# facebookresearch/PartDistillation

Measured on AMD Instinct MI355X. Metric: images/sec training step, R50 Mask2Former 1024² bs=2/GPU, 1/2/4/8 MI355X, higher is better.
Workload: dtype bf16

## Files before the change

### include/pd_attention.h

```cpp
#ifndef PD_ATTENTION_H
#define PD_ATTENTION_H

#include <stdint.h>

#ifdef __cplusplus
extern "C" {
#endif

int64_t pd_attn_workspace_floats(int B, int H, int Lq, int Lk);

int pd_attn_fwd_d32(const void *q, const void *k, const void *v, const uint8_t *mask, void *o, float *lse,
                    float *workspace, int B, int H, int Lq, int Lk, float scale, int dtype, void *stream);

int pd_attn_fwd_d32_ld(const void *q, const void *k, const void *v, const uint8_t *mask, void *o, float *lse,
                       float *workspace, int B, int H, int Lq, int Lk, float scale, int dtype, int ld_kv, void *stream);

int pd_attn_bwd_d32(const void *q, const void *k, const void *v, const uint8_t *mask, const void *o, const void *d_o,
                    const float *lse, void *dq, void *dk, void *dv, float *workspace, int B, int H, int Lq, int Lk,
                    float scale, int dtype, void *stream);

int pd_attn_bwd_d32_ld(const void *q, const void *k, const void *v, const uint8_t *mask, const void *o, const void *d_o,
                       const float *lse, void *dq, void *dk, void *dv, float *workspace, int B, int H, int Lq, int Lk,
                       float scale, int dtype, int ld_kv, void *stream);

#ifdef __cplusplus
}
#endif
#endif
```

### include/pd_declayer.h

```cpp
#ifndef PD_DECLAYER_H
#define PD_DECLAYER_H

#include <stdint.h>

#ifdef __cplusplus
extern "C" {
#endif

typedef struct PdDecPack {
  const void *src;
  void *dst;
  int32_t rows, cols, transpose;
} PdDecPack;
int64_t pd_dec_pack_table_bytes(int count);
int pd_dec_pack_grouped(const PdDecPack *descs, int count, void *table_host_pinned, void *table_device, void *stream);

int pd_dec_split(void);
int64_t pd_dec_workspace_bytes(int R);

int pd_dec_fwd_a(const void *o, const float *res, const float *qpos, int pos_div, const void *w_o, const void *b_o, const float *ln_w,
                 const float *ln_b, float eps, const void *w_qkv, const void *b_qkv, float *z, float *stats, float *y, void *y_c,
                 void *ypos_c, void *q, void *k, void *v, int R, void *stream);

int pd_dec_fwd_b(const void *o, const float *res, const float *qpos, int pos_div, const void *w_o, const void *b_o, const float *ln2_w,
                 const float *ln2_b, const void *w_1, const void *b_1, const void *w_2, const void *b_2, const float *ln3_w,
                 const float *ln3_b, const float *dn_w, const float *dn_b, const void *m0_w, const void *m0_b, const void *m1_w,
                 const void *m1_b, const void *m2_w, const void *m2_b, const void *wq_next, const void *bq_next, float eps, float *z2,
                 float *stats2, void *y2_c, void *h, float *z3, float *stats3, float *y3, void *ypos_c, float *dec_out, float *hstats,
                 void *ef, void *qc_next, void *workspace, int R, int flags, void *stream);

int pd_dec_bwd_b(const void *dqc_next, const void *wqT_next, const float *d_out, const float *d_res, const float *y3, const float *hstats,
                 const float *dn_w, float *dgb_dn, const float *z3, const float *stats3, const float *ln3_w, float *dgb3, float *db3,
                 float *pos_acc, int pos_div, const void *w2T, const void *h, const void *w1T, const float *z2, const float *stats2,
                 const float *ln2_w, float *dgb2, float *db2, const void *woT, void *dz3_c, void *dh, float *dz2, void *dz2_c, void *d_o,
                 void *workspace, int R, void *stream);

int pd_dec_bwd_a(const void *dq, const void *dk, const void *dv, const void *wqkvT, const float *dz_in, const float *z, const float *stats,
                 const float *ln_w, float *dgb, float *db, float *pos_acc, int pos_div, const void *woT, float *dz1, void *dz1_c, void *d_o,
                 int R, void *stream);

#ifdef __cplusplus
}
#endif
#endif
```

### partdistillation_amd/csrc/attention.hip

```cpp
#include <hip/hip_runtime.h>
#include <math.h>
#include <stdint.h>

#include "pd_attention.h"
#include "pd_common.h"
#include "mfma_bf16.h"
#include "pd_msda.h"

int g_attn_bwd_kc = 0;

namespace {

constexpr int D = 32;
constexpr int QP = 128;
constexpr int KT = 64;
constexpr int KC_FWD = 256;
constexpr int KC_DQ = 512;

typedef unsigned short bf16_t;

__device__ __forceinline__ float bf2f(bf16_t h) { return __uint_as_float((unsigned)h << 16); }
__device__ __forceinline__ bf16_t f2bf(float f)
{
  unsigned u = __float_as_uint(f);
// ... 92 lines not shown
    __syncthreads();
    if (!active) continue;
    const int kk0 = half * (KT / 2);
    float s[KT / 2];
    float m_t = -INFINITY;
    const uint8_t *mrow = mask ? mask + ((int64_t)b * Lq + qi) * Lk + k0 + kk0 : nullptr;
#pragma unroll
    for (int kk = 0; kk < KT / 2; ++kk) {
      float acc = 0.f;
#pragma unroll
      for (int d = 0; d < D; ++d) acc += qv[d] * Ks[kk0 + kk][d];
      const bool blocked = (k0 + kk0 + kk >= Lk) || (mrow && mrow[kk]);
      s[kk] = blocked ? -INFINITY : acc;
      m_t = fmaxf(m_t, s[kk]);
    }
    const float m_new = fmaxf(m_run, m_t);
    if (m_new == -INFINITY) continue;
    const float alpha = __expf(m_run - m_new);
    l_run *= alpha;
#pragma unroll
    for (int d = 0; d < D; ++d) o[d] *= alpha;
#pragma unroll
    for (int kk = 0; kk < KT / 2; ++kk) {
      const float p = __expf(s[kk] - m_new);
      l_run += p;
#pragma unroll
      for (int d = 0; d < D; ++d) o[d] += p * Vs[kk0 + kk][d];
    }
    m_run = m_new;
  }
  __syncthreads();
  const int ql = threadIdx.x & (QP - 1);
  if (half == 1) {
#pragma unroll
    for (int d = 0; d < D; ++d) red[ql][d] = o[d];
    red[ql][D] = m_run; red[ql][D + 1] = l_run;
  }
  __syncthreads();
  if (half == 0 && active) {
    const float m2 = red[ql][D], l2 = red[ql][D + 1];
    const float M = fmaxf(m_run, m2);
    const float a1 = (M == -INFINITY) ? 0.f : __expf(m_run - M), a2 = (M == -INFINITY) ? 0.f : __expf(m2 - M);
    const int64_t base = (((int64_t)b * H + h) * nchunk + chunk) * Lq + qi;
    float *po = part_o + base * D;
#pragma unroll
    for (int d = 0; d < D; d += 4)
      *reinterpret_cast<float4 *>(po + d) = make_float4(a1 * o[d] + a2 * red[ql][d], a1 * o[d + 1] + a2 * red[ql][d + 1],
                                                        a1 * o[d + 2] + a2 * red[ql][d + 2], a1 * o[d + 3] + a2 * red[ql][d + 3]);
    part_ml[base * 2] = M;
    part_ml[base * 2 + 1] = a1 * l_run + a2 * l2;
  }
}

template <typename T>
__global__ __launch_bounds__(256) void attn_fwd_combine(const float *__restrict__ part_o, const float *__restrict__ part_ml,
                                                         T *__restrict__ o, float *__restrict__ lse, int B, int H, int Lq, int nchunk)
{
  const int g = blockIdx.x * 8 + (threadIdx.x >> 5), d = threadIdx.x & 31;
  if (g >= B * H * Lq) return;
  const int qi = g % Lq, bh = g / Lq, h = bh % H, b = bh / H;
  float M = -INFINITY;
  const float2 *ml = reinterpret_cast<const float2 *>(part_ml) + (int64_t)bh * nchunk * Lq + qi;
  const float *po = part_o + ((int64_t)bh * nchunk * Lq + qi) * D + d;
  int c = 0;
  for (; c + 8 <= nchunk; c += 8) {
    float m8[8];
#pragma unroll
    for (int u = 0; u < 8; ++u) m8[u] = ml[(int64_t)(c + u) * Lq].x;
#pragma unroll
    for (int u = 0; u < 8; ++u) M = fmaxf(M, m8[u]);
  }
  for (; c < nchunk; ++c) M = fmaxf(M, ml[(int64_t)c * Lq].x);
  float L = 0.f, acc = 0.f;
  if (M != -INFINITY) {
    c = 0;
    for (; c + 8 <= nchunk; c += 8) {
      float2 s8[8];
      float o8[8];
#pragma unroll
      for (int u = 0; u < 8; ++u) { s8[u] = ml[(int64_t)(c + u) * Lq]; o8[u] = po[(int64_t)(c + u) * Lq * D]; }
#pragma unroll
      for (int u = 0; u < 8; ++u) {
        const float w = __expf(s8[u].x - M);
        L += w * s8[u].y;
        acc += w * o8[u];
      }
    }
    for (; c < nchunk; ++c) {
      const float2 sv = ml[(int64_t)c * Lq];
      const float w = __expf(sv.x - M);
      L += w * sv.y;
      acc += w * po[(int64_t)c * Lq * D];
    }
  }
  const float outv = L > 0.f ? acc / L : 0.f;
  T *dst = o + ((int64_t)qi * B + b) * (H * D) + h * D + d;
  if (sizeof(T) == 2) *reinterpret_cast<bf16_t *>(dst) = f2bf(outv); else *reinterpret_cast<float *>(dst) = outv;
  if (d == 0) lse[(int64_t)bh * Lq + qi] = L > 0.f ? M + __logf(L) : -INFINITY;
}

template <typename T>
__global__ __launch_bounds__(256) void attn_bwd_dq(const T *__restrict__ q, const T *__restrict__ k, const T *__restrict__ v,
                                                    const uint8_t *__restrict__ mask, const T *__restrict__ o, const T *__restrict__ d_o,
                                                    const float *__restrict__ lse, float *__restrict__ part_dq, int B, int H, int Lq,
                                                    int Lk, float scale, int nchunk, int qpass)
{
  __shared__ __attribute__((aligned(16))) float Ks[KT][D];
  __shared__ __attribute__((aligned(16))) float Vs[KT][D];
  __shared__ float red[QP][D];
  const int chunk = blockIdx.x, h = blockIdx.y, b = blockIdx.z;
  const int qi = qpass * QP + (threadIdx.x & (QP - 1)), half = threadIdx.x >> 7;
  const bool active = qi < Lq;
  float qv[D], dov[D], dq[D];
  float lse_q = 0.f, delta = 0.f;
#pragma unroll
  for (int d = 0; d < D; ++d) dq[d] = 0.f;
  if (active) {
    const int64_t off = ((int64_t)qi * B + b) * (H * D) + h * D;
    float ov[D];
    IO<T>::load32(q + off, qv);
    IO<T>::load32(d_o + off, dov);
    IO<T>::load32(o + off, ov);
#pragma unroll
    for (int d = 0; d < D; ++d) { delta += dov[d] * ov[d]; qv[d] *= scale; }
    lse_q = lse[((int64_t)b * H + h) * Lq + qi];
  }
  const int kbeg = chunk * KC_DQ, kend = min(Lk, kbeg + KC_DQ);
  for (int k0 = kbeg; k0 < kend; k0 += KT) {
    __syncthreads();
    stage_rows<T>(k, Ks, k0, Lk, b, h, B, H);
    stage_rows<T>(v, Vs, k0, Lk, b, h, B, H);
    __syncthreads();
    if (!active || lse_q == -INFINITY) continue;
    const int kk0 = half * (KT / 2);
    const uint8_t *mrow = mask ? mask + ((int64_t)b * Lq + qi) * Lk + k0 + kk0 : nullptr;
#pragma unroll 4
    for (int kk = 0; kk < KT / 2; ++kk) {
      const bool blocked = (k0 + kk0 + kk >= Lk) || (mrow && mrow[kk]);
      if (blocked) continue;
      float s = 0.f, dp = 0.f;
#pragma unroll
      for (int d = 0; d < D; ++d) { s += qv[d] * Ks[kk0 + kk][d]; dp += dov[d] * Vs[kk0 + kk][d]; }
      const float ds = __expf(s - lse_q) * (dp - delta);
#pragma unroll
      for (int d = 0; d < D; ++d) dq[d] += ds * Ks[kk0 + kk][d];
    }
  }
  __syncthreads();
  const int ql = threadIdx.x & (QP - 1);
  if (half == 1) {
#pragma unroll
    for (int d = 0; d < D; ++d) red[ql][d] = dq[d];
  }
  __syncthreads();
  if (half == 0 && active) {
    float *dst = part_dq + ((((int64_t)b * H + h) * nchunk + chunk) * Lq + qi) * D;
#pragma unroll
    for (int d = 0; d < D; d += 4)
      *reinterpret_cast<float4 *>(dst + d) = make_float4((dq[d] + red[ql][d]) * scale, (dq[d + 1] + red[ql][d + 1]) * scale,
                                                         (dq[d + 2] + red[ql][d + 2]) * scale, (dq[d + 3] + red[ql][d + 3]) * scale);
  }
}

template <typename T>
__global__ __launch_bounds__(256) void attn_bwd_dq_reduce(const float *__restrict__ part_dq, T *__restrict__ dq, int B, int H, int Lq, int nchunk)
{
  const int g = blockIdx.x * 8 + (threadIdx.x >> 5), d = threadIdx.x & 31;
  if (g >= B * H * Lq) return;
  const int qi = g % Lq, bh = g / Lq, h = bh % H, b = bh / H;
  float acc = 0.f;
  for (int c = 0; c < nchunk; ++c) acc += part_dq[(((int64_t)bh * nchunk + c) * Lq + qi) * D + d];
  T *dst = dq + ((int64_t)qi * B + b) * (H * D) + h * D + d;
  if (sizeof(T) == 2) *reinterpret_cast<bf16_t *>(dst) = f2bf(acc); else *reinterpret_cast<float *>(dst) = acc;
}

// ... 351 lines not shown
#pragma unroll
            for (int i = 0; i < 4; ++i) {
              const bool blocked = (mybits >> (8 * g + 4 * hh + i)) & 1u;
              p[i] = blocked ? 0.f : __expf(sN[4 * g + i] * scale - la[i]);
              ds[i] = p[i] * (dpN[4 * g + i] - da[i]);
            }
            pN[g] = pack4(p[0], p[1], p[2], p[3]);
            dsN[g] = pack4(ds[0], ds[1], ds[2], ds[3]);
          }
#pragma unroll
          for (int j = 0; j < 4; ++j) {
            mma(dvacc, lds4(&Ot[r][32 * sub + 8 * j + 4 * hh]), pN[j]);
            mma(dkacc, lds4(&Qt[r][32 * sub + 8 * j + 4 * hh]), dsN[j]);
          }
        }
      }
      if (kvalid) {
        bf16_t *dkp = dk + ((int64_t)key * B + b) * rs + h * D, *dvp = dv + ((int64_t)key * B + b) * rs + h * D;
#pragma unroll
        for (int g = 0; g < 4; ++g) {
          *reinterpret_cast<bf16x4 *>(dkp + 8 * g + 4 * hh) = pack4(dkacc[4 * g] * scale, dkacc[4 * g + 1] * scale, dkacc[4 * g + 2] * scale, dkacc[4 * g + 3] * scale);
          *reinterpret_cast<bf16x4 *>(dvp + 8 * g + 4 * hh) = pack4(dvacc[4 * g], dvacc[4 * g + 1], dvacc[4 * g + 2], dvacc[4 * g + 3]);
        }
      }
    }
  }
  for (int w = 0; w < 4; ++w) {
    __syncthreads();
    if (wave == w) {
#pragma unroll
      for (int sub = 0; sub < 4; ++sub)
#pragma unroll
        for (int e = 0; e < 16; ++e) {
          const int d = (e & 3) + 8 * (e >> 2) + 4 * hh;
          if (w == 0) dqs[32 * sub + r][d] = dqacc[sub][e];
          else dqs[32 * sub + r][d] += dqacc[sub][e];
        }
    }
  }
  __syncthreads();
  for (int idx = tid; idx < Lq * D; idx += 256) {
    const int qq = idx >> 5, d = idx & 31;
    const float val = dqs[qq][d] * scale;
    if (nchunk == 1) dq[((int64_t)qq * B + b) * rs + h * D + d] = f2bf(val);
    else part_dq[((bh * nchunk + chunk) * Lq + qq) * D + d] = val;
  }
}

inline int nchunks(int Lk, int kc) { return Lk <= 0 ? 1 : (Lk + kc - 1) / kc; }
inline int mfma_fwd_chunk(int B, int H, int Lk)
{
  int kc = KC_FWD;
  if (Lk > KC_FWD)
    while (kc > 64 && (int64_t)B * H * nchunks(Lk, kc) < 512) kc >>= 1;
  return kc;
}
inline int mfma_bwd_chunk(int B, int H, int Lk)
{
  if (g_attn_bwd_kc == 128 || g_attn_bwd_kc == 256 || g_attn_bwd_kc == 512) return g_attn_bwd_kc;
  int kc = KC_DQ;
  while (kc > 128 && (int64_t)B * H * nchunks(Lk, kc) < 256) kc >>= 1;
  return kc;
}

int check(const void *a, const void *b, const void *c, int B, int H, int Lq, int Lk, int dtype, const char *who)
{
  if (B < 0 || H <= 0 || Lq < 0 || Lk < 0) return pd_set_error(PD_ERR_INVALID_ARG, "%s: bad sizes B=%d H=%d Lq=%d Lk=%d", who, B, H, Lq, Lk);
  if (dtype != PD_F32 && dtype != PD_BF16) return pd_set_error(PD_ERR_INVALID_ARG, "%s: dtype %d (float32 / bfloat16 only)", who, dtype);
  if (B * Lq * Lk != 0 && (!a || !b || !c)) return pd_set_error(PD_ERR_INVALID_ARG, "%s: null pointer", who);
  return PD_OK;
}

}

int g_pd_dbg_attn_scalar = 0;

extern "C" int64_t pd_attn_workspace_floats(int B, int H, int Lq, int Lk)
{
  const int64_t n1 = (int64_t)B * H * nchunks(Lk, mfma_fwd_chunk(B, H, Lk)) * Lq * (D + 2);
  const int64_t n2 = (int64_t)B * H * nchunks(Lk, 128) * Lq * D;
  return (n1 > n2 ? n1 : n2) + 64;
}

extern "C" int pd_attn_fwd_d32(const void *q, const void *k, const void *v, const uint8_t *mask, void *o, float *lse,
                               float *workspace, int B, int H, int Lq, int Lk, float scale, int dtype, void *stream_)
{
  return pd_attn_fwd_d32_ld(q, k, v, mask, o, lse, workspace, B, H, Lq, Lk, scale, dtype, H * D, stream_);
}

extern "C" int pd_attn_fwd_d32_ld(const void *q, const void *k, const void *v, const uint8_t *mask, void *o, float *lse,
                                  float *workspace, int B, int H, int Lq, int Lk, float scale, int dtype, int ld_kv, void *stream_)
{
  int rc = check(q, k, v, B, H, Lq, Lk, dtype, "pd_attn_fwd_d32");
  if (rc) return rc;
  if (ld_kv < H * D || (ld_kv & 7)) return pd_set_error(PD_ERR_INVALID_ARG, "pd_attn_fwd_d32_ld: ld_kv=%d (>= H * 32, a multiple of 8)", ld_kv);
  if (ld_kv != H * D && !(dtype == PD_BF16 && Lq <= MQ && Lk > 0 && !g_pd_dbg_attn_scalar))
    return pd_set_error(PD_ERR_INVALID_ARG, "pd_attn_fwd_d32_ld: strided k / v only on the matrix-core path (bf16, <= %d queries)", MQ);
  if (B * Lq == 0) return PD_OK;
  if (!o || !lse || !workspace) return pd_set_error(PD_ERR_INVALID_ARG, "pd_attn_fwd_d32: null output");
  hipStream_t s = (hipStream_t)stream_;
  if (dtype == PD_BF16 && Lq <= MQ && Lk > 0 && !g_pd_dbg_attn_scalar) {
    const int kc = mfma_fwd_chunk(B, H, Lk), nc = nchunks(Lk, kc);
    float *part_o = workspace, *part_ml = workspace + (int64_t)B * H * nc * Lq * D;
    if (mask) hipLaunchKernelGGL(attn_fwd_mfma<true>, dim3(nc, H, B), dim3(256), 0, s, (const bf16_t *)q, (const bf16_t *)k, (const bf16_t *)v,
                                 mask, (bf16_t *)o, lse, part_o, part_ml, B, H, Lq, Lk, scale, nc, ld_kv, kc);
    else hipLaunchKernelGGL(attn_fwd_mfma<false>, dim3(nc, H, B), dim3(256), 0, s, (const bf16_t *)q, (const bf16_t *)k, (const bf16_t *)v,
                            mask, (bf16_t *)o, lse, part_o, part_ml, B, H, Lq, Lk, scale, nc, ld_kv, kc);
    if (nc > 1) hipLaunchKernelGGL(attn_fwd_combine<bf16_t>, dim3((B * H * Lq + 7) / 8), dim3(256), 0, s, part_o, part_ml, (bf16_t *)o, lse, B, H, Lq, nc);
    return pd_check_launch("pd_attn_fwd_d32");
  }
  const int nc = nchunks(Lk, KC_FWD);
  float *part_o = workspace, *part_ml = workspace + (int64_t)B * H * nc * Lq * D;
  for (int qp = 0; qp * QP < Lq; ++qp) {
    if (dtype == PD_BF16)
      hipLaunchKernelGGL(attn_fwd_partial<bf16_t>, dim3(nc, H, B), dim3(256), 0, s, (const bf16_t *)q, (const bf16_t *)k,
                         (const bf16_t *)v, mask, part_o, part_ml, B, H, Lq, Lk, scale, nc, qp);
    else
      hipLaunchKernelGGL(attn_fwd_partial<float>, dim3(nc, H, B), dim3(256), 0, s, (const float *)q, (const float *)k,
                         (const float *)v, mask, part_o, part_ml, B, H, Lq, Lk, scale, nc, qp);
  }
  const int groups = B * H * Lq;
  if (dtype == PD_BF16)
    hipLaunchKernelGGL(attn_fwd_combine<bf16_t>, dim3((groups + 7) / 8), dim3(256), 0, s, part_o, part_ml, (bf16_t *)o, lse, B, H, Lq, nc);
  else
    hipLaunchKernelGGL(attn_fwd_combine<float>, dim3((groups + 7) / 8), dim3(256), 0, s, part_o, part_ml, (float *)o, lse, B, H, Lq, nc);
  return pd_check_launch("pd_attn_fwd_d32");
}

extern "C" int pd_attn_bwd_d32(const void *q, const void *k, const void *v, const uint8_t *mask, const void *o, const void *d_o,
                               const float *lse, void *dq, void *dk, void *dv, float *workspace, int B, int H, int Lq,
                               int Lk, float scale, int dtype, void *stream_)
{
  return pd_attn_bwd_d32_ld(q, k, v, mask, o, d_o, lse, dq, dk, dv, workspace, B, H, Lq, Lk, scale, dtype, H * D, stream_);
}

extern "C" int pd_attn_bwd_d32_ld(const void *q, const void *k, const void *v, const uint8_t *mask, const void *o, const void *d_o,
                                  const float *lse, void *dq, void *dk, void *dv, float *workspace, int B, int H, int Lq,
                                  int Lk, float scale, int dtype, int ld_kv, void *stream_)
{
  int rc = check(q, k, v, B, H, Lq, Lk, dtype, "pd_attn_bwd_d32");
  if (rc) return rc;
  if (ld_kv < H * D || (ld_kv & 3)) return pd_set_error(PD_ERR_INVALID_ARG, "pd_attn_bwd_d32_ld: ld_kv=%d (>= H * 32, a multiple of 4)", ld_kv);
  if (ld_kv != H * D && !(dtype == PD_BF16 && Lq <= MQ && !g_pd_dbg_attn_scalar))
    return pd_set_error(PD_ERR_INVALID_ARG, "pd_attn_bwd_d32_ld: strided k / v only on the matrix-core path (bf16, <= %d queries)", MQ);
  if (B * Lq * Lk == 0) return PD_OK;
  if (!o || !d_o || !lse || !dq || !dk || !dv || !workspace) return pd_set_error(PD_ERR_INVALID_ARG, "pd_attn_bwd_d32: null pointer");
  hipStream_t s = (hipStream_t)stream_;
  const int groups = B * H * Lq;
  if (dtype == PD_BF16 && Lq <= MQ && !g_pd_dbg_attn_scalar) {
    const int kc = mfma_bwd_chunk(B, H, Lk), nc = nchunks(Lk, kc);
    if (mask) hipLaunchKernelGGL(attn_bwd_mfma<true>, dim3(nc, H, B), dim3(256), 0, s, (const bf16_t *)q, (const bf16_t *)k, (const bf16_t *)v,
                                 mask, (const bf16_t *)o, (const bf16_t *)d_o, lse, workspace, (bf16_t *)dq, (bf16_t *)dk, (bf16_t *)dv,
                                 B, H, Lq, Lk, scale, nc, kc, ld_kv);
    else hipLaunchKernelGGL(attn_bwd_mfma<false>, dim3(nc, H, B), dim3(256), 0, s, (const bf16_t *)q, (const bf16_t *)k, (const bf16_t *)v,
                            mask, (const bf16_t *)o, (const bf16_t *)d_o, lse, workspace, (bf16_t *)dq, (bf16_t *)dk, (bf16_t *)dv,
                            B, H, Lq, Lk, scale, nc, kc, ld_kv);
    if (nc > 1) hipLaunchKernelGGL(attn_bwd_dq_reduce<bf16_t>, dim3((groups + 7) / 8), dim3(256), 0, s, workspace, (bf16_t *)dq, B, H, Lq, nc);
    return pd_check_launch("pd_attn_bwd_d32");
  }
  const int nc = nchunks(Lk, KC_DQ);
  if (dtype == PD_BF16) {
    for (int qp = 0; qp * QP < Lq; ++qp)
      hipLaunchKernelGGL(attn_bwd_dq<bf16_t>, dim3(nc, H, B), dim3(256), 0, s, (const bf16_t *)q, (const bf16_t *)k, (const bf16_t *)v,
                         mask, (const bf16_t *)o, (const bf16_t *)d_o, lse, workspace, B, H, Lq, Lk, scale, nc, qp);
    hipLaunchKernelGGL(attn_bwd_dq_reduce<bf16_t>, dim3((groups + 7) / 8), dim3(256), 0, s, workspace, (bf16_t *)dq, B, H, Lq, nc);
    hipLaunchKernelGGL(attn_bwd_dkv<bf16_t>, dim3((Lk + 255) / 256, H, B), dim3(256), 0, s, (const bf16_t *)q, (const bf16_t *)k,
                       (const bf16_t *)v, mask, (const bf16_t *)o, (const bf16_t *)d_o, lse, (bf16_t *)dk, (bf16_t *)dv, B, H, Lq, Lk, scale);
  } else {
    for (int qp = 0; qp * QP < Lq; ++qp)
      hipLaunchKernelGGL(attn_bwd_dq<float>, dim3(nc, H, B), dim3(256), 0, s, (const float *)q, (const float *)k, (const float *)v,
                         mask, (const float *)o, (const float *)d_o, lse, workspace, B, H, Lq, Lk, scale, nc, qp);
    hipLaunchKernelGGL(attn_bwd_dq_reduce<float>, dim3((groups + 7) / 8), dim3(256), 0, s, workspace, (float *)dq, B, H, Lq, nc);
    hipLaunchKernelGGL(attn_bwd_dkv<float>, dim3((Lk + 255) / 256, H, B), dim3(256), 0, s, (const float *)q, (const float *)k,
                       (const float *)v, mask, (const float *)o, (const float *)d_o, lse, (float *)dk, (float *)dv, B, H, Lq, Lk, scale);
  }
  return pd_check_launch("pd_attn_bwd_d32");
}
```

### partdistillation_amd/csrc/cmdbuf.hip

```cpp
#include <hip/hip_runtime.h>
#include <stdint.h>
#include <string.h>

#include <type_traits>
#include <utility>

#include "pd_common.h"
#include "pd_cmdbuf.h"
#include "pd_attention.h"
#include "pd_conv.h"
#include "pd_declayer.h"
#include "pd_criterion.h"
#include "pd_fused.h"
#include "pd_gemm.h"
#include "pd_grouping.h"
#include "pd_igemm.h"
#include "pd_input.h"
#include "pd_kmeans.h"
#include "pd_msda.h"
#include "pd_mx8.h"
#include "pd_optim.h"
#include "pd_rowwise.h"
#include "pd_smallgemm.h"
#include "pd_stem.h"
// ... 15 lines not shown
    return static_cast<T>(static_cast<int64_t>(w));
  }
}

template <auto F> struct Thunk;
template <class... A, int (*F)(A...)>
struct Thunk<F> {
  static constexpr int nargs = (int)sizeof...(A);
  template <size_t... I>
  static int invoke(const uint64_t *w, std::index_sequence<I...>) { return F(word_to<A>(w[I])...); }
  static int call(const uint64_t *w) { return invoke(w, std::index_sequence_for<A...>{}); }
};

struct Entry { const char *name; int (*call)(const uint64_t *); int nargs; };
#define PD_E(f) {#f, &Thunk<&f>::call, Thunk<&f>::nargs}
const Entry kTable[] = {
  PD_E(pd_adamw_clipped),
  PD_E(pd_adamw_clipped_shadow),
  PD_E(pd_add_layernorm_bwd),
  PD_E(pd_add_layernorm_bwd_amax),
  PD_E(pd_add_layernorm_fwd),
  PD_E(pd_add_layernorm_fwd_amax),
  PD_E(pd_add_rows_amax_f32),
  PD_E(pd_affine_act_bwd2_bf16),
  PD_E(pd_affine_act_bwd_bf16),
  PD_E(pd_affine_act_fwd_bf16),
  PD_E(pd_attn_bwd_d32),
  PD_E(pd_attn_fwd_d32),
  PD_E(pd_attn_mask_u8),
  PD_E(pd_cast_bf16_f32_amax),
  PD_E(pd_colsum_acc),
  PD_E(pd_conv3x3_nhwc_f16x2),
  PD_E(pd_conv3x3_nhwc_f32x3),
  PD_E(pd_conv3x3_wgrad_nhwc_f16x2),
  PD_E(pd_conv3x3_wgrad_nhwc_f32x3),
  PD_E(pd_conv_bf16_dgrad),
  PD_E(pd_conv_bf16_fwd),
  PD_E(pd_conv_bf16_wgrad),
  PD_E(pd_conv_bf16_wgrad_grouped),
  PD_E(pd_dec_bwd_a),
  PD_E(pd_dec_bwd_b),
  PD_E(pd_dec_fwd_a),
  PD_E(pd_dec_fwd_b),
  PD_E(pd_dec_pack_grouped),
  PD_E(pd_decoder_head_bf16),
  PD_E(pd_filter_transpose_grouped),
  PD_E(pd_gemm_tn_f16x2),
  PD_E(pd_gemm_tn_f16x2_bf16out),
  PD_E(pd_gemm_tn_f32),
  PD_E(pd_gemm_tn_f32x3),
  PD_E(pd_gemm_tn_f32x3_pre),
  PD_E(pd_gemm_tn_f32x3_relu_bits),
  PD_E(pd_gemm_tn_f32x3_relumask),
  PD_E(pd_gemm_wgrad_acc_f16x2_ws),
  PD_E(pd_gemm_wgrad_acc_f32),
  PD_E(pd_gemm_wgrad_acc_f32x3),
  PD_E(pd_gemm_wgrad_acc_f32x3_ws),
  PD_E(pd_gemm_wgrad_f16x2_grouped),
  PD_E(pd_gemm_wgrad_f32),
  PD_E(pd_gemm_wgrad_f32x3_grouped),
  PD_E(pd_gn_coeffs_bwd),
  PD_E(pd_gn_coeffs_fwd),
  PD_E(pd_igemm_bf16),
  PD_E(pd_igemm_bf16_seq),
  PD_E(pd_kmeans_assign),
  PD_E(pd_kmeans_assign_bounded),
  PD_E(pd_kmeans_assign_partial),
  PD_E(pd_kmeans_reduce),
  PD_E(pd_kmeans_reduce_update),
  PD_E(pd_kmeans_reduce_update_shift),
  PD_E(pd_kmeans_update),
  PD_E(pd_layernorm_rows_f32_bwd),
  PD_E(pd_layernorm_rows_f32_fwd),
  PD_E(pd_loss_vectors_bwd),
  PD_E(pd_loss_vectors_fwd),
  PD_E(pd_lsa_batched),
  PD_E(pd_mask_assign),
  PD_E(pd_mask_point_losses_bwd),
  PD_E(pd_mask_point_losses_fwd),
  PD_E(pd_matcher_costs),
  PD_E(pd_copy_segments),
  PD_E(pd_attn_fwd_d32_ld),
  PD_E(pd_attn_bwd_d32_ld),
  PD_E(pd_match_point_logits),
  PD_E(pd_swin_merge_ln_fwd),
  PD_E(pd_swin_tail_ln_fwd),
  PD_E(pd_swin_tail_ln_bwd),
  PD_E(pd_swin_merge_ln_bwd),
  PD_E(pd_matcher_point_terms),
  PD_E(pd_maxpool3s2_bwd_bf16),
  PD_E(pd_maxpool3s2_fwd_bf16),
  PD_E(pd_mem_prep_bwd),
  PD_E(pd_mem_prep_fwd),
  PD_E(pd_memcpy_d2d_async),
  PD_E(pd_memset_async),
  PD_E(pd_msda_backward),
  PD_E(pd_msda_forward),
  PD_E(pd_msda_forward_amax),
  PD_E(pd_msda_fused_backward),
  PD_E(pd_msda_fused_forward),
  PD_E(pd_msda_prep_bwd),
  PD_E(pd_msda_prep_bwd_amax),
  PD_E(pd_msda_prep_fwd),
  PD_E(pd_multi_gather_sumsq),
  PD_E(pd_mx8_gemm),
  PD_E(pd_mx8_quantize_bf16),
  PD_E(pd_mx8_quantize_grouped),
  PD_E(pd_nc_affine2_amax_f32),
  PD_E(pd_nc_affine2_f32),
  PD_E(pd_nc_affine_amax_f32),
  PD_E(pd_nc_affine_f32),
  PD_E(pd_nc_sums_f32),
  PD_E(pd_normalize_u8_nhwc),
  PD_E(pd_pair_logits_bwd_rows),
  PD_E(pd_pair_logits_bwd_tok),
  PD_E(pd_pair_logits_fwd),
  PD_E(pd_point_sample_nhwc_f32),
  PD_E(pd_point_sample_nhwc_f32_bf16),
  PD_E(pd_point_sample_planar_bwd_f32),
  PD_E(pd_point_sample_planar_f32),
  PD_E(pd_point_sample_u8),
  PD_E(pd_relu_bwd_colsum),
  PD_E(pd_resample_cols_u8),
  PD_E(pd_resample_rows_u8),
  PD_E(pd_resize_bilinear_nhwc_f32),
  PD_E(pd_rle_sample_u8),
  PD_E(pd_row_amax_f32),
  PD_E(pd_scores_argmax_u8),
  PD_E(pd_sgemm_nn_bf16),
  PD_E(pd_sgemm_nn_splitn_bf16),
  PD_E(pd_sgemm_tn_batched_bf16),
  PD_E(pd_sgemm_tn_bf16),
  PD_E(pd_sgemm_tn_multi_bf16),
  PD_E(pd_sgemm_tn_splitk_bf16),
  PD_E(pd_sgemm_wgrad_bf16),
  PD_E(pd_sgemm_wgrad_grouped_bf16),
  PD_E(pd_sgemm_wgrad_split_bf16),
  PD_E(pd_skinny_linear_bwd),
  PD_E(pd_skinny_linear_fwd),
  PD_E(pd_split3_bf16),
  PD_E(pd_stem7x7_fwd),
  PD_E(pd_stem7x7_wgrad),
  PD_E(pd_sum3_sum2_f32),
  PD_E(pd_sumsq_accumulate),
  PD_E(pd_swin_ln_bwd),
  PD_E(pd_swin_ln_fwd),
  PD_E(pd_transpose_batched_f32),
  PD_E(pd_uncertain_points),
  PD_E(pd_upsample2x_bwd_nhwc_f32),
  PD_E(pd_upsample_add_amax_nhwc_f32),
  PD_E(pd_upsample_add_nhwc_f32),
  PD_E(pd_wgrad_bf16),
  PD_E(pd_wgrad_bf16_seq),
  PD_E(pd_window_attn_bwd_w12),
  PD_E(pd_window_attn_fwd_w12),
};
constexpr int kCount = (int)(sizeof(kTable) / sizeof(kTable[0]));
}

extern "C" int pd_memset_async(void *dst, int value, int64_t bytes, void *stream)
{
  if (bytes <= 0) return PD_OK;
  return hipMemsetAsync(dst, value, (size_t)bytes, (hipStream_t)stream) == hipSuccess ? PD_OK : pd_set_error(PD_ERR_LAUNCH, "pd_memset_async failed");
}

extern "C" int pd_memcpy_d2d_async(void *dst, const void *src, int64_t bytes, void *stream)
// ... 36 lines not shown
```

### partdistillation_amd/csrc/common.hip

```cpp
#include <hip/hip_runtime.h>
#include <stdarg.h>
#include <stdio.h>
#include <string.h>

#include "pd_common.h"
#include "pd_msda.h"

namespace {
thread_local char g_err[512] = {0};
}

int pd_set_error(int code, const char *fmt, ...)
{
  va_list ap;
  va_start(ap, fmt);
  vsnprintf(g_err, sizeof(g_err), fmt, ap);
  va_end(ap);
  return code;
}

int pd_check_launch(const char *what)
{
  hipError_t e = hipGetLastError();
  if (e == hipSuccess) return PD_OK;
  return pd_set_error(PD_ERR_LAUNCH, "%s: %s", what, hipGetErrorString(e));
}

extern "C" const char *pd_last_error(void) { return g_err; }
extern "C" int pd_abi_version(void) { return 40; }

extern int g_pd_dbg_atomic_scope;
extern int g_pd_dbg_force_generic;
extern int g_pd_dbg_ablate;
extern int g_pd_dbg_x3_narrow;
extern int g_pd_dbg_f16x2;
extern int g_pd_dbg_wgrad_wide;
extern "C" void pd_dbg_set_wgrad_xcd(int v);
extern "C" void pd_dbg_set_wgrad_fast(int v);
extern int g_pd_dbg_bwd_variant;
extern int g_pd_dbg_msda_gate_pct;
extern int g_pd_dbg_wgrad_wgs;
extern int g_pd_dbg_bwd_threads;
extern int g_pd_dbg_attn_scalar;
extern int g_pd_dbg_wattn;
extern int g_pd_dbg_x3;
extern int g_pd_dbg_kmeans;
extern int g_pd_dbg_conv_group_rows;
extern int g_pd_dbg_conv_xcd_major;
extern int g_pd_dbg_sgemm_deep;
extern int g_ig_bn, g_ig_nst, g_ig_splits, g_ig_patch, g_ig_pcls;
extern int g_mx_bn, g_mx_nst;
extern int g_swin_ln_abl;
extern int g_ln_bwd_cap;
extern int g_crit_abl;
extern int g_attn_bwd_kc;
extern int g_wg_nst, g_wg_splits, g_wg_mode;
extern "C" int pd_debug_set(const char *key, int value)
{
  if (!key) return PD_ERR_INVALID_ARG;
  if (!strcmp(key, "msda_bwd_atomic_scope")) { g_pd_dbg_atomic_scope = value; return PD_OK; }
  if (!strcmp(key, "msda_ablate")) { g_pd_dbg_ablate = value; return PD_OK; }
  if (!strcmp(key, "msda_bwd_variant")) { g_pd_dbg_bwd_variant = value; return PD_OK; }
  if (!strcmp(key, "msda_gate_pct")) { g_pd_dbg_msda_gate_pct = value; return PD_OK; }
  if (!strcmp(key, "attn_scalar")) { g_pd_dbg_attn_scalar = value; return PD_OK; }
  if (!strcmp(key, "msda_bwd_threads")) { g_pd_dbg_bwd_threads = value; return PD_OK; }
  if (!strcmp(key, "wgrad_wgs")) { g_pd_dbg_wgrad_wgs = value; return PD_OK; }
  if (!strcmp(key, "kmeans_ablate")) { g_pd_dbg_kmeans = value; return PD_OK; }
  if (!strcmp(key, "wg_nst")) { g_wg_nst = value; return PD_OK; }
  if (!strcmp(key, "wg_splits")) { g_wg_splits = value; return PD_OK; }
  if (!strcmp(key, "wg_mode")) { g_wg_mode = value; return PD_OK; }
  if (!strcmp(key, "ig_bn")) { g_ig_bn = value; return PD_OK; }
  if (!strcmp(key, "ig_patch")) { g_ig_patch = value; return PD_OK; }
  if (!strcmp(key, "ig_pcls")) { g_ig_pcls = value; return PD_OK; }
  if (!strcmp(key, "ig_nst")) { g_ig_nst = value; return PD_OK; }
  if (!strcmp(key, "mx_bn")) { g_mx_bn = value; return PD_OK; }
  if (!strcmp(key, "attn_bwd_kc")) { g_attn_bwd_kc = value; return PD_OK; }
  if (!strcmp(key, "crit_abl")) { g_crit_abl = value; return PD_OK; }
  if (!strcmp(key, "ln_bwd_cap")) { g_ln_bwd_cap = value; return PD_OK; }
  if (!strcmp(key, "swin_ln_abl")) { g_swin_ln_abl = value; return PD_OK; }
  if (!strcmp(key, "mx_nst")) { g_mx_nst = value; return PD_OK; }
  if (!strcmp(key, "ig_splits")) { g_ig_splits = value; return PD_OK; }
  if (!strcmp(key, "sgemm_deep")) { g_pd_dbg_sgemm_deep = value; return PD_OK; }
  if (!strcmp(key, "conv_group_rows")) { g_pd_dbg_conv_group_rows = value; return PD_OK; }
  if (!strcmp(key, "conv_xcd_major")) { g_pd_dbg_conv_xcd_major = value; return PD_OK; }
  if (!strcmp(key, "x3_ablate")) { g_pd_dbg_x3 = value; return PD_OK; }
  if (!strcmp(key, "f16x2_tile")) { g_pd_dbg_f16x2 = value; return PD_OK; }
  if (!strcmp(key, "wgrad_wide")) { g_pd_dbg_wgrad_wide = value; return PD_OK; }
  if (!strcmp(key, "wgrad_xcd")) { pd_dbg_set_wgrad_xcd(value); return PD_OK; }
  if (!strcmp(key, "wgrad_fast")) { pd_dbg_set_wgrad_fast(value); return PD_OK; }
  if (!strcmp(key, "x3_narrow")) { g_pd_dbg_x3_narrow = value; return PD_OK; }
  if (!strcmp(key, "wattn_ablate")) { g_pd_dbg_wattn = value; return PD_OK; }
  if (!strcmp(key, "msda_force_generic")) { g_pd_dbg_force_generic = value; return PD_OK; }
  return pd_set_error(PD_ERR_INVALID_ARG, "pd_debug_set: unknown key %s", key);
}
```

### partdistillation_amd/csrc/declayer.hip

```cpp
#include <hip/hip_runtime.h>
#include <stdint.h>
#include <stdlib.h>

#include "pd_common.h"
#include "pd_msda.h"
#include "pd_declayer.h"

namespace {

typedef unsigned short bf16_t;
typedef __bf16 hwbf16x8 __attribute__((ext_vector_type(8)));
typedef __bf16 hwbf16x2 __attribute__((ext_vector_type(2)));
typedef float f32x4 __attribute__((ext_vector_type(4)));
typedef float f32x2 __attribute__((ext_vector_type(2)));

constexpr int C = 256, FF = 2048, RB = 16, NTH = 512, NW = 8;
constexpr int PA = C + 8;
constexpr int PZ = C + 4;

__device__ __forceinline__ float bf2f(bf16_t h) { return __uint_as_float((unsigned)h << 16); }
__device__ __forceinline__ float bf_lo(unsigned u) { return __uint_as_float(u << 16); }
__device__ __forceinline__ float bf_hi(unsigned u) { return __uint_as_float(u & 0xffff0000u); }
__device__ __forceinline__ unsigned pk_bf16(float lo, float hi)
{
  const f32x2 x = {lo, hi};
  return __builtin_bit_cast(unsigned, __builtin_convertvector(x, hwbf16x2));
}
__device__ __forceinline__ uint2 pack4(float a, float b, float c, float d) { return make_uint2(pk_bf16(a, b), pk_bf16(c, d)); }
__device__ __forceinline__ float rbf(float x) { return bf_lo(pk_bf16(x, 0.f)); }

template <int CTRL>
__device__ __forceinline__ float dpp_mov(float v)
{
  return __int_as_float(__builtin_amdgcn_update_dpp(0, __float_as_int(v), CTRL, 0xF, 0xF, true));
}
__device__ __forceinline__ float wave_sum(float v)
{
  v += dpp_mov<0xB1>(v);
  v += dpp_mov<0x4E>(v);
  v += dpp_mov<0x141>(v);
  v += dpp_mov<0x140>(v);
  v += __shfl_xor(v, 16, 64);
  v += __shfl_xor(v, 32, 64);
  return v;
}
__device__ __forceinline__ float4 add4(float4 a, float4 b) { return make_float4(a.x + b.x, a.y + b.y, a.z + b.z, a.w + b.w); }
__device__ __forceinline__ float4 ld4(const float *p) { return *reinterpret_cast<const float4 *>(p); }
__device__ __forceinline__ void st4(float *p, float4 v) { *reinterpret_cast<float4 *>(p) = v; }
__device__ __forceinline__ float4 zero4() { return make_float4(0.f, 0.f, 0.f, 0.f); }

__device__ __forceinline__ void zero_acc(f32x4 (&acc)[2])
{
#pragma unroll
  for (int t = 0; t < 2; ++t)
#pragma unroll
    for (int r = 0; r < 4; ++r) acc[t][r] = 0.f;
}

template <bool BIAS, bool RELU>
__device__ __forceinline__ void epi4(const f32x4 &a, const bf16_t *bias_lds, int n, float (&v)[4])
{
#pragma unroll
  for (int r = 0; r < 4; ++r) v[r] = a[r];
  if (BIAS) {
    const uint2 b = *reinterpret_cast<const uint2 *>(bias_lds + n);
    v[0] += bf_lo(b.x); v[1] += bf_hi(b.x); v[2] += bf_lo(b.y); v[3] += bf_hi(b.y);
  }
  if (RELU) {
#pragma unroll
    for (int r = 0; r < 4; ++r) v[r] = fmaxf(v[r], 0.f);
  }
}
template <bool BIAS, bool RELU>
__device__ __forceinline__ void store_tile_bf16(const f32x4 (&acc)[2], const bf16_t *bias_lds, int nb_bias, bf16_t *dst, int pitch, int nb, int lane)
{
  const int m = lane & 15, g = lane >> 4;
#pragma unroll
  for (int t = 0; t < 2; ++t) {
    float v[4];
    epi4<BIAS, RELU>(acc[t], bias_lds, nb_bias + 16 * t + 4 * g, v);
    *reinterpret_cast<uint2 *>(dst + m * pitch + nb + 16 * t + 4 * g) = pack4(v[0], v[1], v[2], v[3]);
  }
}
// ... 24 lines not shown
{
  for (int i = tid * 8; i < n; i += NTH * 8) *reinterpret_cast<uint4 *>(dst + i) = *reinterpret_cast<const uint4 *>(src + i);
}
__device__ __forceinline__ void lds_copy_f32(float *dst, const float *__restrict__ src, int n, int tid)
{
  for (int i = tid * 4; i < n; i += NTH * 4) st4(dst + i, ld4(src + i));
}

__device__ __forceinline__ float4 ln_row(float4 v, float4 gm, float4 bt, float eps, float &mu, float &rs)
{
  const float s = (v.x + v.y) + (v.z + v.w);
  mu = wave_sum(s) * (1.f / C);
  v.x -= mu; v.y -= mu; v.z -= mu; v.w -= mu;
  const float q = (v.x * v.x + v.y * v.y) + (v.z * v.z + v.w * v.w);
  rs = rsqrtf(wave_sum(q) * (1.f / C) + eps);
  return make_float4(v.x * rs * gm.x + bt.x, v.y * rs * gm.y + bt.y, v.z * rs * gm.z + bt.z, v.w * rs * gm.w + bt.w);
}
__device__ __forceinline__ float4 ln_row_bwd(float4 t, float4 z, float mu, float rs, float4 gm, float4 &ag, float4 &ab)
{
  float4 h = make_float4((z.x - mu) * rs, (z.y - mu) * rs, (z.z - mu) * rs, (z.w - mu) * rs);
  ag.x += t.x * h.x; ag.y += t.y * h.y; ag.z += t.z * h.z; ag.w += t.w * h.w;
  ab = add4(ab, t);
  t.x *= gm.x; t.y *= gm.y; t.z *= gm.z; t.w *= gm.w;
  const float s1 = (t.x + t.y) + (t.z + t.w);
  const float s2 = (t.x * h.x + t.y * h.y) + (t.z * h.z + t.w * h.w);
  const float m1 = wave_sum(s1) * (1.f / C), m2 = wave_sum(s2) * (1.f / C);
  return make_float4(rs * (t.x - m1 - h.x * m2), rs * (t.y - m1 - h.y * m2), rs * (t.z - m1 - h.z * m2), rs * (t.w - m1 - h.w * m2));
}
__device__ __forceinline__ float4 bf4(const bf16_t *p)
{
  const uint2 u = *reinterpret_cast<const uint2 *>(p);
  return make_float4(bf_lo(u.x), bf_hi(u.x), bf_lo(u.y), bf_hi(u.y));
}
__device__ __forceinline__ void st_bf4(bf16_t *p, float4 v) { *reinterpret_cast<uint2 *>(p) = pack4(v.x, v.y, v.z, v.w); }

template <int NARR>
__device__ __forceinline__ void flush_colsums(const float *red, float *const (&outs)[NARR], int tid)
{
  for (int i = tid; i < NARR * C; i += NTH) {
    const int k = i / C, c = i - k * C;
    if (!outs[k]) continue;
    float s = 0.f;
#pragma unroll
    for (int w = 0; w < NW; ++w) s += red[(w * NARR + k) * C + c];
    atomicAdd(outs[k] + c, s);
  }
}

constexpr int BLK = 8192;
struct WHalf { uint4 v[2][4]; };
__device__ __forceinline__ void wloadh(WHalf &w, const bf16_t *__restrict__ blk, int half, int lane)
{
  const bf16_t *p = blk + lane * 8 + half * (4 * 512);
#pragma unroll
  for (int t = 0; t < 2; ++t)
#pragma unroll
    for (int s = 0; s < 4; ++s) w.v[t][s] = *reinterpret_cast<const uint4 *>(p + (t * 8 + s) * 512);
}
__device__ __forceinline__ void wmmah(f32x4 (&acc)[2], const WHalf &w, const bf16_t *xs)
{
#pragma unroll
  for (int s = 0; s < 4; ++s) {
    const hwbf16x8 x = *reinterpret_cast<const hwbf16x8 *>(xs + 32 * s);
    acc[0] = __builtin_amdgcn_mfma_f32_16x16x32_bf16(__builtin_bit_cast(hwbf16x8, w.v[0][s]), x, acc[0], 0, 0, 0);
    acc[1] = __builtin_amdgcn_mfma_f32_16x16x32_bf16(__builtin_bit_cast(hwbf16x8, w.v[1][s]), x, acc[1], 0, 0, 0);
  }
}
#define PD_HP(h) do { if ((h) < 2 * NBLK) wloadh(w[(h) & 3], bp((h) >> 1), (h) & 1, lane); } while (0)
#define PD_BLK(b, XS) do { PD_HP(2 * (b) + 3); wmmah(acc, w[(2 * (b)) & 3], (XS)); PD_HP(2 * (b) + 4); wmmah(acc, w[(2 * (b) + 1) & 3], (XS) + 128); } while (0)

__device__ __forceinline__ void slab_store(float *__restrict__ slab, const f32x4 (&acc)[2], int nb, int lane)
{
  const int m = lane & 15, g = lane >> 4;
#pragma unroll
  for (int t = 0; t < 2; ++t) st4(slab + m * C + nb + 16 * t + 4 * g, make_float4(acc[t][0], acc[t][1], acc[t][2], acc[t][3]));
}
__device__ __forceinline__ float4 slab_sum(const float *__restrict__ slabs, int P, int row, int lane)
{
  float4 s = zero4();
  for (int p = 0; p < P; ++p) s = add4(s, ld4(slabs + (size_t)p * (RB * C) + row * C + 4 * lane));
  return s;
}

struct FwdA {
  const bf16_t *o; const float *res, *qpos; int pos_div;
  const bf16_t *w_o, *b_o; const float *ln_w, *ln_b; float eps;
  const bf16_t *w_qkv, *b_qkv;
  float *z, *stats, *y; bf16_t *y_c, *ypos_c, *q, *k, *v; int R;
};

__global__ __launch_bounds__(NTH) void dec_fwd_a(const FwdA a)
{
  extern __shared__ __attribute__((aligned(16))) unsigned char smem[];
  bf16_t *X0 = reinterpret_cast<bf16_t *>(smem);
  bf16_t *X1 = X0 + RB * PA;
  bf16_t *X2 = X1 + RB * PA;
  bf16_t *X3 = X2 + RB * PA;
  bf16_t *X4 = X3 + RB * PA;
  float *Zs = reinterpret_cast<float *>(X4 + RB * PA);
  bf16_t *Bs = reinterpret_cast<bf16_t *>(Zs + RB * PZ);
  float *Ls = reinterpret_cast<float *>(Bs + 4 * C);
  const int tid = threadIdx.x, wave = tid >> 6, lane = tid & 63, r0 = blockIdx.x * RB, R = a.R;
  constexpr int NBLK = 4;
  auto bp = [&](int b) { return b == 0 ? a.w_o + (size_t)wave * BLK : a.w_qkv + (size_t)((b - 1) * 8 + wave) * BLK; };
  WHalf w[4];
  PD_HP(0); PD_HP(1); PD_HP(2);
  tile_in(X0, a.o, r0, R, tid);
  lds_copy_bf16(Bs, a.b_o, C, tid);
  lds_copy_bf16(Bs + C, a.b_qkv, 3 * C, tid);
  lds_copy_f32(Ls, a.ln_w, C, tid);
  lds_copy_f32(Ls + C, a.ln_b, C, tid);
  float4 res[2], pos[2];
#pragma unroll
  for (int i = 0; i < 2; ++i) {
    const int m = min(r0 + 2 * wave + i, R - 1);
    res[i] = ld4(a.res + (size_t)m * C + 4 * lane);
    pos[i] = ld4(a.qpos + (size_t)(m / a.pos_div) * C + 4 * lane);
  }
  __syncthreads();
  const int xo = (lane & 15) * PA + 8 * (lane >> 4);
  f32x4 acc[2];
  zero_acc(acc);
  PD_BLK(0, X0 + xo);
  store_tile_f32r<true>(acc, Bs, 32 * wave, Zs, 32 * wave, lane);
  __syncthreads();
#pragma unroll
  for (int i = 0; i < 2; ++i) {
    const int row = 2 * wave + i, m = r0 + row;
    const float4 zv = add4(ld4(Zs + row * PZ + 4 * lane), res[i]);
    float mu, rs;
    const float4 y = ln_row(zv, ld4(Ls + 4 * lane), ld4(Ls + C + 4 * lane), a.eps, mu, rs);
    const float4 yp = add4(y, pos[i]);
    st_bf4(X1 + row * PA + 4 * lane, y);
    st_bf4(X2 + row * PA + 4 * lane, yp);
    if (m < R) {
      st4(a.z + (size_t)m * C + 4 * lane, zv);
      st4(a.y + (size_t)m * C + 4 * lane, y);
      if (lane == 0) { a.stats[m] = mu; a.stats[R + m] = rs; }
    }
  }
  __syncthreads();
  tile_out(a.y_c, X1, r0, R, tid);
  tile_out(a.ypos_c, X2, r0, R, tid);
  zero_acc(acc);
  PD_BLK(1, X2 + xo);
  store_tile_bf16<true, false>(acc, Bs + C, 32 * wave, X0, PA, 32 * wave, lane);
  zero_acc(acc);
  PD_BLK(2, X2 + xo);
  store_tile_bf16<true, false>(acc, Bs + 2 * C, 32 * wave, X3, PA, 32 * wave, lane);
  zero_acc(acc);
  PD_BLK(3, X1 + xo);
  store_tile_bf16<true, false>(acc, Bs + 3 * C, 32 * wave, X4, PA, 32 * wave, lane);
  __syncthreads();
  tile_out(a.q, X0, r0, R, tid);
  tile_out(a.k, X3, r0, R, tid);
  tile_out(a.v, X4, r0, R, tid);
}
constexpr size_t kSmemFwdA = (size_t)5 * RB * PA * 2 + (size_t)RB * PZ * 4 + 4 * C * 2 + 2 * C * 4;

struct FwdB {
  const bf16_t *o; const float *res, *qpos; int pos_div;
  const bf16_t *w_o, *b_o; const float *ln2_w, *ln2_b;
  const bf16_t *w_1, *b_1, *w_2, *b_2; const float *ln3_w, *ln3_b, *dn_w, *dn_b;
  const bf16_t *m_w[3], *m_b[3], *wq_next, *bq_next; float eps;
  float *z2, *stats2; bf16_t *y2_c, *h; float *z3, *stats3, *y3; bf16_t *ypos_c; float *dec_out, *hstats;
  bf16_t *ef, *qc_next; int R; float *slabs, *rows; int nsplit;
};

template <int P, int PART, bool LAYER, bool MLP>
__global__ __launch_bounds__(NTH) void dec_fwd_b(const FwdB a)
{
  static_assert(PART != 2 || !LAYER, "PART 2 starts behind the FFN");
  constexpr int NB = 8 / P, HW = FF / P, PHS = HW + 8;
  extern __shared__ __attribute__((aligned(16))) unsigned char smem[];
  bf16_t *X0 = reinterpret_cast<bf16_t *>(smem);
  bf16_t *X1 = X0 + RB * PA;
  bf16_t *X2 = X1 + RB * PA;
  bf16_t *Hs = X2 + RB * PA;
  float *Zs = reinterpret_cast<float *>(Hs + RB * (PHS > PA ? PHS : PA));
  bf16_t *Bs = reinterpret_cast<bf16_t *>(Zs + RB * PZ);
  float *Ls = reinterpret_cast<float *>(Bs + (6 * C + FF));
  float *Ys = Ls + 6 * C;
  float *Ps = Ys + RB * PZ;
  const int tid = threadIdx.x, wave = tid >> 6, lane = tid & 63, R = a.R;
  const int rb = blockIdx.x / P, p = blockIdx.x - rb * P, r0 = rb * RB;
  constexpr int B1 = C, B2 = C + FF, BM = 2 * C + FF, BQ = 5 * C + FF;
  constexpr int I0 = LAYER ? 2 * NB + 1 : 0;
  constexpr int NBLK = I0 + (MLP && PART != 1 ? 4 : 0);
  auto bp = [&](int b) -> const bf16_t * {
    if (LAYER && b == 0) return a.w_o + (size_t)wave * BLK;
// ... 69 lines not shown
      const int idx = i * NTH + tid, row = idx / (HW / 8), col = (idx % (HW / 8)) * 8;
      if (r0 + row < R) *reinterpret_cast<uint4 *>(a.h + (size_t)(r0 + row) * FF + p * HW + col) = *reinterpret_cast<const uint4 *>(Hs + row * PHS + col);
    }
    const int ho = (lane & 15) * PHS + 8 * (lane >> 4);
    zero_acc(acc);
#pragma unroll
    for (int c = 0; c < NB; ++c) {
      PD_BLK(NB + 1 + c, Hs + ho + 256 * c);
    }
    if (PART == 1) {
      slab_store(a.slabs + (size_t)(rb * P + p) * (RB * C), acc, 32 * wave, lane);
      return;
    }
    store_tile_f32r<true>(acc, Bs + B2, 32 * wave, Zs, 32 * wave, lane);
    __syncthreads();
  }
#pragma unroll
  for (int i = 0; i < 2; ++i) {
    const int row = 2 * wave + i, m = r0 + row;
    float4 y3 = ld4(Ys + row * PZ + 4 * lane);
    float mu, rs;
    if (LAYER || PART == 2) {
      float4 x3;
      if (PART == 2) {
        x3 = add4(slab_sum(a.slabs + (size_t)rb * a.nsplit * (RB * C), a.nsplit, row, lane), bf4(Bs + B2 + 4 * lane));
        x3 = make_float4(rbf(x3.x), rbf(x3.y), rbf(x3.z), rbf(x3.w));
      } else {
        x3 = ld4(Zs + row * PZ + 4 * lane);
      }
      const float4 zv = add4(x3, y3);
      y3 = ln_row(zv, ld4(Ls + 2 * C + 4 * lane), ld4(Ls + 3 * C + 4 * lane), a.eps, mu, rs);
      if (m < R) {
        st4(a.z3 + (size_t)m * C + 4 * lane, zv);
        st4(a.y3 + (size_t)m * C + 4 * lane, y3);
        if (lane == 0) { a.stats3[m] = mu; a.stats3[R + m] = rs; }
      }
    }
    st_bf4(X2 + row * PA + 4 * lane, add4(y3, ld4(Ps + row * PZ + 4 * lane)));
    const float4 d = ln_row(y3, ld4(Ls + 4 * C + 4 * lane), ld4(Ls + 5 * C + 4 * lane), a.eps, mu, rs);
    st_bf4(X0 + row * PA + 4 * lane, d);
    if (m < R) {
      st4(a.dec_out + (size_t)m * C + 4 * lane, d);
      if (lane == 0) { a.hstats[m] = mu; a.hstats[R + m] = rs; }
    }
  }
  __syncthreads();
  tile_out(a.ypos_c, X2, r0, R, tid);
  if (!MLP) return;
  zero_acc(acc);
  PD_BLK(I0, X0 + xo);
  store_tile_bf16<true, true>(acc, Bs + BM, 32 * wave, X1, PA, 32 * wave, lane);
  __syncthreads();
  zero_acc(acc);
  PD_BLK(I0 + 1, X1 + xo);
  store_tile_bf16<true, true>(acc, Bs + BM + C, 32 * wave, X0, PA, 32 * wave, lane);
  __syncthreads();
  zero_acc(acc);
  PD_BLK(I0 + 2, X0 + xo);
  store_tile_bf16<true, false>(acc, Bs + BM + 2 * C, 32 * wave, X1, PA, 32 * wave, lane);
  zero_acc(acc);
  PD_BLK(I0 + 3, X2 + xo);
  store_tile_bf16<true, false>(acc, Bs + BQ, 32 * wave, Hs, PA, 32 * wave, lane);
  __syncthreads();
  tile_out(a.qc_next, Hs, r0, R, tid);
  {
    const int row = tid >> 5, col = (tid & 31) * 8, m = r0 + row;
    if (m < R) {
      const int B = a.pos_div, q = m / B, b = m - q * B, Q = R / B;
      *reinterpret_cast<uint4 *>(a.ef + ((size_t)b * Q + q) * C + col) = *reinterpret_cast<const uint4 *>(X1 + row * PA + col);
    }
  }
}
template <int P>
constexpr size_t smem_fwd_b()
{
  return (size_t)3 * RB * PA * 2 + (size_t)RB * ((FF / P + 8) > PA ? (FF / P + 8) : PA) * 2 + (size_t)3 * RB * PZ * 4 + (size_t)(6 * C + FF) * 2 + 6 * C * 4;
}

struct BwdB {
  const bf16_t *dqc_next, *wqT_next; const float *d_out, *d_res, *y3, *hstats, *dn_w; float *dgb_dn;
  const float *z3, *stats3, *ln3_w; float *dgb3, *db3, *pos_acc; int pos_div;
  const bf16_t *w2T, *h, *w1T; const float *z2, *stats2, *ln2_w; float *dgb2, *db2; const bf16_t *woT;
  bf16_t *dz3_c, *dh; float *dz2; bf16_t *dz2_c, *d_o; int R; float *slabs, *rows; int nsplit;
};

template <int P, int PART, bool NXT>
__global__ __launch_bounds__(NTH) void dec_bwd_b(const BwdB a)
{
  constexpr int NB = 8 / P, HW = FF / P, PHS = HW + 8;
  extern __shared__ __attribute__((aligned(16))) unsigned char smem[];
  bf16_t *X0 = reinterpret_cast<bf16_t *>(smem);
  bf16_t *X1 = X0 + RB * PA;
  bf16_t *Hs = X1 + RB * PA;
  float *Zs = reinterpret_cast<float *>(Hs + RB * PHS);
  float *red = Zs + RB * PZ;
  float *Ls = red + NW * 5 * C;
  float *Gs = Ls + 3 * C;
  const int tid = threadIdx.x, wave = tid >> 6, lane = tid & 63, R = a.R;
  const int rb = blockIdx.x / P, p = blockIdx.x - rb * P, r0 = rb * RB;
  constexpr int I0 = NXT ? 1 : 0;
  constexpr int IW = PART == 2 ? 0 : I0 + 2 * NB;
  constexpr int NBLK = PART == 1 ? I0 + 2 * NB : IW + 1;
  auto bp = [&](int b) -> const bf16_t * {
    if (PART == 2) return a.woT + (size_t)wave * BLK;
    if (NXT && b == 0) return a.wqT_next + (size_t)wave * BLK;
    const int j = b - I0;
    return j < NB ? a.w2T + (size_t)(p * (64 / P) + wave * NB + j) * BLK
                  : j < 2 * NB ? a.w1T + (size_t)(8 * wave + p * NB + j - NB) * BLK : a.woT + (size_t)wave * BLK;
  };
  WHalf w[4];
  PD_HP(0); PD_HP(1); PD_HP(2);
  const int xo = (lane & 15) * PA + 8 * (lane >> 4);
  f32x4 acc[2];
  lds_copy_f32(Ls + 2 * C, a.ln2_w, C, tid);
  if (PART != 2) {
  if (NXT) tile_in(X0, a.dqc_next, r0, R, tid);
#pragma unroll
  for (int i = 0; i < HW * RB / 8 / NTH; ++i) {
    const int idx = i * NTH + tid, row = idx / (HW / 8), col = (idx % (HW / 8)) * 8;
    *reinterpret_cast<uint4 *>(Hs + row * PHS + col) = *reinterpret_cast<const uint4 *>(a.h + (size_t)min(r0 + row, R - 1) * FF + p * HW + col);
  }
  lds_copy_f32(Ls, a.dn_w, C, tid);
  lds_copy_f32(Ls + C, a.ln3_w, C, tid);
  float4 dy[2], y3v[2], z3v[2];
  float st[2][4];
#pragma unroll
  for (int i = 0; i < 2; ++i) {
    const int mr = r0 + 2 * wave + i, m = min(mr, R - 1);
    const size_t o = (size_t)m * C + 4 * lane;
    dy[i] = mr < R ? ld4(a.d_out + o) : zero4();
    y3v[i] = ld4(a.y3 + o); z3v[i] = ld4(a.z3 + o);
    st[i][0] = a.hstats[m]; st[i][1] = a.hstats[R + m];
    st[i][2] = a.stats3[m]; st[i][3] = a.stats3[R + m];
  }
  __syncthreads();
  if (NXT) {
    zero_acc(acc);
    PD_BLK(0, X0 + xo);
    store_tile_f32r<false>(acc, nullptr, 0, Zs, 32 * wave, lane);
    __syncthreads();
  }
  {
    float4 ag_dn = zero4(), ab_dn = zero4(), ag = zero4(), ab = zero4(), ad = zero4();
    const float4 gdn = ld4(Ls + 4 * lane), g3w = ld4(Ls + C + 4 * lane);
#pragma unroll
    for (int i = 0; i < 2; ++i) {
      const int row = 2 * wave + i, mr = r0 + row;
      const bool valid = mr < R;
      float4 t = ln_row_bwd(dy[i], y3v[i], st[i][0], st[i][1], gdn, ag_dn, ab_dn);
      if (a.d_res && valid) t = add4(t, ld4(a.d_res + (size_t)mr * C + 4 * lane));
      if (NXT && valid) {
        const float4 ps = ld4(Zs + row * PZ + 4 * lane);
        t = add4(t, ps);
        if (p == 0) {
          float *pa = a.pos_acc + (size_t)(mr / a.pos_div) * C + 4 * lane;
          atomicAdd(pa, ps.x); atomicAdd(pa + 1, ps.y); atomicAdd(pa + 2, ps.z); atomicAdd(pa + 3, ps.w);
        }
      }
      if (!valid) t = zero4();
      const float4 o = ln_row_bwd(t, z3v[i], st[i][2], st[i][3], g3w, ag, ab);
      ad = add4(ad, o);
      st4(Gs + row * PZ + 4 * lane, o);
      st_bf4(X0 + row * PA + 4 * lane, o);
      if (PART == 1 && p == 0 && valid) st4(a.rows + (size_t)mr * C + 4 * lane, o);
    }
    float *rw = red + wave * 5 * C + 4 * lane;
    st4(rw, ag_dn); st4(rw + C, ab_dn); st4(rw + 2 * C, ag); st4(rw + 3 * C, ab); st4(rw + 4 * C, ad);
  }
  __syncthreads();
  if (p == 0) {
    tile_out(a.dz3_c, X0, r0, R, tid);
    float *const outs[5] = {a.dgb_dn, a.dgb_dn + C, a.dgb3, a.dgb3 + C, a.db3};
    flush_colsums<5>(red, outs, tid);
  }
#pragma unroll
  for (int c = 0; c < NB; ++c) {
    zero_acc(acc);
    PD_BLK(I0 + c, X0 + xo);
    const int m = lane & 15, g = lane >> 4;
#pragma unroll
    for (int t = 0; t < 2; ++t) {
      bf16_t *hp = Hs + m * PHS + (wave * NB + c) * 32 + 16 * t + 4 * g;
      const uint2 hv = *reinterpret_cast<const uint2 *>(hp);
      float v[4] = {acc[t][0], acc[t][1], acc[t][2], acc[t][3]};
      if (!(bf_lo(hv.x) > 0.f)) v[0] = 0.f;
      if (!(bf_hi(hv.x) > 0.f)) v[1] = 0.f;
      if (!(bf_lo(hv.y) > 0.f)) v[2] = 0.f;
      if (!(bf_hi(hv.y) > 0.f)) v[3] = 0.f;
      *reinterpret_cast<uint2 *>(hp) = pack4(v[0], v[1], v[2], v[3]);
    }
  }
  __syncthreads();
#pragma unroll
  for (int i = 0; i < HW * RB / 8 / NTH; ++i) {
    const int idx = i * NTH + tid, row = idx / (HW / 8), col = (idx % (HW / 8)) * 8;
    if (r0 + row < R) *reinterpret_cast<uint4 *>(a.dh + (size_t)(r0 + row) * FF + p * HW + col) = *reinterpret_cast<const uint4 *>(Hs + row * PHS + col);
  }
  const int ho = (lane & 15) * PHS + 8 * (lane >> 4);
  zero_acc(acc);
// ... 147 lines not shown
  while (lo < hi) {
    const int mid = (lo + hi + 1) >> 1;
    if (tab[mid].first_block <= bid) lo = mid; else hi = mid - 1;
  }
  PackProblem pr = tab[lo];
  pr.src = pd_as_global(pr.src); pr.dst = pd_as_global(pr.dst);
  const int local = bid - pr.first_block;
  const int K = pr.transpose ? pr.rows : pr.cols, kcn = K / 256, nb = local / kcn, kc = local - nb * kcn;
  bf16_t *dst = pr.dst + (size_t)local * BLK;
  const int tid = threadIdx.x;
  if (!pr.transpose) {
#pragma unroll
    for (int j = 0; j < 4; ++j) {
      const int piece = j * 256 + tid, i = piece >> 6, lane = piece & 63, t = i >> 3, s = i & 7;
      const uint4 v = *reinterpret_cast<const uint4 *>(pr.src + (size_t)(32 * nb + 16 * t + (lane & 15)) * pr.cols + 256 * kc + 32 * s + 8 * (lane >> 4));
      *reinterpret_cast<uint4 *>(dst + (size_t)piece * 8) = v;
    }
    return;
  }
#pragma unroll
  for (int j = 0; j < 4; ++j) {
    const int piece = j * 256 + tid, k = piece >> 2, c8 = (piece & 3) * 8;
    *reinterpret_cast<uint4 *>(&tile[k][c8]) = *reinterpret_cast<const uint4 *>(pr.src + (size_t)(256 * kc + k) * pr.cols + 32 * nb + c8);
  }
  __syncthreads();
#pragma unroll
  for (int j = 0; j < 4; ++j) {
    const int piece = j * 256 + tid, i = piece >> 6, lane = piece & 63, t = i >> 3, s = i & 7;
    const int n = 16 * t + (lane & 15), k0 = 32 * s + 8 * (lane >> 4);
    unsigned short e[8];
#pragma unroll
    for (int q = 0; q < 8; ++q) e[q] = tile[k0 + q][n];
    uint4 o;
    o.x = e[0] | ((unsigned)e[1] << 16); o.y = e[2] | ((unsigned)e[3] << 16); o.z = e[4] | ((unsigned)e[5] << 16); o.w = e[6] | ((unsigned)e[7] << 16);
    *reinterpret_cast<uint4 *>(dst + (size_t)piece * 8) = o;
  }
}

template <class K>
int allow_smem(K kernel, size_t bytes, const char *who)
{
  if (hipFuncSetAttribute(reinterpret_cast<const void *>(kernel), hipFuncAttributeMaxDynamicSharedMemorySize, (int)bytes) != hipSuccess)
    return pd_set_error(PD_ERR_LAUNCH, "%s: cannot reserve %zu bytes of LDS", who, bytes);
  return PD_OK;
}

int g_split = -1;
int split_mode()
{
  if (g_split < 0) {
    const char *e = getenv("PD_DEC_SPLIT");
    const int v = e ? atoi(e) : 4;
    g_split = (v == 1 || v == 2 || v == 4 || v == 8) ? v : 4;
  }
  return g_split;
}

template <int P, int PART, bool LAYER, bool MLP>
int launch_fwd_b(const FwdB &a, hipStream_t s)
{
  static int ok = allow_smem(dec_fwd_b<P, PART, LAYER, MLP>, smem_fwd_b<P>(), "pd_dec_fwd_b");
  if (ok != PD_OK) return ok;
  hipLaunchKernelGGL((dec_fwd_b<P, PART, LAYER, MLP>), dim3(((a.R + RB - 1) / RB) * (PART == 1 ? P : 1)), dim3(NTH), smem_fwd_b<P>(), s, a);
  return pd_check_launch("pd_dec_fwd_b");
}
template <int P>
int launch_fwd_b_split(const FwdB &a, bool mlp, hipStream_t s)
{
  const int rc = launch_fwd_b<P, 1, true, false>(a, s);
  if (rc != PD_OK) return rc;
  return mlp ? launch_fwd_b<1, 2, false, true>(a, s) : launch_fwd_b<1, 2, false, false>(a, s);
}
template <int P, int PART, bool NXT>
int launch_bwd_b(const BwdB &a, hipStream_t s)
{
  static int ok = allow_smem(dec_bwd_b<P, PART, NXT>, smem_bwd_b<P>(), "pd_dec_bwd_b");
  if (ok != PD_OK) return ok;
  hipLaunchKernelGGL((dec_bwd_b<P, PART, NXT>), dim3(((a.R + RB - 1) / RB) * (PART == 1 ? P : 1)), dim3(NTH), smem_bwd_b<P>(), s, a);
  return pd_check_launch("pd_dec_bwd_b");
}
template <int P>
int launch_bwd_b_split(const BwdB &a, hipStream_t s)
{
  const int rc = a.dqc_next ? launch_bwd_b<P, 1, true>(a, s) : launch_bwd_b<P, 1, false>(a, s);
  if (rc != PD_OK) return rc;
  return launch_bwd_b<1, 2, false>(a, s);
}

}

extern "C" int pd_dec_split(void) { return split_mode(); }
extern "C" int64_t pd_dec_workspace_bytes(int R) { return R <= 0 ? 0 : (int64_t)((R + RB - 1) / RB) * (8 + 1) * RB * C * 4; }
extern "C" int64_t pd_dec_pack_table_bytes(int count) { return (int64_t)count * sizeof(PackProblem); }

extern "C" int pd_dec_pack_grouped(const PdDecPack *descs, int count, void *table_host_pinned, void *table_device, void *stream)
{
  if (count <= 0) return PD_OK;
  if (!descs || !table_host_pinned || !table_device) return pd_set_error(PD_ERR_INVALID_ARG, "pd_dec_pack_grouped: null pointer");
  PackProblem *h = reinterpret_cast<PackProblem *>(table_host_pinned);
  int blocks = 0;
  for (int i = 0; i < count; ++i) {
    const PdDecPack &d = descs[i];
    const int N = d.transpose ? d.cols : d.rows, K = d.transpose ? d.rows : d.cols;
    if (!d.src || !d.dst || N <= 0 || K <= 0 || N % 32 || K % 256)
      return pd_set_error(PD_ERR_INVALID_ARG, "pd_dec_pack_grouped: problem %d: output rows %% 32 == 0 and contraction %% 256 == 0 required (%d x %d)", i, N, K);
    h[i] = PackProblem{(const bf16_t *)d.src, (bf16_t *)d.dst, d.rows, d.cols, d.transpose, blocks};
    blocks += (N / 32) * (K / 256);
  }
  if (hipMemcpyAsync(table_device, h, (size_t)count * sizeof(PackProblem), hipMemcpyHostToDevice, (hipStream_t)stream) != hipSuccess)
    return pd_set_error(PD_ERR_LAUNCH, "pd_dec_pack_grouped: table upload failed");
  hipLaunchKernelGGL(dec_pack_grouped, dim3((unsigned)blocks), dim3(256), 0, (hipStream_t)stream, (const PackProblem *)table_device, count);
  return pd_check_launch("pd_dec_pack_grouped");
}

extern "C" int pd_dec_fwd_a(const void *o, const float *res, const float *qpos, int pos_div, const void *w_o, const void *b_o, const float *ln_w,
                            const float *ln_b, float eps, const void *w_qkv, const void *b_qkv, float *z, float *stats, float *y, void *y_c,
                            void *ypos_c, void *q, void *k, void *v, int R, void *stream)
{
  if (!o || !res || !qpos || !w_o || !b_o || !ln_w || !ln_b || !w_qkv || !b_qkv || !z || !stats || !y || !y_c || !ypos_c || !q || !k || !v)
    return pd_set_error(PD_ERR_INVALID_ARG, "pd_dec_fwd_a: null pointer");
  if (R <= 0 || pos_div <= 0) return pd_set_error(PD_ERR_INVALID_ARG, "pd_dec_fwd_a: R = %d, pos_div = %d", R, pos_div);
  static int ok = allow_smem(dec_fwd_a, kSmemFwdA, "pd_dec_fwd_a");
  if (ok != PD_OK) return ok;
  FwdA a{(const bf16_t *)o, res, qpos, pos_div, (const bf16_t *)w_o, (const bf16_t *)b_o, ln_w, ln_b, eps, (const bf16_t *)w_qkv, (const bf16_t *)b_qkv,
         z, stats, y, (bf16_t *)y_c, (bf16_t *)ypos_c, (bf16_t *)q, (bf16_t *)k, (bf16_t *)v, R};
  hipLaunchKernelGGL(dec_fwd_a, dim3((R + RB - 1) / RB), dim3(NTH), kSmemFwdA, (hipStream_t)stream, a);
  return pd_check_launch("pd_dec_fwd_a");
}

extern "C" int pd_dec_fwd_b(const void *o, const float *res, const float *qpos, int pos_div, const void *w_o, const void *b_o, const float *ln2_w,
                            const float *ln2_b, const void *w_1, const void *b_1, const void *w_2, const void *b_2, const float *ln3_w,
                            const float *ln3_b, const float *dn_w, const float *dn_b, const void *m0_w, const void *m0_b, const void *m1_w,
                            const void *m1_b, const void *m2_w, const void *m2_b, const void *wq_next, const void *bq_next, float eps, float *z2,
                            float *stats2, void *y2_c, void *h, float *z3, float *stats3, float *y3, void *ypos_c, float *dec_out, float *hstats,
                            void *ef, void *qc_next, void *workspace, int R, int flags, void *stream)
{
  const bool layer = flags & 1, mlp = flags & 2;
  if (!res || !qpos || !dn_w || !dn_b || !ypos_c || !dec_out || !hstats) return pd_set_error(PD_ERR_INVALID_ARG, "pd_dec_fwd_b: null pointer");
  if (layer && (!o || !w_o || !b_o || !ln2_w || !ln2_b || !w_1 || !b_1 || !w_2 || !b_2 || !ln3_w || !ln3_b || !z2 || !stats2 || !y2_c || !h || !z3 || !stats3 ||
                !y3))
    return pd_set_error(PD_ERR_INVALID_ARG, "pd_dec_fwd_b: null pointer (layer part)");
  if (mlp && (!m0_w || !m0_b || !m1_w || !m1_b || !m2_w || !m2_b || !wq_next || !bq_next || !ef || !qc_next))
    return pd_set_error(PD_ERR_INVALID_ARG, "pd_dec_fwd_b: null pointer (head part)");
  if (R <= 0 || pos_div <= 0 || R % pos_div) return pd_set_error(PD_ERR_INVALID_ARG, "pd_dec_fwd_b: R = %d, pos_div = %d", R, pos_div);
  FwdB a{(const bf16_t *)o, res, qpos, pos_div, (const bf16_t *)w_o, (const bf16_t *)b_o, ln2_w, ln2_b, (const bf16_t *)w_1, (const bf16_t *)b_1,
         (const bf16_t *)w_2, (const bf16_t *)b_2, ln3_w, ln3_b, dn_w, dn_b,
         {(const bf16_t *)m0_w, (const bf16_t *)m1_w, (const bf16_t *)m2_w}, {(const bf16_t *)m0_b, (const bf16_t *)m1_b, (const bf16_t *)m2_b},
         (const bf16_t *)wq_next, (const bf16_t *)bq_next, eps, z2, stats2, (bf16_t *)y2_c, (bf16_t *)h, z3, stats3, y3, (bf16_t *)ypos_c, dec_out, hstats,
         (bf16_t *)ef, (bf16_t *)qc_next, R, reinterpret_cast<float *>(workspace),
         reinterpret_cast<float *>(workspace) + (size_t)((R + RB - 1) / RB) * 8 * RB * C, (layer && workspace) ? split_mode() : 1};
  hipStream_t s = (hipStream_t)stream;
  if (!layer) return mlp ? launch_fwd_b<1, 0, false, true>(a, s) : launch_fwd_b<1, 0, false, false>(a, s);
  switch (a.nsplit) {
    case 2: return launch_fwd_b_split<2>(a, mlp, s);
    case 4: return launch_fwd_b_split<4>(a, mlp, s);
    case 8: return launch_fwd_b_split<8>(a, mlp, s);
    default: return mlp ? launch_fwd_b<1, 0, true, true>(a, s) : launch_fwd_b<1, 0, true, false>(a, s);
  }
}

extern "C" int pd_dec_bwd_b(const void *dqc_next, const void *wqT_next, const float *d_out, const float *d_res, const float *y3, const float *hstats,
                            const float *dn_w, float *dgb_dn, const float *z3, const float *stats3, const float *ln3_w, float *dgb3, float *db3,
                            float *pos_acc, int pos_div, const void *w2T, const void *h, const void *w1T, const float *z2, const float *stats2,
                            const float *ln2_w, float *dgb2, float *db2, const void *woT, void *dz3_c, void *dh, float *dz2, void *dz2_c, void *d_o,
                            void *workspace, int R, void *stream)
{
  if (!d_out || !y3 || !hstats || !dn_w || !dgb_dn || !z3 || !stats3 || !ln3_w || !dgb3 || !db3 || !w2T || !h || !w1T || !z2 || !stats2 || !ln2_w ||
      !dgb2 || !db2 || !woT || !dz3_c || !dh || !dz2 || !dz2_c || !d_o)
    return pd_set_error(PD_ERR_INVALID_ARG, "pd_dec_bwd_b: null pointer");
  if ((dqc_next != nullptr) != (wqT_next != nullptr) || (dqc_next && !pos_acc)) return pd_set_error(PD_ERR_INVALID_ARG, "pd_dec_bwd_b: next-layer operands");
  if (R <= 0 || pos_div <= 0) return pd_set_error(PD_ERR_INVALID_ARG, "pd_dec_bwd_b: R = %d, pos_div = %d", R, pos_div);
  BwdB a{(const bf16_t *)dqc_next, (const bf16_t *)wqT_next, d_out, d_res, y3, hstats, dn_w, dgb_dn, z3, stats3, ln3_w, dgb3, db3, pos_acc, pos_div,
         (const bf16_t *)w2T, (const bf16_t *)h, (const bf16_t *)w1T, z2, stats2, ln2_w, dgb2, db2, (const bf16_t *)woT, (bf16_t *)dz3_c, (bf16_t *)dh, dz2,
         (bf16_t *)dz2_c, (bf16_t *)d_o, R, reinterpret_cast<float *>(workspace),
         reinterpret_cast<float *>(workspace) + (size_t)((R + RB - 1) / RB) * 8 * RB * C, workspace ? split_mode() : 1};
  hipStream_t s = (hipStream_t)stream;
  switch (a.nsplit) {
    case 2: return launch_bwd_b_split<2>(a, s);
    case 4: return launch_bwd_b_split<4>(a, s);
    case 8: return launch_bwd_b_split<8>(a, s);
    default: return a.dqc_next ? launch_bwd_b<1, 0, true>(a, s) : launch_bwd_b<1, 0, false>(a, s);
  }
}

extern "C" int pd_dec_bwd_a(const void *dq, const void *dk, const void *dv, const void *wqkvT, const float *dz_in, const float *z, const float *stats,
                            const float *ln_w, float *dgb, float *db, float *pos_acc, int pos_div, const void *woT, float *dz1, void *dz1_c, void *d_o,
                            int R, void *stream)
{
  if (!dq || !dk || !dv || !wqkvT || !dz_in || !z || !stats || !ln_w || !dgb || !db || !pos_acc || !woT || !dz1 || !dz1_c || !d_o)
    return pd_set_error(PD_ERR_INVALID_ARG, "pd_dec_bwd_a: null pointer");
  if (R <= 0 || pos_div <= 0) return pd_set_error(PD_ERR_INVALID_ARG, "pd_dec_bwd_a: R = %d, pos_div = %d", R, pos_div);
  static int ok = allow_smem(dec_bwd_a, kSmemBwdA, "pd_dec_bwd_a");
  if (ok != PD_OK) return ok;
  BwdA a{(const bf16_t *)dq, (const bf16_t *)dk, (const bf16_t *)dv, (const bf16_t *)wqkvT, dz_in, z, stats, ln_w, dgb, db, pos_acc, pos_div,
         (const bf16_t *)woT, dz1, (bf16_t *)dz1_c, (bf16_t *)d_o, R};
  hipLaunchKernelGGL(dec_bwd_a, dim3((R + RB - 1) / RB), dim3(NTH), kSmemBwdA, (hipStream_t)stream, a);
  return pd_check_launch("pd_dec_bwd_a");
}
```

### partdistillation_amd/functions/attention.py

```python
import torch
from torch.autograd import Function

from .. import lib as _lib

_DT = {torch.float32: _lib.PD_F32, torch.bfloat16: _lib.PD_BF16}
_WS = {}


def _workspace(B, H, Lq, Lk, device):
    n = int(_lib.load().pd_attn_workspace_floats(B, H, Lq, Lk))
    from .. import cmdbuf
    if cmdbuf.active() is not None:
        return torch.empty(max(n, 1), dtype=torch.float32, device=device)
    key = str(device)
    ws = _WS.get(key)
    if ws is None or ws.numel() < n:
        ws = torch.empty(n, dtype=torch.float32, device=device)
        _WS[key] = ws
    return ws


def _stream():
    return _lib.current_stream()


def _ld_kv(k, v):
    assert k.dim() == 2 and k.shape == v.shape and k.stride(1) == 1 and v.stride(1) == 1 and k.stride(0) == v.stride(0) >= k.shape[1]
    return k.stride(0)


def attn_fwd_raw(q, k, v, m8, B, nheads, scale):
    Lq, Lk = q.shape[0] // B, k.shape[0] // B
    o = torch.empty_like(q)
    lse = torch.empty((B, nheads, Lq), dtype=torch.float32, device=q.device)
    ws = _workspace(B, nheads, Lq, Lk, q.device)
    _lib.check(_lib.load().pd_attn_fwd_d32_ld(q.data_ptr(), k.data_ptr(), v.data_ptr(), m8.data_ptr() if m8 is not None else None,
                                              o.data_ptr(), lse.data_ptr(), ws.data_ptr(), B, nheads, Lq, Lk, float(scale),
                                              _DT[q.dtype], _ld_kv(k, v), _stream()))
    return o, lse


def attn_bwd_raw(q, k, v, m8, o, d_o, lse, B, nheads, scale):
    Lq, Lk = q.shape[0] // B, k.shape[0] // B
    dq = torch.empty_like(q)
    dk, dv = (torch.empty(k.shape, dtype=k.dtype, device=k.device) for _ in range(2))
    ws = _workspace(B, nheads, Lq, Lk, q.device)
    _lib.check(_lib.load().pd_attn_bwd_d32_ld(q.data_ptr(), k.data_ptr(), v.data_ptr(), m8.data_ptr() if m8 is not None else None,
                                              o.data_ptr(), d_o.data_ptr(), lse.data_ptr(), dq.data_ptr(), dk.data_ptr(), dv.data_ptr(),
                                              ws.data_ptr(), B, nheads, Lq, Lk, float(scale), _DT[q.dtype], _ld_kv(k, v), _stream()))
    return dq, dk, dv


class MaskedAttention32(Function):

    @staticmethod
    def forward(ctx, q, k, v, mask, nheads, scale):
        if not q.is_cuda:
            raise RuntimeError("pd_attn_fwd_d32 runs on the GPU only (no CPU fallback in partdistillation_amd)")
        q, k, v = q.contiguous(), k.contiguous(), v.contiguous()
        Lq, B, C = q.shape
        Lk = k.shape[0]
        assert C == nheads * 32 and q.dtype in _DT and k.dtype == q.dtype and v.dtype == q.dtype
        m8 = None
        if mask is not None:
            m8 = mask.contiguous().view(torch.uint8)
            assert m8.shape == (B, Lq, Lk)
        o = torch.empty_like(q)
        lse = torch.empty((B, nheads, Lq), dtype=torch.float32, device=q.device)
        ws = _workspace(B, nheads, Lq, Lk, q.device)
        with torch.cuda.device(q.device):
            rc = _lib.load().pd_attn_fwd_d32(q.data_ptr(), k.data_ptr(), v.data_ptr(), m8.data_ptr() if m8 is not None else None,
                                             o.data_ptr(), lse.data_ptr(), ws.data_ptr(), B, nheads, Lq, Lk, float(scale),
                                             _DT[q.dtype], _stream())
        _lib.check(rc)
        ctx.save_for_backward(q, k, v, m8, o, lse)
        ctx.nheads, ctx.scale = nheads, float(scale)
        return o

    @staticmethod
    def backward(ctx, d_o):
        q, k, v, m8, o, lse = ctx.saved_tensors
        d_o = d_o.contiguous()
        Lq, B, C = q.shape
        Lk = k.shape[0]
        dq, dk, dv = torch.empty_like(q), torch.empty_like(k), torch.empty_like(v)
        ws = _workspace(B, ctx.nheads, Lq, Lk, q.device)
        with torch.cuda.device(q.device):
            rc = _lib.load().pd_attn_bwd_d32(q.data_ptr(), k.data_ptr(), v.data_ptr(), m8.data_ptr() if m8 is not None else None,
                                             o.data_ptr(), d_o.data_ptr(), lse.data_ptr(), dq.data_ptr(), dk.data_ptr(), dv.data_ptr(),
                                             ws.data_ptr(), B, ctx.nheads, Lq, Lk, ctx.scale, _DT[q.dtype], _stream())
        _lib.check(rc)
        return dq, dk, dv, None, None, None


def masked_attention_d32(q, k, v, mask, nheads, scale=None):
    return MaskedAttention32.apply(q, k, v, mask, nheads, (32 ** -0.5) if scale is None else scale)
```

### partdistillation_amd/functions/declayer.py

```python
import ctypes

import torch

from .. import lib as _lib

C, FF = 256, 2048
bf16 = torch.bfloat16


def _stream():
    return _lib.current_stream()


def _p(t):
    return None if t is None else t.data_ptr()


def supported(C_, ff, cdt):
    return C_ == C and ff == FF and cdt == bf16


class _PackDesc(ctypes.Structure):
    _fields_ = [("src", ctypes.c_void_p), ("dst", ctypes.c_void_p), ("rows", ctypes.c_int32), ("cols", ctypes.c_int32), ("transpose", ctypes.c_int32)]


_PK = {}


def pack(weights, transpose=False):
    from .fused import PinnedRing
    key = (tuple((w.data_ptr(), tuple(w.shape)) for w in weights), bool(transpose))
    L = _lib.load()
    dev = weights[0].device
    hit = _PK.get(key)
    if hit is None:
        offs, total = [], 0
        for w in weights:
            assert w.dtype == bf16 and w.is_contiguous() and w.dim() == 2
            n, k = (w.shape[1], w.shape[0]) if transpose else w.shape
            assert n % 32 == 0 and k % 256 == 0, (n, k)
            offs.append(total)
            total += w.numel()
        tb = int(L.pd_dec_pack_table_bytes(len(weights)))
        hit = _PK[key] = ((_PackDesc * len(weights))(), offs, total, PinnedRing(tb, torch.uint8, pin=True), torch.empty(tb, dtype=torch.uint8, device=dev))
        if len(_PK) > 16:
            _PK.pop(next(iter(_PK)))
    descs, offs, total, ring, tdev = hit
    from .. import cmdbuf
    if cmdbuf.active() is not None:
        descs = (_PackDesc * len(weights))()
        tdev = torch.empty(tdev.numel(), dtype=torch.uint8, device=dev)
        for w in weights:
            cmdbuf.require_stable(w.data_ptr(), "weight to pack")
    buf = torch.empty(total, dtype=bf16, device=dev)
    base = buf.data_ptr()
    for d, w, o in zip(descs, weights, offs):
        d.src, d.dst, d.rows, d.cols, d.transpose = w.data_ptr(), base + 2 * o, w.shape[0], w.shape[1], int(bool(transpose))
    host = ring.acquire()
    rc = L.pd_dec_pack_grouped(descs, len(weights), host.data_ptr(), tdev.data_ptr(), _stream())
    ring.release()
    _lib.check(rc)
    return [buf[o:o + w.numel()] for w, o in zip(weights, offs)]


def workspace(R, dev):
    return torch.empty(int(_lib.load().pd_dec_workspace_bytes(int(R))), dtype=torch.uint8, device=dev)


def _e(shape, dtype, dev):
    return torch.empty(shape, dtype=dtype, device=dev)


def fwd_a(o, res, qpos, pos_div, w_o, b_o, ln_w, ln_b, eps, w_qkv, b_qkv):
    R, dev = o.shape[0], o.device
    z, y = _e((R, C), torch.float32, dev), _e((R, C), torch.float32, dev)
    stats = _e((2, R), torch.float32, dev)
    y_c, ypos_c, q, k, v = (_e((R, C), bf16, dev) for _ in range(5))
    _lib.check(_lib.load().pd_dec_fwd_a(o.data_ptr(), res.data_ptr(), qpos.data_ptr(), int(pos_div), w_o.data_ptr(), b_o.data_ptr(), ln_w.data_ptr(),
                                        ln_b.data_ptr(), float(eps), w_qkv.data_ptr(), b_qkv.data_ptr(), z.data_ptr(), stats.data_ptr(), y.data_ptr(),
                                        y_c.data_ptr(), ypos_c.data_ptr(), q.data_ptr(), k.data_ptr(), v.data_ptr(), R, _stream()))
    return z, stats, y, y_c, ypos_c, q, k, v


def fwd_b(o, res, qpos, pos_div, lay, dn_w, dn_b, mlp, q_next, eps, dec_out, ws=None):
    R, dev = res.shape[0], res.device
    layer, head = lay is not None, mlp is not None
    out = {}
    if layer:
        out.update(z2=_e((R, C), torch.float32, dev), stats2=_e((2, R), torch.float32, dev), y2_c=_e((R, C), bf16, dev), h=_e((R, FF), bf16, dev),
                   z3=_e((R, C), torch.float32, dev), stats3=_e((2, R), torch.float32, dev), y3=_e((R, C), torch.float32, dev))
    out.update(ypos_c=_e((R, C), bf16, dev), hstats=_e((2, R), torch.float32, dev))
    if head:
        out.update(ef=_e((pos_div, R // pos_div, C), bf16, dev), qc=_e((R, C), bf16, dev))
    g = out.get
    L = lay if layer else (None,) * 10
    M = mlp if head else (None,) * 6
    Qn = q_next if head else (None, None)
    _lib.check(_lib.load().pd_dec_fwd_b(_p(o), res.data_ptr(), qpos.data_ptr(), int(pos_div), *[_p(t) for t in L], dn_w.data_ptr(), dn_b.data_ptr(),
                                        *[_p(t) for t in M], _p(Qn[0]), _p(Qn[1]), float(eps), _p(g("z2")), _p(g("stats2")), _p(g("y2_c")), _p(g("h")),
                                        _p(g("z3")), _p(g("stats3")), _p(g("y3")), out["ypos_c"].data_ptr(), dec_out.data_ptr(), out["hstats"].data_ptr(),
                                        _p(g("ef")), _p(g("qc")), _p(ws), R, (1 if layer else 0) | (2 if head else 0), _stream()))
    return out


def bwd_b(dqc_next, wqT_next, d_out, d_res, y3, hstats, dn_w, dgb_dn, z3, stats3, ln3_w, dgb3, db3, pos_acc, pos_div, w2T, h, w1T, z2, stats2,
          ln2_w, dgb2, db2, woT, ws=None):
    R, dev = z3.shape[0], z3.device
    dz3_c, dz2_c, d_o = (_e((R, C), bf16, dev) for _ in range(3))
    dh = _e((R, FF), bf16, dev)
    dz2 = _e((R, C), torch.float32, dev)
    _lib.check(_lib.load().pd_dec_bwd_b(_p(dqc_next), _p(wqT_next), d_out.data_ptr(), _p(d_res), y3.data_ptr(), hstats.data_ptr(), dn_w.data_ptr(),
                                        dgb_dn.data_ptr(), z3.data_ptr(), stats3.data_ptr(), ln3_w.data_ptr(), dgb3.data_ptr(), db3.data_ptr(), _p(pos_acc),
                                        int(pos_div), w2T.data_ptr(), h.data_ptr(), w1T.data_ptr(), z2.data_ptr(), stats2.data_ptr(), ln2_w.data_ptr(),
                                        dgb2.data_ptr(), db2.data_ptr(), woT.data_ptr(), dz3_c.data_ptr(), dh.data_ptr(), dz2.data_ptr(), dz2_c.data_ptr(),
                                        d_o.data_ptr(), _p(ws), R, _stream()))
    return dz3_c, dh, dz2, dz2_c, d_o


def bwd_a(dq, dk, dv, wqkvT, dz_in, z, stats, ln_w, dgb, db, pos_acc, pos_div, woT):
    R, dev = z.shape[0], z.device
    dz1 = _e((R, C), torch.float32, dev)
    dz1_c, d_o = _e((R, C), bf16, dev), _e((R, C), bf16, dev)
    _lib.check(_lib.load().pd_dec_bwd_a(dq.data_ptr(), dk.data_ptr(), dv.data_ptr(), wqkvT.data_ptr(), dz_in.data_ptr(), z.data_ptr(), stats.data_ptr(),
                                        ln_w.data_ptr(), dgb.data_ptr(), db.data_ptr(), pos_acc.data_ptr(), int(pos_div), woT.data_ptr(), dz1.data_ptr(),
                                        dz1_c.data_ptr(), d_o.data_ptr(), R, _stream()))
    return dz1, dz1_c, d_o
```

### partdistillation_amd/functions/decoder_core.py

```python
from typing import List

import torch
from torch.autograd import Function

from .. import cmdbuf
from .. import lib as _lib
from . import rowwise as rw
from . import conv_bf16, igemm
from . import declayer as dl
from . import smallgemm as sg
from .attention import attn_bwd_raw, attn_fwd_raw


class DecoderSpec:

    def __init__(self, B, Q, C, nheads, num_layers, sizes, pos_tables, pooled, eps, cdt, num_levels=3):
        self.B, self.Q, self.C, self.H, self.L = B, Q, C, nheads, num_layers
        self.sizes, self.pos, self.pooled, self.eps, self.cdt, self.num_levels = sizes, pos_tables, pooled, eps, cdt, num_levels


import os

SMALL_M = int(os.environ.get("PD_SGEMM_MAX_M", "1024"))
SMALL_M_WGRAD = 1024


def _small(x, cdt, limit=None):
    return cdt == torch.bfloat16 and x.shape[0] <= (SMALL_M if limit is None else limit)


KV_IGEMM_ROWS = int(__import__("os").environ.get("PD_KV_IGEMM_ROWS", "4096"))


def _lin(x, w, b, relu=False):
    if _small(x, x.dtype) and w.shape[1] % 64 == 0:
        return sg.linear(x, w, b, relu)
    y = torch.addmm(b, x, w.t())
    return torch.relu_(y) if relu else y


def _lin_relu(x, w, b):
    return _lin(x, w, b, True)


def _dgrad(dy, w, relu_ref=None, out=None, accumulate=False):
    if _small(dy, dy.dtype) and w.shape[0] % 64 == 0:
        return sg.dgrad(dy, w, relu_ref, out, accumulate)
    if accumulate:
        out.addmm_(dy, w)
        dx = out
    else:
        dx = torch.mm(dy, w) if out is None else torch.mm(dy, w, out=out)
    if relu_ref is not None:
        rw.relu_bwd_colsum(dx, relu_ref, None)
    return dx


def _wgrad(dy, x, out=None, bias_acc=None, queue=None, big=None):
    if _small(dy, dy.dtype, SMALL_M_WGRAD):
        if queue is not None:
            return queue.add(dy, x, out, bias_acc)
        return sg.wgrad(dy, x, out, bias_acc)
    if big is not None and dy.dtype == torch.bfloat16 and dy.shape[1] % 8 == 0 and x.shape[1] % 8 == 0 and dy.is_contiguous() \
            and x.is_contiguous():
        dw = out if out is not None else torch.empty((dy.shape[1], x.shape[1]), dtype=torch.bfloat16, device=dy.device)
        big.append(conv_bf16.rows_entry(dy, x, dw, bias_acc))
        return dw
    dw = torch.mm(dy.t(), x) if out is None else torch.mm(dy.t(), x, out=out)
    if bias_acc is not None:
        rw.colsum_acc(dy, bias_acc)
    return dw


GROUP_WGRADS = True
MULTI_QKV = os.environ.get("PD_MULTI_QKV", "1") != "0"
FUSED_HEAD = os.environ.get("PD_FUSED_HEAD", "1") != "0"
KV_BATCH = os.environ.get("PD_DEC_KVBATCH", "1") != "0"
FUSED_LAYER = os.environ.get("PD_DEC_FUSED", "1") != "0"


class _Acc:

    def __init__(self):
        self.n, self.bias_n = 0, 0

    def take(self, n):
        off = self.n
        self.n += n
        return (off, n)


N_GLOBAL = 11
N_LAYER = 18


def _drop_backward_of(key, rec, cache):
    for k in [k for k in cache if k[0] == "bwd" and k[1] == id(rec)]:
        cache.pop(k)


_RECS = cmdbuf.LRU(24, _drop_backward_of)


def _rec_get(key):
    return _RECS.get(key)


def _flat_params(o):
    if isinstance(o, torch.Tensor):
        return [o]
    if isinstance(o, (list, tuple)):
        return [t for x in o for t in _flat_params(x)]
    return []


def _rec_put(key, rec):
    _RECS.put(key, rec)


class DecoderCore(Function):
    @staticmethod
    def forward(ctx, spec: DecoderSpec, *t):
        ctx.set_materialize_grads(False)
        B, Q, C, H, L, cdt = spec.B, spec.Q, spec.C, spec.H, spec.L, spec.cdt
        nl = spec.num_levels
        xs = t[:nl]
        g = t[nl:nl + N_GLOBAL]
        query_feat, query_embed, level_embed, dn_w, dn_b = g[:5]
        mlp = g[5:11]
        layers = [t[nl + N_GLOBAL + i * N_LAYER: nl + N_GLOBAL + (i + 1) * N_LAYER] for i in range(L)]
        R = Q * B
        qpos = query_embed.contiguous()
        tgt = query_feat.unsqueeze(1).expand(Q, B, C).reshape(R, C)
        tgtpos_c = (query_feat + query_embed).to(cdt).unsqueeze(1).expand(Q, B, C).reshape(R, C)
        fused_head = (FUSED_HEAD and cdt == torch.bfloat16 and C == 256 and all(tuple(mlp[j].shape) == (256, 256) for j in (0, 2, 4))
                      and all(mlp[j].is_contiguous() and mlp[j].dtype == torch.bfloat16 for j in range(6)))
        multi = MULTI_QKV and cdt == torch.bfloat16 and C <= 256 and C % 64 == 0
        pooled_ok = all(p_.dtype == torch.bfloat16 and p_.shape[2] % 8 == 0 and (p_.is_contiguous() or p_.transpose(1, 2).is_contiguous()) for p_ in spec.pooled)
        use_rec = (cmdbuf.usable() and xs[0].is_cuda and fused_head and multi and pooled_ok and any(ctx.needs_input_grad))
        fused_layer = (FUSED_LAYER and xs[0].is_cuda and fused_head and multi and pooled_ok and Q <= 1024 and igemm.supported(C, C) and
                       all(dl.supported(C, lay[12].shape[0], cdt) and tuple(lay[12].shape) == (dl.FF, C) and tuple(lay[14].shape) == (C, dl.FF) and
                           all(lay[j].dtype == torch.bfloat16 and lay[j].is_contiguous() for j in (0, 1, 2, 3, 6, 7, 8, 9, 12, 13, 14, 15)) and
                           all(lay[j].dtype == torch.float32 for j in (4, 5, 10, 11, 16, 17)) for lay in layers) and
                       dn_w.dtype == torch.float32 and query_embed.dtype == torch.float32)
        ctx.fused_layer = fused_layer
        flat_layers = [p_ for lay in layers for p_ in lay]
        if cmdbuf.DEBUG and not use_rec:
            import sys
            print("[cmdbuf] decoder forward runs eagerly:", dict(cuda=xs[0].is_cuda, fused_head=fused_head, multi=multi,
                  pooled=[(str(p_.dtype), p_.is_contiguous()) for p_ in spec.pooled], needs_grad=any(ctx.needs_input_grad)), file=sys.stderr, flush=True)
        if not use_rec:
            ctx.rec = None
            outs = DecoderCore._fwd_layers(spec, xs, qpos, tgt, tgtpos_c, level_embed, dn_w, dn_b, mlp, layers, fused_head, multi, fused_layer)
        else:
            consts = list(spec.pos[:nl]) + list(spec.pooled[:nl])
            head = list(xs) + [qpos, tgt, tgtpos_c] + consts
            params = [level_embed, dn_w, dn_b] + list(mlp) + flat_layers
            slots = head + params
            key = ("fwd", B, Q, C, H, L, nl, tuple(tuple(x.shape) for x in xs), params[0].data_ptr(), flat_layers[0].data_ptr(), str(xs[0].device),
                   _lib.current_stream(), fused_layer)
            rec = _rec_get(key)
# ... 92 lines not shown
            o, lse = attn_fwd_raw(q, k, v, None, B, H, scale)
            z, y, y_c, _, mean, rstd = rw.add_ln_fwd(_lin(o, sow, sob), tgt, snw, snb, spec.eps, c_dtype=cdt, want_yc=True)
            slf = (tgtpos_c, tgt_c, q, k, v, o, lse, z, mean, rstd)
            tgt, tgt_c = y, y_c
            h = _lin_relu(tgt_c, w1, b1)
            z, y, _, ypos_c, mean, rstd = rw.add_ln_fwd(_lin(h, w2, b2), tgt, fnw, fnb, spec.eps, c_dtype=cdt, pos=qpos,
                                                        pos_div=B, want_ypos=True)
            ffn = (tgt_c, h, z, mean, rstd, y)
            tgt, tgtpos_c = y, ypos_c
            saved.append((cross, slf, ffn))
            mask = head(i + 1, tgt, (i + 1) % nl if i + 1 < L else None)
        return dec_outs, tgt, saved, head_stats, mem, mempos

    @staticmethod
    def _mask_from_ef(spec, ef, lvl):
        B, Q = spec.B, spec.Q
        pooled = spec.pooled[lvl]
        pooled_t = pooled.transpose(1, 2)
        if pooled_t.is_contiguous() and sg.bmm_tn_supported(ef, pooled_t):
            return rw.attn_mask_u8(sg.bmm_tn(ef, pooled_t))
        logits = torch.empty((B, Q, pooled.shape[2]), dtype=torch.bfloat16, device=ef.device)
        for b in range(B):
            if pooled_t.is_contiguous():
                sg.linear(ef[b], pooled_t[b], None, False, out=logits[b])
            else:
                sg.dgrad(ef[b], pooled[b], out=logits[b])
        return rw.attn_mask_u8(logits)

    @staticmethod
    def _fwd_layers_fused(spec, xs, qpos, tgt, tgtpos_c, level_embed, dn_w, dn_b, mlp, layers):
        B, Q, C, H, L, cdt = spec.B, spec.Q, spec.C, spec.H, spec.L, spec.cdt
        nl = spec.num_levels
        R, scale = Q * B, 32 ** -0.5
        dev = xs[0].device
        if cmdbuf.active() is not None:
            tgt = rw.copy_d2d(torch.empty_like(tgt), tgt)
        mem, mempos = [], []
        for l in range(nl):
            m, mp = rw.mem_prep_fwd(xs[l], level_embed[l], spec.pos[l], cdt)
            mem.append(m), mempos.append(mp)
        dec_outs = torch.empty((L + 1, R, C), dtype=torch.float32, device=dev)
        saved, head_stats = [], []
        per = 6
        pk = dl.pack([w_ for lay in layers for w_ in (lay[0][:C], lay[2], lay[6], lay[8], lay[12], lay[14])] + [mlp[0], mlp[2], mlp[4]])
        mlp_p = [pk[per * L], mlp[1], pk[per * L + 1], mlp[3], pk[per * L + 2], mlp[5]]

        def qnext(i):
            return (pk[per * i], layers[i][1][:C])

        ws = dl.workspace(R, dev)
        Kb = Vb = None
        if KV_BATCH and cdt == torch.bfloat16 and C % 128 == 0:
            grp = [[i for i in range(L) if i % nl == l] for l in range(nl)]
            wk = [torch.empty((len(g_) * C, C), dtype=cdt, device=dev) for g_ in grp]
            wv = [torch.empty((len(g_) * C, C), dtype=cdt, device=dev) for g_ in grp]
            bk = [torch.empty(len(g_) * C, dtype=cdt, device=dev) for g_ in grp]
            bv = [torch.empty(len(g_) * C, dtype=cdt, device=dev) for g_ in grp]
            pairs = []
            for l, g_ in enumerate(grp):
                for j, i in enumerate(g_):
                    ciw, cib = layers[i][0], layers[i][1]
                    pairs += [(wk[l][j * C:(j + 1) * C], ciw[C:2 * C]), (wv[l][j * C:(j + 1) * C], ciw[2 * C:]),
                              (bk[l][j * C:(j + 1) * C], cib[C:2 * C]), (bv[l][j * C:(j + 1) * C], cib[2 * C:])]
            for a0 in range(0, len(pairs), rw.MAX_COPY_SEGS):
                rw.copy_segments(pairs[a0:a0 + rw.MAX_COPY_SEGS])
            Kb = [igemm.linear(mempos[l], wk[l], bk[l], out_col_slab=C) if grp[l] else None for l in range(nl)]
            Vb = [igemm.linear(mem[l], wv[l], bv[l], out_col_slab=C) if grp[l] else None for l in range(nl)]
        r = dl.fwd_b(None, tgt, qpos, B, None, dn_w, dn_b, mlp_p, qnext(0), spec.eps, dec_outs[0])
        head_stats.append((r["hstats"][0], r["hstats"][1]))
        mask = DecoderCore._mask_from_ef(spec, r["ef"], 0)
        tgtpos_c, qc = r["ypos_c"], r["qc"]
        for i in range(L):
            lvl = i % nl
            (ciw, cib, cow, cob, cnw, cnb, siw, sib, sow, sob, snw, snb, w1, b1, w2, b2, fnw, fnb) = layers[i]
            _, p_co, p_si, p_so, p_w1, p_w2 = pk[per * i:per * i + per]
            if Kb is not None:
                j = i // nl
                k, v = Kb[lvl][j], Vb[lvl][j]
            elif mem[lvl].shape[0] >= KV_IGEMM_ROWS:
                k = igemm.linear(mempos[lvl], ciw[C:2 * C], cib[C:2 * C])
                v = igemm.linear(mem[lvl], ciw[2 * C:], cib[2 * C:])
            else:
                k, v = sg.linear_multi([(mempos[lvl], ciw[C:2 * C], cib[C:2 * C]), (mem[lvl], ciw[2 * C:], cib[2 * C:])])
            o, lse = attn_fwd_raw(qc, k, v, mask, B, H, scale)
            z1, st1, y1, y1_c, y1pos_c, sq, sk, sv = dl.fwd_a(o, tgt, qpos, B, p_co, cob, cnw, cnb, spec.eps, p_si, sib)
            cross = (tgtpos_c, qc, k, v, mask, o, lse, z1, st1[0], st1[1])
            o_s, lse_s = attn_fwd_raw(sq, sk, sv, None, B, H, scale)
            slf = (y1pos_c, y1_c, sq, sk, sv, o_s, lse_s, None, None, None)
            last = i + 1 == L
            r = dl.fwd_b(o_s, y1, qpos, B, (p_so, sob, snw, snb, p_w1, b1, p_w2, b2, fnw, fnb), dn_w, dn_b, None if last else mlp_p,
                         None if last else qnext(i + 1), spec.eps, dec_outs[i + 1], ws)
            slf = slf[:7] + (r["z2"], r["stats2"][0], r["stats2"][1])
            ffn = (r["y2_c"], r["h"], r["z3"], r["stats3"][0], r["stats3"][1], r["y3"])
            saved.append((cross, slf, ffn))
            head_stats.append((r["hstats"][0], r["hstats"][1]))
            tgt, tgtpos_c = r["y3"], r["ypos_c"]
            if not last:
                qc = r["qc"]
                mask = DecoderCore._mask_from_ef(spec, r["ef"], (i + 1) % nl)
        return dec_outs, tgt, saved, head_stats, mem, mempos

    @staticmethod
    def backward(ctx, d_out, d_final):
        spec = ctx.spec
        B, Q, C, H, L, cdt = spec.B, spec.Q, spec.C, spec.H, spec.L, spec.cdt
        nl = spec.num_levels
        R = Q * B
        query_feat, query_embed, level_embed, dn_w, dn_b, mlp, layers = ctx.params
        dev = query_feat.device
        d_out = d_out.contiguous() if d_out is not None else torch.zeros((L + 1, R, C), dtype=torch.float32, device=dev)
        d_fin = d_final.contiguous() if d_final is not None else None
        need_x = tuple(bool(ctx.needs_input_grad[1 + l]) for l in range(nl))
        tgt0 = query_feat.unsqueeze(1).expand(Q, B, C).reshape(R, C)
        rec_f = getattr(ctx, "rec", None)
        args = (spec, ctx.saved, ctx.head_stats, ctx.mem, ctx.mempos, ctx.x_shapes, d_out, d_fin, tgt0, level_embed, dn_w, layers, getattr(ctx, "fused_layer", False))
        if rec_f is None:
            outs = DecoderCore._bwd_layers(*args)
        else:
            if rec_f.generation != ctx.rec_gen:
                raise RuntimeError("the fused decoder ran another forward before this backward: the recorded region's activation arena was "
                                   "overwritten (set PD_CMDBUF=0 for graphs that keep several forward passes alive)")
            flat_layers = [p_ for lay in layers for p_ in lay]
            head = [d_out] + ([d_fin] if d_fin is not None else []) + [tgt0]
            params = [level_embed, dn_w] + flat_layers
            slots = head + params
            key = ("bwd", id(rec_f), d_fin is not None)
            rec = _rec_get(key)
            if rec is None or not rec.matches(slots):
                rec = cmdbuf.Recording(slots, "decoder backward", stable=[rec_f], pinned=range(len(head), len(slots)))
                with rec:
                    outs = DecoderCore._bwd_layers(*args)
                    outs = outs[:-1] + (cmdbuf.Fresh([g_ for lay in outs[-1] for g_ in lay]),)
                outs = rec.finish(outs)
                _rec_put(key, rec)
            else:
                cmdbuf.unalias_grads(_flat_params(ctx.params), rec.owns)
                outs = rec.replay(slots)
            fl = outs[-1]
            outs = outs[:-1] + ([tuple(fl[6 * i:6 * i + 6]) for i in range(L)],)
        buf, slots_, dz0, d_res, d_pos_c, dtoks, d_level, wgrads = outs
        lay, n_bias, s_dnw, s_dnb, s_pos = slots_

        def A(s):
            return buf[s[0]:s[0] + s[1]]
        d_pos0 = d_pos_c.float().view(Q, B, C).sum(1)
        d_query_feat = (dz0 + d_res).view(Q, B, C).sum(1) + d_pos0
        d_query_embed = A(s_pos).view(Q, C) + d_pos0
        d_xs = [None] * nl
        for l in range(nl):
            if dtoks[l] is not None and need_x[l]:
                _, _, Hh, Ww = ctx.x_shapes[l]
                d_xs[l] = dtoks[l].view(B, Hh, Ww, C).permute(0, 3, 1, 2)
        bias_c = buf[:n_bias] if layers[0][1].dtype == torch.float32 else buf[:n_bias].to(layers[0][1].dtype)

        def Bc(s):
            return bias_c[s[0]:s[0] + s[1]]

        grads = [None]
        grads += d_xs
        grads += [d_query_feat, d_query_embed, d_level if rec_f is None else d_level.detach(), A(s_dnw), A(s_dnb)] + [None] * 6
        for i in range(L):
            g_ciw, g_cow, g_siw, g_sow, g_w1, g_w2 = wgrads[i]
            s_ = lay[i]
            grads += [g_ciw, Bc(s_["cib"]), g_cow, Bc(s_["cob"]), A(s_["cnw"]), A(s_["cnb"]),
                      g_siw, Bc(s_["sib"]), g_sow, Bc(s_["sob"]), A(s_["snw"]), A(s_["snb"]),
                      g_w1, Bc(s_["b1"]), g_w2, Bc(s_["b2"]), A(s_["fnw"]), A(s_["fnb"])]
        return tuple(grads)

    @staticmethod
    def _bwd_layers(spec, saved, head_stats, mem_f, mempos_f, x_shapes, d_out, d_final, tgt0, level_embed, dn_w, layers, fused_layer=False):
        B, Q, C, H, L, cdt = spec.B, spec.Q, spec.C, spec.H, spec.L, spec.cdt
        nl = spec.num_levels
        R, scale = Q * B, 32 ** -0.5
        dev = d_out.device
        acc = _Acc()
        lay = []
        for i in range(L):
            lay.append({"cib": acc.take(3 * C), "cob": acc.take(C), "sib": acc.take(3 * C), "sob": acc.take(C),
                        "b1": acc.take(layers[i][13].numel()), "b2": acc.take(C)})
        n_bias = acc.n
        for i in range(L):
            lay[i].update({"cnw": acc.take(C), "cnb": acc.take(C), "snw": acc.take(C), "snb": acc.take(C),
                           "fnw": acc.take(C), "fnb": acc.take(C)})
        s_dnw, s_dnb, s_pos = acc.take(C), acc.take(C), acc.take(Q * C)
        buf = torch.zeros(acc.n, dtype=torch.float32, device=dev)

        def A(s):
            return buf[s[0]:s[0] + s[1]]

        big_rows = cdt == torch.bfloat16 and any(not _small(m, cdt) for m in mem_f) and C % 64 == 0
        if big_rows:
            wts = igemm.transposed([layers[i][0][j * C:(j + 1) * C] for i in range(L) for j in (1, 2)])

        def dgrad_mem(dy, i, j, acc_into):
            w = layers[i][0][j * C:(j + 1) * C]
            if big_rows and not _small(dy, dy.dtype):
                return igemm.linear(dy, wts[2 * i + (j - 1)], res=acc_into)
            if acc_into is None:
                return _dgrad(dy, w)
            _dgrad(dy, w, out=acc_into, accumulate=True)
            return acc_into

        dmem: List = [None] * nl
        dmempos: List = [None] * nl
        wgrads = [None] * L
        wq = sg.WgradQueue() if GROUP_WGRADS else None
        big = [] if GROUP_WGRADS else None
        d_res = d_final
        d_pos_c = None
        if fused_layer:
            pkT = dl.pack([w_ for lay_ in layers for w_ in (lay_[0][:C], lay_[2], lay_[6], lay_[8], lay_[12], lay_[14])], transpose=True)
            ws = dl.workspace(R, dev)
            dq_next = None

            def A2(s0):
                return buf[s0[0]:s0[0] + 2 * s0[1]]
        for i in reversed(range(L)):
            lvl = i % nl
            (ciw, cib, cow, cob, cnw, cnb, siw, sib, sow, sob, snw, snb, w1, b1, w2, b2, fnw, fnb) = layers[i]
            cross, slf, ffn = saved[i]
            if fused_layer:
                cqT, coT, siT, soT, w1T, w2T = pkT[6 * i:6 * i + 6]
                hm, hr = head_stats[i + 1]
                x_c, h, z3, m3, r3, y3 = ffn
                tp_c, t_c, q, k, v, o, lse, z2, m2, r2 = slf
                dz3_c, dh, dz2, dz2_c, d_os = dl.bwd_b(dq_next, pkT[6 * (i + 1)] if dq_next is not None else None, d_out[i + 1], d_res, y3, hm, dn_w,
                                                       A2(s_dnw), z3, m3, fnw, A2(lay[i]["fnw"]), A(lay[i]["b2"]),
                                                       A(s_pos) if dq_next is not None else None, B, w2T, h, w1T, z2, m2, snw, A2(lay[i]["snw"]),
                                                       A(lay[i]["sob"]), soT, ws)
                g_w2 = _wgrad(dz3_c, h, queue=wq)
                g_w1 = _wgrad(dh, x_c, bias_acc=A(lay[i]["b1"]), queue=wq)
                g_sow = _wgrad(dz2_c, o, queue=wq)
                dq, dk, dv = attn_bwd_raw(q, k, v, None, o, d_os, lse, B, H, scale)
                g_siw = torch.empty_like(siw)
                sb = A(lay[i]["sib"])
                _wgrad(dq, tp_c, g_siw[:C], sb[:C], queue=wq)
                _wgrad(dk, tp_c, g_siw[C:2 * C], sb[C:2 * C], queue=wq)
                _wgrad(dv, t_c, g_siw[2 * C:], sb[2 * C:], queue=wq)
                tp_c, q, k, v, mask, o, lse, z1, m1, r1 = cross
                dz1, dz1_c, d_oc = dl.bwd_a(dq, dk, dv, siT, dz2, z1, m1, cnw, A2(lay[i]["cnw"]), A(lay[i]["cob"]), A(s_pos), B, coT)
                g_cow = _wgrad(dz1_c, o, queue=wq)
                dq, dk, dv = attn_bwd_raw(q, k, v, mask, o, d_oc, lse, B, H, scale)
                g_ciw = torch.empty_like(ciw)
                cb = A(lay[i]["cib"])
                _wgrad(dq, tp_c, g_ciw[:C], cb[:C], queue=wq)
                _wgrad(dk, mempos_f[lvl], g_ciw[C:2 * C], cb[C:2 * C], queue=wq, big=big)
                _wgrad(dv, mem_f[lvl], g_ciw[2 * C:], cb[2 * C:], queue=wq, big=big)
                dmempos[lvl] = dgrad_mem(dk, i, 1, dmempos[lvl])
                dmem[lvl] = dgrad_mem(dv, i, 2, dmem[lvl])
                dq_next = dq
                if i == 0:
                    d_pos_c = _dgrad(dq, ciw[:C])
                d_res = dz1
                wgrads[i] = (g_ciw, g_cow, g_siw, g_sow, g_w1, g_w2)
                continue
            hm, hr = head_stats[i + 1]
            dzh, _ = rw.add_ln_bwd(ffn[5], hm, hr, dn_w, dy=d_out[i + 1], dgamma=A(s_dnw), dbeta=A(s_dnb))
            x_c, h, z, mean, rstd, _ = ffn
            dz, dz_c = rw.add_ln_bwd(z, mean, rstd, fnw, dy=dzh, dy2=d_res, dypos_c=d_pos_c, dz_c_dtype=cdt,
                                     dgamma=A(lay[i]["fnw"]), dbeta=A(lay[i]["fnb"]), dbias=A(lay[i]["b2"]),
                                     dpos_acc=A(s_pos) if d_pos_c is not None else None, pos_div=B, out=dzh)
            g_w2 = _wgrad(dz_c, h, queue=wq)
            dh = _dgrad(dz_c, w2, relu_ref=h)
            g_w1 = _wgrad(dh, x_c, bias_acc=A(lay[i]["b1"]), queue=wq)
            dx_c = _dgrad(dh, w1)
            tp_c, t_c, q, k, v, o, lse, z, mean, rstd = slf
            dz, dz_c = rw.add_ln_bwd(z, mean, rstd, snw, dy=dz, dy_c=dx_c, dz_c_dtype=cdt, dgamma=A(lay[i]["snw"]),
                                     dbeta=A(lay[i]["snb"]), dbias=A(lay[i]["sob"]), out=dz)
            g_sow = _wgrad(dz_c, o, queue=wq)
            dq, dk, dv = attn_bwd_raw(q, k, v, None, o, _dgrad(dz_c, sow), lse, B, H, scale)
            g_siw = torch.empty_like(siw)
            sb = A(lay[i]["sib"])
            _wgrad(dq, tp_c, g_siw[:C], sb[:C], queue=wq)
            _wgrad(dk, tp_c, g_siw[C:2 * C], sb[C:2 * C], queue=wq)
            _wgrad(dv, t_c, g_siw[2 * C:], sb[2 * C:], queue=wq)
            d_tp = _dgrad(dq, siw[:C])
            _dgrad(dk, siw[C:2 * C], out=d_tp, accumulate=True)
            d_tc = _dgrad(dv, siw[2 * C:])
            tp_c, q, k, v, mask, o, lse, z, mean, rstd = cross
            dz, dz_c = rw.add_ln_bwd(z, mean, rstd, cnw, dy=dz, dy_c=d_tc, dypos_c=d_tp, dz_c_dtype=cdt,
                                     dgamma=A(lay[i]["cnw"]), dbeta=A(lay[i]["cnb"]), dbias=A(lay[i]["cob"]),
                                     dpos_acc=A(s_pos), pos_div=B, out=dz)
            g_cow = _wgrad(dz_c, o, queue=wq)
            dq, dk, dv = attn_bwd_raw(q, k, v, mask, o, _dgrad(dz_c, cow), lse, B, H, scale)
            g_ciw = torch.empty_like(ciw)
            cb = A(lay[i]["cib"])
            _wgrad(dq, tp_c, g_ciw[:C], cb[:C], queue=wq)
            _wgrad(dk, mempos_f[lvl], g_ciw[C:2 * C], cb[C:2 * C], queue=wq, big=big)
            _wgrad(dv, mem_f[lvl], g_ciw[2 * C:], cb[2 * C:], queue=wq, big=big)
            d_pos_c = _dgrad(dq, ciw[:C])
            dmempos[lvl] = dgrad_mem(dk, i, 1, dmempos[lvl])
            dmem[lvl] = dgrad_mem(dv, i, 2, dmem[lvl])
            d_res = dz
            wgrads[i] = (g_ciw, g_cow, g_siw, g_sow, g_w1, g_w2)

        hm, hr = head_stats[0]
        dz0, _ = rw.add_ln_bwd(tgt0, hm, hr, dn_w, dy=d_out[0], dgamma=A(s_dnw), dbeta=A(s_dnb))

        dtoks = [None] * nl
        d_level = torch.zeros_like(level_embed)
        use_colsum = level_embed.dtype == torch.float32 and C % 128 == 0
        for l in range(nl):
            _, _, Hh, Ww = x_shapes[l]
            if dmem[l] is None:
                continue
            dtok = rw.mem_prep_bwd(dmem[l], dmempos[l], B, Hh, Ww, C)
            if use_colsum and dtok.is_contiguous():
                rw.colsum_acc(dtok.view(-1, C), d_level[l])
            else:
                torch.sum(dtok.view(-1, C), dim=0, out=d_level[l])
            dtoks[l] = dtok
        if wq is not None:
            wq.run()
            conv_bf16.run_now(big)
        return buf, (lay, n_bias, s_dnw, s_dnb, s_pos), dz0, d_res, d_pos_c, dtoks, d_level, wgrads


def _ln_into(x_f32, gamma, beta, eps, y_out, cdt):
    rows, C = x_f32.shape
    from .. import lib as _lib
    y_c = torch.empty((rows, C), dtype=cdt, device=x_f32.device)
    stats = torch.empty((2, rows), dtype=torch.float32, device=x_f32.device)
    _lib.check(_lib.load().pd_add_layernorm_fwd(None, 0, x_f32.data_ptr(), gamma.data_ptr(), beta.data_ptr(), float(eps), None,
                                                y_out.data_ptr(), y_c.data_ptr(), None, 1, None, rw._DT[cdt], stats[0].data_ptr(),
                                                stats[1].data_ptr(), rows, C, rw._stream()))
    return None, y_out, y_c, None, stats[0], stats[1]
```

### partdistillation_amd/lib.py

```python
import ctypes
import os
import subprocess

_HERE = os.path.dirname(os.path.abspath(__file__))
LIB_PATH = os.environ.get("PD_LIB_PATH") or os.path.join(_HERE, "libpd_hip.so")
CSRC = os.path.join(_HERE, "csrc")

PD_F32, PD_F64, PD_BF16 = 0, 1, 2
ABI_VERSION = 40

_c_int, _c_vp = ctypes.c_int, ctypes.c_void_p

SIGNATURES = {
    "pd_msda_forward": (_c_int, [_c_vp] * 6 + [_c_int] * 9 + [_c_vp]),
    "pd_msda_backward": (_c_int, [_c_vp] * 9 + [_c_int] * 9 + [_c_vp]),
    "pd_msda_backward_last_gate": (_c_int, [_c_vp]),
    "pd_stem7x7_fwd": (_c_int, [_c_vp, _c_int] + [_c_vp] * 4 + [_c_int] * 4 + [_c_vp]),
    "pd_stem_wgrad_workspace_floats": (ctypes.c_int64, []),
    "pd_stem7x7_wgrad": (_c_int, [_c_vp, _c_int] + [_c_vp] * 4 + [_c_int, _c_vp] + [_c_int] * 4 + [_c_vp]),
    "pd_msda_fused_supported": (_c_int, [_c_int] * 7),
    "pd_msda_fused_forward": (_c_int, [_c_vp] * 4 + [_c_int] + [_c_vp] * 4 + [_c_int] * 7 + [_c_vp]),
    "pd_msda_fused_backward": (_c_int, [_c_vp] * 4 + [_c_int] + [_c_vp] * 6 + [_c_int, _c_vp, _c_vp] + [_c_int] * 7 + [_c_vp]),
    "pd_lsa_batched": (_c_int, [_c_vp] * 4 + [_c_int] * 3 + [_c_vp]),
    "pd_sumsq_accumulate": (_c_int, [_c_vp, ctypes.c_int64, _c_int, _c_vp, _c_vp]),
    "pd_adamw_clipped": (_c_int, [_c_vp] * 4 + [ctypes.c_int64, _c_int] + [ctypes.c_double] * 5 + [_c_int, _c_vp, ctypes.c_double, _c_vp, _c_vp]),
    "pd_gemm_tn_f32": (_c_int, [_c_vp] * 4 + [_c_int] * 7 + [_c_vp]),
    "pd_gemm_tn_f32x3": (_c_int, [_c_vp] * 4 + [_c_int] * 7 + [_c_vp]),
    "pd_gemm_wgrad_f16x2_takes_wide_tiles": (_c_int, [_c_int] * 2),
    "pd_gemm_wgrad_f16x2_ws_floats": (ctypes.c_int64, [_c_int] * 2),
    "pd_gemm_wgrad_f16x2_grouped_ws_floats": (ctypes.c_int64, [_c_vp, _c_int]),
    "pd_gemm_wgrad_acc_f16x2_ws": (_c_int, [_c_vp] * 7 + [ctypes.c_int64] + [_c_int] * 6 + [_c_vp]),
    "pd_gemm_wgrad_f16x2_grouped": (_c_int, [_c_vp, _c_int, _c_vp, _c_vp, _c_vp, ctypes.c_int64, _c_vp]),
    "pd_conv3x3_wgrad_nhwc_f16x2": (_c_int, [_c_vp] * 7 + [ctypes.c_int64] + [_c_int] * 5 + [_c_vp]),
    "pd_conv3x3_nhwc_f16x2": (_c_int, [_c_vp] * 7 + [_c_int] * 5 + [_c_vp]),
    "pd_gemm_tn_f16x2_which": (_c_int, [_c_int] * 6),
    "pd_gemm_tn_f16x2_bits_words": (ctypes.c_int64, [_c_int] * 2),
    "pd_gemm_tn_f16x2": (_c_int, [_c_vp] * 9 + [_c_int] * 7 + [_c_vp]),
    "pd_gemm_tn_f16x2_bf16out": (_c_int, [_c_vp] * 6 + [_c_int] * 6 + [_c_vp]),
    "pd_cast_bf16_f32_amax": (_c_int, [_c_vp, _c_int, _c_int, _c_vp, _c_vp, _c_vp]),
    "pd_row_amax_f32": (_c_int, [_c_vp, _c_int, _c_int, _c_int, _c_vp, _c_vp]),
    "pd_gemm_tn_f32x3_relumask": (_c_int, [_c_vp] * 5 + [_c_int] * 6 + [_c_vp]),
    "pd_gemm_tn_f32x3_relu_bits": (_c_int, [_c_vp] * 5 + [_c_int] * 6 + [_c_vp]),
    "pd_gemm_tn_f32x3_relu_bits_words": (ctypes.c_int64, [_c_int] * 2),
    "pd_split3_bf16": (_c_int, [_c_vp, _c_int, _c_int, _c_int, _c_int, _c_vp, _c_vp]),
    "pd_gemm_tn_f32x3_pre": (_c_int, [_c_vp] * 6 + [_c_int] * 6 + [_c_vp]),
    "pd_gemm_wgrad_f32": (_c_int, [_c_vp] * 4 + [_c_int] * 6 + [_c_vp]),
    "pd_gemm_wgrad_acc_f32": (_c_int, [_c_vp] * 4 + [_c_int] * 6 + [_c_vp]),
    "pd_conv3x3_nhwc_f32x3": (_c_int, [_c_vp] * 4 + [_c_int] * 5 + [_c_vp]),
    "pd_gemm_wgrad_acc_f32x3": (_c_int, [_c_vp] * 4 + [_c_int] * 6 + [_c_vp]),
    "pd_conv3x3_wgrad_nhwc_f32x3": (_c_int, [_c_vp] * 5 + [ctypes.c_int64] + [_c_int] * 5 + [_c_vp]),
    "pd_gemm_wgrad_f32x3_ws_floats": (ctypes.c_int64, [_c_int] * 2),
    "pd_gemm_wgrad_f32x3_grouped_table_bytes": (ctypes.c_int64, [_c_int]),
    "pd_gemm_wgrad_f32x3_grouped_ws_floats": (ctypes.c_int64, [_c_vp, _c_int]),
    "pd_gemm_wgrad_f32x3_grouped": (_c_int, [_c_vp, _c_int, _c_vp, _c_vp, _c_vp, ctypes.c_int64, _c_vp]),
    "pd_gemm_wgrad_acc_f32x3_ws": (_c_int, [_c_vp] * 5 + [ctypes.c_int64] + [_c_int] * 6 + [_c_vp]),
    "pd_adamw_clipped_shadow": (_c_int, [_c_vp] * 5 + [ctypes.c_int64] + [ctypes.c_double] * 5 + [_c_int, _c_vp, ctypes.c_double, _c_vp, _c_vp]),
    "pd_conv_bf16_supported": (_c_int, [_c_int] * 5),
    "pd_conv_bf16_fwd": (_c_int, [_c_vp] * 6 + [_c_int] * 11 + [_c_vp]),
    "pd_conv_bf16_wgrad_workspace_floats": (ctypes.c_int64, [_c_int] * 6),
    "pd_conv_bf16_wgrad": (_c_int, [_c_vp] * 4 + [ctypes.c_int64] + [_c_int] * 10 + [_c_vp]),
    "pd_conv_bf16_wgrad_grouped_table_bytes": (ctypes.c_int64, [_c_int]),
    "pd_conv_bf16_wgrad_grouped_workspace_floats": (ctypes.c_int64, [_c_vp, _c_int]),
    "pd_conv_bf16_wgrad_grouped": (_c_int, [_c_vp, _c_int, _c_vp, _c_vp, _c_vp, ctypes.c_int64, _c_vp]),
    "pd_conv_bf16_dgrad": (_c_int, [_c_vp] * 4 + [_c_int] * 10 + [_c_vp]),
    "pd_maxpool3s2_fwd_bf16": (_c_int, [_c_vp] * 3 + [_c_int] * 4 + [_c_vp]),
    "pd_maxpool3s2_bwd_bf16": (_c_int, [_c_vp] * 3 + [_c_int] * 4 + [_c_vp]),
    "pd_affine_act_fwd_bf16": (_c_int, [_c_vp] * 5 + [ctypes.c_int64, _c_int, _c_int, _c_vp]),
    "pd_affine_act_bwd_bf16": (_c_int, [_c_vp] * 5 + [ctypes.c_int64, _c_int, _c_int, _c_vp]),
    "pd_affine_act_bwd2_bf16": (_c_int, [_c_vp] * 6 + [ctypes.c_int64, _c_int, _c_int, _c_vp]),
    "pd_multi_gather_sumsq": (_c_int, [_c_vp] * 8 + [_c_int, _c_int, _c_vp]),
    "pd_attn_workspace_floats": (ctypes.c_int64, [_c_int] * 4),
    "pd_attn_fwd_d32": (_c_int, [_c_vp] * 7 + [_c_int] * 4 + [ctypes.c_float, _c_int, _c_vp]),
    "pd_attn_bwd_d32": (_c_int, [_c_vp] * 11 + [_c_int] * 4 + [ctypes.c_float, _c_int, _c_vp]),
    "pd_attn_fwd_d32_ld": (_c_int, [_c_vp] * 7 + [_c_int] * 4 + [ctypes.c_float, _c_int, _c_int, _c_vp]),
    "pd_attn_bwd_d32_ld": (_c_int, [_c_vp] * 11 + [_c_int] * 4 + [ctypes.c_float, _c_int, _c_int, _c_vp]),
    "pd_nc_sums_f32": (_c_int, [_c_vp] * 6 + [_c_int] * 5 + [_c_vp]),
    "pd_nc_affine_f32": (_c_int, [_c_vp] * 4 + [_c_int] * 4 + [_c_vp]),
    "pd_nc_affine_amax_f32": (_c_int, [_c_vp] * 5 + [_c_int] * 4 + [_c_vp]),
    "pd_nc_affine2_amax_f32": (_c_int, [_c_vp] * 8 + [_c_int] * 4 + [_c_vp]),
    "pd_upsample_add_amax_nhwc_f32": (_c_int, [_c_vp, ctypes.c_int64] + [_c_vp] * 3 + [_c_int] * 6 + [_c_vp]),
    "pd_nc_affine2_f32": (_c_int, [_c_vp] * 7 + [_c_int] * 4 + [_c_vp]),
    "pd_add_layernorm_fwd": (_c_int, [_c_vp, _c_int, _c_vp, _c_vp, _c_vp, ctypes.c_float, _c_vp, _c_vp, _c_vp, _c_vp, _c_int, _c_vp,
                                      _c_int, _c_vp, _c_vp, _c_int, _c_int, _c_vp]),
    "pd_add_layernorm_bwd": (_c_int, [_c_vp] * 4 + [_c_int] + [_c_vp] * 6 + [_c_int] + [_c_vp] * 4 + [_c_int] * 3 + [_c_vp]),
    "pd_add_layernorm_fwd_amax": (_c_int, [_c_vp, _c_int, _c_vp, _c_vp, _c_vp, ctypes.c_float, _c_vp, _c_vp, _c_vp, _c_vp, _c_int, _c_vp,
                                           _c_int, _c_vp, _c_vp, _c_vp, _c_vp, _c_int, _c_int, _c_vp]),
    "pd_add_layernorm_bwd_amax": (_c_int, [_c_vp] * 4 + [_c_int] + [_c_vp] * 6 + [_c_int] + [_c_vp] * 4 + [_c_int] + [_c_vp] + [_c_int] * 2 + [_c_vp]),
    "pd_colsum_acc": (_c_int, [_c_vp, _c_int, _c_int, _c_int, _c_vp, _c_vp]),
    "pd_relu_bwd_colsum": (_c_int, [_c_vp, _c_vp, _c_int, _c_int, _c_int, _c_vp, _c_vp]),
    "pd_mem_prep_fwd": (_c_int, [_c_vp, ctypes.c_int64, _c_vp, _c_vp, _c_vp, _c_vp, _c_int, _c_int, _c_int, _c_int, _c_vp]),
    "pd_mem_prep_bwd": (_c_int, [_c_vp, _c_vp, _c_int, _c_vp, ctypes.c_int64, _c_int, _c_int, _c_int, _c_vp]),
    "pd_attn_mask_u8": (_c_int, [_c_vp, _c_int, _c_int, _c_int, _c_vp, _c_vp]),
    "pd_add_rows_amax_f32": (_c_int, [_c_vp] * 6 + [_c_int, _c_int, _c_vp]),
    "pd_sum3_sum2_f32": (_c_int, [_c_vp] * 6 + [ctypes.c_int64, _c_vp]),
    "pd_transpose_batched_f32": (_c_int, [_c_vp, _c_int, _c_vp]),
    "pd_normalize_u8_nhwc": (_c_int, [_c_vp, _c_int, _c_int, _c_int, _c_vp, _c_vp, _c_vp, _c_vp]),
    "pd_resize_bilinear_nhwc_f32": (_c_int, [_c_vp] + [_c_int] * 4 + [_c_vp] * 3 + [_c_int, _c_int, _c_vp]),
    "pd_matcher_point_terms": (_c_int, [_c_vp, _c_int, _c_int, _c_int, _c_vp, _c_vp, _c_vp, _c_vp, _c_vp]),
    "pd_match_point_logits": (_c_int, [_c_vp] * 4 + [_c_int] * 7 + [_c_vp]),
    "pd_matcher_costs": (_c_int, [_c_vp, _c_int, _c_vp] + [ctypes.c_int64] * 3 + [_c_vp] * 3 + [_c_int] * 6 + [ctypes.c_float] * 3 + [_c_vp]),
    "pd_mask_point_losses_fwd": (_c_int, [_c_vp] * 5 + [_c_int, _c_int, _c_vp]),
    "pd_mask_point_losses_bwd": (_c_int, [_c_vp] * 6 + [_c_int, _c_int, _c_vp]),
    "pd_uncertain_points": (_c_int, [_c_vp] * 4 + [_c_int] * 4 + [_c_vp]),
    "pd_point_sample_u8": (_c_int, [_c_vp] * 4 + [_c_int] * 5 + [_c_vp]),
    "pd_skinny_linear_fwd": (_c_int, [_c_vp] * 3 + [_c_int, _c_vp] + [_c_int] * 3 + [_c_vp]),
    "pd_skinny_linear_partial_floats": (ctypes.c_int64, [_c_int] * 3),
    "pd_skinny_linear_bwd": (_c_int, [_c_vp, _c_vp, _c_int, _c_vp, _c_vp, _c_vp, _c_int, _c_vp, _c_vp, _c_vp] + [_c_int] * 4 + [_c_vp]),
    "pd_loss_vectors_fwd": (_c_int, [_c_vp, ctypes.c_int64, ctypes.c_int64] + [_c_vp] * 9 + [_c_int] * 5 + [_c_vp]),
    "pd_loss_vectors_bwd": (_c_int, [_c_vp, ctypes.c_int64, ctypes.c_int64] + [_c_vp] * 10 + [_c_int] * 5 + [_c_vp]),
    "pd_pair_logits_fwd": (_c_int, [_c_vp] * 5 + [_c_int] * 4 + [_c_vp]),
    "pd_pair_logits_bwd_tok": (_c_int, [_c_vp] * 5 + [_c_int] * 4 + [_c_vp]),
    "pd_pair_logits_workspace_floats": (ctypes.c_int64, [_c_int] * 3),
    "pd_pair_logits_bwd_rows": (_c_int, [_c_vp] * 6 + [_c_int] * 4 + [_c_vp]),
    "pd_msda_prep_fwd": (_c_int, [_c_vp] * 6 + [ctypes.c_int64] + [_c_int] * 5 + [_c_vp]),
    "pd_msda_prep_bwd_amax": (_c_int, [_c_vp] * 7 + [ctypes.c_int64] + [_c_int] * 5 + [_c_vp]),
    "pd_msda_forward_amax": (_c_int, [_c_vp] * 7 + [_c_int] * 9 + [_c_vp]),
    "pd_msda_prep_bwd": (_c_int, [_c_vp] * 6 + [ctypes.c_int64] + [_c_int] * 5 + [_c_vp]),
    "pd_sgemm_tn_batched_bf16": (_c_int, [_c_vp] * 3 + [_c_int] * 7 + [ctypes.c_int64] * 3 + [_c_vp]),
    "pd_sgemm_tn_multi_bf16": (_c_int, [_c_vp, _c_int, _c_int, _c_vp]),
    "pd_decoder_head_bf16": (_c_int, [_c_vp] * 3 + [ctypes.c_float] + [_c_vp] * 10 + [_c_int] * 4 + [_c_vp]),
    "pd_dec_fwd_a": (_c_int, [_c_vp] * 3 + [_c_int] + [_c_vp] * 4 + [ctypes.c_float] + [_c_vp] * 10 + [_c_int] + [_c_vp]),
    "pd_dec_fwd_b": (_c_int, [_c_vp] * 3 + [_c_int] + [_c_vp] * 20 + [ctypes.c_float] + [_c_vp] * 13 + [_c_int] * 2 + [_c_vp]),
    "pd_dec_bwd_b": (_c_int, [_c_vp] * 14 + [_c_int] + [_c_vp] * 15 + [_c_int] + [_c_vp]),
    "pd_dec_split": (_c_int, []),
    "pd_dec_workspace_bytes": (ctypes.c_int64, [_c_int]),
    "pd_dec_pack_table_bytes": (ctypes.c_int64, [_c_int]),
    "pd_dec_pack_grouped": (_c_int, [_c_vp, _c_int, _c_vp, _c_vp, _c_vp]),
    "pd_dec_bwd_a": (_c_int, [_c_vp] * 11 + [_c_int] + [_c_vp] * 4 + [_c_int] + [_c_vp]),
    "pd_sgemm_split_workspace_floats": (ctypes.c_int64, [_c_int] * 3),
    "pd_sgemm_split_tickets": (ctypes.c_int64, [_c_int] * 2),
    "pd_sgemm_tn_splitk_bf16": (_c_int, [_c_vp] * 5 + [ctypes.c_int64, _c_vp] + [_c_int] * 7 + [_c_vp]),
    "pd_sgemm_nn_splitn_bf16": (_c_int, [_c_vp] * 5 + [ctypes.c_int64, _c_vp] + [_c_int] * 7 + [_c_vp]),
    "pd_sgemm_tn_bf16": (_c_int, [_c_vp] * 4 + [_c_int] * 7 + [_c_vp]),
    "pd_sgemm_nn_bf16": (_c_int, [_c_vp] * 4 + [_c_int] * 7 + [_c_vp]),
    "pd_sgemm_wgrad_bf16": (_c_int, [_c_vp] * 4 + [_c_int] * 6 + [_c_vp]),
    "pd_gn_coeffs_fwd": (_c_int, [_c_vp] * 3 + [_c_int] * 4 + [ctypes.c_float] + [_c_vp] * 6),
    "pd_gn_coeffs_bwd": (_c_int, [_c_vp] * 4 + [_c_int] * 4 + [_c_vp] * 6),
    "pd_point_sample_nhwc_f32": (_c_int, [_c_vp] * 3 + [_c_int] * 5 + [_c_vp]),
    "pd_point_sample_nhwc_f32_bf16": (_c_int, [_c_vp] * 3 + [_c_int] * 5 + [_c_vp]),
    "pd_point_sample_planar_f32": (_c_int, [_c_vp] * 3 + [_c_int] * 5 + [_c_vp]),
    "pd_point_sample_planar_bwd_needs_zero": (_c_int, [_c_int] * 3),
    "pd_point_sample_planar_bwd_needs_zero_n": (_c_int, [_c_int] * 4),
    "pd_point_sample_planar_bwd_f32": (_c_int, [_c_vp] * 3 + [_c_int] * 5 + [_c_vp]),
    "pd_upsample_add_nhwc_f32": (_c_int, [_c_vp, ctypes.c_int64] + [_c_vp] * 2 + [_c_int] * 6 + [_c_vp]),
    "pd_upsample2x_bwd_nhwc_f32": (_c_int, [_c_vp] * 2 + [_c_int] * 4 + [_c_vp]),
    "pd_scores_argmax_u8": (_c_int, [_c_vp] * 3 + [_c_int] * 7 + [_c_vp]),
    "pd_kmeans_assign": (_c_int, [_c_vp, _c_vp, _c_int] + [_c_vp] * 7 + [_c_int, _c_int, _c_vp]),
    "pd_kmeans_assign_partial": (_c_int, [_c_vp, _c_vp, _c_int] + [_c_vp] * 7 + [_c_int, _c_int, _c_vp]),
    "pd_kmeans_reduce": (_c_int, [_c_vp] * 6 + [_c_int] * 3 + [_c_vp]),
    "pd_kmeans_reduce_update_scratch_floats": (ctypes.c_int64, [_c_int] * 3),
    "pd_kmeans_reduce_update": (_c_int, [_c_vp] * 11 + [_c_int] * 3 + [_c_vp]),
    "pd_kmeans_assign_bounded": (_c_int, [_c_vp, _c_vp, _c_int] + [_c_vp] * 11 + [_c_int, _c_int, _c_vp]),
    "pd_kmeans_reduce_update_shift": (_c_int, [_c_vp] * 12 + [_c_int] * 3 + [_c_vp]),
    "pd_kmeans_update": (_c_int, [_c_vp] * 8 + [_c_int] * 3 + [_c_vp]),
    "pd_mask_assign": (_c_int, [_c_vp] * 6 + [_c_int] * 7 + [_c_vp]),
    "pd_window_attn_fwd_w12": (_c_int, [_c_vp] * 6 + [_c_int] * 3 + [ctypes.c_float, _c_vp, _c_vp, _c_int, _c_vp]),
    "pd_window_attn_bwd_w12": (_c_int, [_c_vp] * 9 + [_c_int] * 3 + [ctypes.c_float, _c_vp, _c_vp, _c_int, _c_vp]),
    "pd_layernorm_rows_f32_fwd": (_c_int, [_c_vp] * 3 + [ctypes.c_float] + [_c_vp] * 3 + [ctypes.c_int64, _c_int, _c_vp]),
    "pd_layernorm_rows_f32_bwd": (_c_int, [_c_vp] * 8 + [ctypes.c_int64, _c_int, _c_vp]),
    "pd_swin_tail_ln_fwd": (_c_int, [_c_vp] * 3 + [_c_int] + [_c_vp] * 2 + [ctypes.c_float] + [_c_vp] * 4 + [ctypes.c_int64, _c_int, _c_vp]),
    "pd_swin_tail_ln_bwd": (_c_int, [_c_vp] * 7 + [_c_int] + [_c_vp] * 4 + [ctypes.c_int64, _c_int, _c_vp]),
    "pd_swin_merge_ln_fwd": (_c_int, [_c_vp] * 3 + [ctypes.c_float] + [_c_vp] * 3 + [_c_int] * 4 + [_c_vp]),
    "pd_swin_merge_ln_bwd": (_c_int, [_c_vp] * 8 + [_c_int] * 4 + [_c_vp]),
    "pd_swin_ln_fwd": (_c_int, [_c_vp, _c_vp, _c_vp, _c_int, _c_vp, _c_vp, _c_vp, ctypes.c_float, _c_vp, _c_vp, _c_vp, _c_int, _c_vp,
                                _c_int, _c_vp, _c_vp, _c_int, _c_int, _c_int, _c_vp, _c_vp, _c_int, _c_vp]),
    "pd_swin_ln_bwd": (_c_int, [_c_vp, _c_vp, _c_int, _c_vp, _c_vp, _c_vp, _c_vp, _c_vp, _c_vp, _c_vp, _c_vp, _c_int, _c_vp, _c_vp,
                                _c_int, _c_vp, _c_vp, _c_int, _c_int, _c_int, _c_vp, _c_vp, _c_int, _c_int, ctypes.c_int64, _c_vp]),
    "pd_resample_rows_u8": (_c_int, [_c_vp] + [_c_int] * 6 + [_c_vp] * 3 + [_c_int, _c_int, _c_vp, _c_vp]),
    "pd_resample_cols_u8": (_c_int, [_c_vp] + [_c_int] * 3 + [_c_vp] * 3 + [_c_int] * 5 + [_c_vp, _c_vp]),
    "pd_rle_sample_u8": (_c_int, [_c_vp, _c_vp] + [_c_int] * 4 + [_c_vp, _c_vp] + [_c_int] * 3 + [_c_vp, _c_vp, _c_vp]),
    "pd_sgemm_wgrad_grouped_table_bytes": (ctypes.c_int64, [_c_int]),
    "pd_sgemm_wgrad_grouped_bf16": (_c_int, [_c_vp, _c_int, _c_vp, _c_vp, _c_vp]),
    "pd_sgemm_wgrad_split_workspace": (ctypes.c_int64, [_c_int] * 3),
    "pd_sgemm_wgrad_split_bf16": (_c_int, [_c_vp] * 5 + [_c_int] * 6 + [_c_vp]),
    "pd_igemm_bf16_supported": (_c_int, [_c_int] * 5),
    "pd_igemm_bf16_workspace_bytes": (ctypes.c_int64, [_c_vp]),
    "pd_igemm_bf16": (_c_int, [_c_vp, _c_vp, ctypes.c_int64, _c_vp]),
    "pd_igemm_bf16_time": (_c_int, [_c_vp, _c_vp, ctypes.c_int64, _c_int, _c_vp, _c_vp]),
    "pd_igemm_bf16_seq_workspace_bytes": (ctypes.c_int64, [_c_vp, _c_int]),
    "pd_igemm_bf16_seq": (_c_int, [_c_vp, _c_int, _c_vp, ctypes.c_int64, _c_vp]),
    "pd_wgrad_bf16_workspace_bytes": (ctypes.c_int64, [_c_vp]),
    "pd_wgrad_bf16": (_c_int, [_c_vp, _c_vp, ctypes.c_int64, _c_vp]),
    "pd_wgrad_bf16_seq_workspace_bytes": (ctypes.c_int64, [_c_vp, _c_int]),
    "pd_wgrad_bf16_seq": (_c_int, [_c_vp, _c_int, _c_vp, ctypes.c_int64, _c_vp]),
    "pd_wgrad_bf16_time": (_c_int, [_c_vp, _c_vp, ctypes.c_int64, _c_int, _c_vp, _c_vp]),
    "pd_mx8_quantize_bf16": (_c_int, [_c_vp, ctypes.c_int64, _c_int, ctypes.c_int64, _c_int, _c_vp, _c_vp, _c_vp]),
    "pd_mx8_quantize_table_bytes": (ctypes.c_int64, [_c_int]),
    "pd_mx8_quantize_grouped": (_c_int, [_c_vp, _c_int, _c_int, _c_vp, _c_vp, _c_vp]),
    "pd_mx8_gemm": (_c_int, [_c_vp, _c_vp]),
    "pd_mx8_gemm_supported": (_c_int, [_c_int] * 3),
    "pd_filter_transpose_table_bytes": (ctypes.c_int64, [_c_int]),
    "pd_filter_transpose_grouped": (_c_int, [_c_vp, _c_int, _c_vp, _c_vp, _c_vp]),
    "pd_eval_table_bytes": (ctypes.c_int64, [_c_int]),
    "pd_eval_pack_grouped": (_c_int, [_c_vp, _c_int, _c_vp, _c_vp, _c_vp]),
    "pd_eval_intersect_grouped": (_c_int, [_c_vp, _c_int, _c_vp, _c_vp, _c_vp]),
    "pd_eval_confusion_grouped": (_c_int, [_c_vp, _c_int, _c_int, _c_vp, _c_int, _c_vp, _c_vp, _c_vp]),
    "pd_eval_recall_grouped": (_c_int, [_c_vp, _c_int] + [_c_vp] * 6),
    "pd_grouping_table_bytes": (ctypes.c_int64, [_c_int]),
    "pd_scores_argmax_resized_u8": (_c_int, [_c_vp, _c_int, _c_vp, _c_vp, _c_vp]),
    "pd_masks_resize_u8": (_c_int, [_c_vp, _c_int, _c_vp, _c_vp, _c_vp]),
    "pd_cmd_fn_index": (_c_int, [ctypes.c_char_p]),
    "pd_cmd_fn_nargs": (_c_int, [_c_int]),
    "pd_cmd_replay": (_c_int, [_c_vp, _c_int, _c_vp, _c_int, _c_vp]),
    "pd_memset_async": (_c_int, [_c_vp, _c_int, ctypes.c_int64, _c_vp]),
    "pd_memcpy_d2d_async": (_c_int, [_c_vp, _c_vp, ctypes.c_int64, _c_vp]),
    "pd_copy_segments": (_c_int, [_c_vp, _c_int, _c_vp]),
# ... 65 lines not shown
```

Measured before the change: 112.1.

## Fold split-K attention combine and dq reduction into decoder layer kernels

Adds 'parts' variants of the cross-attention forward and backward that leave per-chunk partial outputs (max/sum/out, and dq slabs) unmerged. The merge or sum is then done inside the tile-load stage of the following fused decoder-layer kernels (fwd_a and bwd_b). This removes the separate combine and dq-reduce launches and the round trip of the merged tensor through memory. In exchange, each tile of the consumer kernel redoes the merge reads, and the layout coupling between the attention and decoder kernels grows. The path is on by default behind an environment flag.

```diff
diff --git a/include/pd_attention.h b/include/pd_attention.h
--- a/include/pd_attention.h
+++ b/include/pd_attention.h
@@ -23,6 +23,14 @@
                        const float *lse, void *dq, void *dk, void *dv, float *workspace, int B, int H, int Lq, int Lk,
                        float scale, int dtype, int ld_kv, void *stream);
 
+int pd_attn_fwd_splits(int B, int H, int Lq, int Lk, int dtype);
+int pd_attn_bwd_splits(int B, int H, int Lq, int Lk, int dtype);
+int pd_attn_fwd_parts_d32_ld(const void *q, const void *k, const void *v, const uint8_t *mask, float *workspace, int B, int H, int Lq, int Lk,
+                             float scale, int dtype, int ld_kv, void *stream);
+int pd_attn_bwd_parts_d32_ld(const void *q, const void *k, const void *v, const uint8_t *mask, const void *o, const void *d_o,
+                             const float *lse, void *dk, void *dv, float *workspace, int B, int H, int Lq, int Lk, float scale, int dtype,
+                             int ld_kv, void *stream);
+
 #ifdef __cplusplus
 }
 #endif
diff --git a/include/pd_declayer.h b/include/pd_declayer.h
--- a/include/pd_declayer.h
+++ b/include/pd_declayer.h
@@ -22,6 +22,10 @@
                  const float *ln_b, float eps, const void *w_qkv, const void *b_qkv, float *z, float *stats, float *y, void *y_c,
                  void *ypos_c, void *q, void *k, void *v, int R, void *stream);
 
+int pd_dec_fwd_a_parts(const float *parts, int nsplit, void *o_out, float *lse_out, const float *res, const float *qpos, int pos_div,
+                       const void *w_o, const void *b_o, const float *ln_w, const float *ln_b, float eps, const void *w_qkv, const void *b_qkv,
+                       float *z, float *stats, float *y, void *y_c, void *ypos_c, void *q, void *k, void *v, int R, void *stream);
+
 int pd_dec_fwd_b(const void *o, const float *res, const float *qpos, int pos_div, const void *w_o, const void *b_o, const float *ln2_w,
                  const float *ln2_b, const void *w_1, const void *b_1, const void *w_2, const void *b_2, const float *ln3_w,
                  const float *ln3_b, const float *dn_w, const float *dn_b, const void *m0_w, const void *m0_b, const void *m1_w,
@@ -35,6 +39,12 @@
                  const float *ln2_w, float *dgb2, float *db2, const void *woT, void *dz3_c, void *dh, float *dz2, void *dz2_c, void *d_o,
                  void *workspace, int R, void *stream);
 
+int pd_dec_bwd_b_slabs(const float *dq_slabs, int nsplit, void *dq_out, const void *wqT_next, const float *d_out, const float *d_res,
+                       const float *y3, const float *hstats, const float *dn_w, float *dgb_dn, const float *z3, const float *stats3,
+                       const float *ln3_w, float *dgb3, float *db3, float *pos_acc, int pos_div, const void *w2T, const void *h, const void *w1T,
+                       const float *z2, const float *stats2, const float *ln2_w, float *dgb2, float *db2, const void *woT, void *dz3_c, void *dh,
+                       float *dz2, void *dz2_c, void *d_o, void *workspace, int R, void *stream);
+
 int pd_dec_bwd_a(const void *dq, const void *dk, const void *dv, const void *wqkvT, const float *dz_in, const float *z, const float *stats,
                  const float *ln_w, float *dgb, float *db, float *pos_acc, int pos_div, const void *woT, float *dz1, void *dz1_c, void *d_o,
                  int R, void *stream);
diff --git a/partdistillation_amd/csrc/attention.hip b/partdistillation_amd/csrc/attention.hip
--- a/partdistillation_amd/csrc/attention.hip
+++ b/partdistillation_amd/csrc/attention.hip
@@ -198,15 +198,15 @@
 #pragma unroll
       for (int u = 0; u < 8; ++u) {
         const float w = __expf(s8[u].x - M);
-        L += w * s8[u].y;
-        acc += w * o8[u];
+        L = fmaf(w, s8[u].y, L);
+        acc = fmaf(w, o8[u], acc);
       }
     }
     for (; c < nchunk; ++c) {
       const float2 sv = ml[(int64_t)c * Lq];
       const float w = __expf(sv.x - M);
-      L += w * sv.y;
-      acc += w * po[(int64_t)c * Lq * D];
+      L = fmaf(w, sv.y, L);
+      acc = fmaf(w, po[(int64_t)c * Lq * D], acc);
     }
   }
   const float outv = L > 0.f ? acc / L : 0.f;
@@ -724,14 +724,26 @@
   return (n1 > n2 ? n1 : n2) + 64;
 }
 
+extern "C" int pd_attn_fwd_splits(int B, int H, int Lq, int Lk, int dtype)
+{
+  if (!(dtype == PD_BF16 && Lq > 0 && Lq <= MQ && Lk > 0 && B > 0 && H > 0 && !g_pd_dbg_attn_scalar)) return 0;
+  return nchunks(Lk, mfma_fwd_chunk(B, H, Lk));
+}
+
+extern "C" int pd_attn_bwd_splits(int B, int H, int Lq, int Lk, int dtype)
+{
+  if (!(dtype == PD_BF16 && Lq > 0 && Lq <= MQ && Lk > 0 && B > 0 && H > 0 && !g_pd_dbg_attn_scalar)) return 0;
+  return nchunks(Lk, mfma_bwd_chunk(B, H, Lk));
+}
+
 extern "C" int pd_attn_fwd_d32(const void *q, const void *k, const void *v, const uint8_t *mask, void *o, float *lse,
                                float *workspace, int B, int H, int Lq, int Lk, float scale, int dtype, void *stream_)
 {
   return pd_attn_fwd_d32_ld(q, k, v, mask, o, lse, workspace, B, H, Lq, Lk, scale, dtype, H * D, stream_);
 }
 
-extern "C" int pd_attn_fwd_d32_ld(const void *q, const void *k, const void *v, const uint8_t *mask, void *o, float *lse,
-                                  float *workspace, int B, int H, int Lq, int Lk, float scale, int dtype, int ld_kv, void *stream_)
+static int attn_fwd_impl(const void *q, const void *k, const void *v, const uint8_t *mask, void *o, float *lse,
+                         float *workspace, int B, int H, int Lq, int Lk, float scale, int dtype, int ld_kv, void *stream_, bool parts)
 {
   int rc = check(q, k, v, B, H, Lq, Lk, dtype, "pd_attn_fwd_d32");
   if (rc) return rc;
@@ -739,7 +751,9 @@
   if (ld_kv != H * D && !(dtype == PD_BF16 && Lq <= MQ && Lk > 0 && !g_pd_dbg_attn_scalar))
     return pd_set_error(PD_ERR_INVALID_ARG, "pd_attn_fwd_d32_ld: strided k / v only on the matrix-core path (bf16, <= %d queries)", MQ);
   if (B * Lq == 0) return PD_OK;
-  if (!o || !lse || !workspace) return pd_set_error(PD_ERR_INVALID_ARG, "pd_attn_fwd_d32: null output");
+  if (parts && pd_attn_fwd_splits(B, H, Lq, Lk, dtype) < 2)
+    return pd_set_error(PD_ERR_INVALID_ARG, "pd_attn_fwd_parts_d32_ld: one split (or not the matrix-core path): nothing to leave unmerged");
+  if ((!parts && (!o || !lse)) || !workspace) return pd_set_error(PD_ERR_INVALID_ARG, "pd_attn_fwd_d32: null output");
   hipStream_t s = (hipStream_t)stream_;
   if (dtype == PD_BF16 && Lq <= MQ && Lk > 0 && !g_pd_dbg_attn_scalar) {
     const int kc = mfma_fwd_chunk(B, H, Lk), nc = nchunks(Lk, kc);
@@ -748,7 +762,7 @@
                                  mask, (bf16_t *)o, lse, part_o, part_ml, B, H, Lq, Lk, scale, nc, ld_kv, kc);
     else hipLaunchKernelGGL(attn_fwd_mfma<false>, dim3(nc, H, B), dim3(256), 0, s, (const bf16_t *)q, (const bf16_t *)k, (const bf16_t *)v,
                             mask, (bf16_t *)o, lse, part_o, part_ml, B, H, Lq, Lk, scale, nc, ld_kv, kc);
-    if (nc > 1) hipLaunchKernelGGL(attn_fwd_combine<bf16_t>, dim3((B * H * Lq + 7) / 8), dim3(256), 0, s, part_o, part_ml, (bf16_t *)o, lse, B, H, Lq, nc);
+    if (nc > 1 && !parts) hipLaunchKernelGGL(attn_fwd_combine<bf16_t>, dim3((B * H * Lq + 7) / 8), dim3(256), 0, s, part_o, part_ml, (bf16_t *)o, lse, B, H, Lq, nc);
     return pd_check_launch("pd_attn_fwd_d32");
   }
   const int nc = nchunks(Lk, KC_FWD);
@@ -769,6 +783,18 @@
   return pd_check_launch("pd_attn_fwd_d32");
 }
 
+extern "C" int pd_attn_fwd_d32_ld(const void *q, const void *k, const void *v, const uint8_t *mask, void *o, float *lse,
+                                  float *workspace, int B, int H, int Lq, int Lk, float scale, int dtype, int ld_kv, void *stream_)
+{
+  return attn_fwd_impl(q, k, v, mask, o, lse, workspace, B, H, Lq, Lk, scale, dtype, ld_kv, stream_, false);
+}
+
+extern "C" int pd_attn_fwd_parts_d32_ld(const void *q, const void *k, const void *v, const uint8_t *mask, float *workspace, int B, int H,
+                                        int Lq, int Lk, float scale, int dtype, int ld_kv, void *stream_)
+{
+  return attn_fwd_impl(q, k, v, mask, nullptr, nullptr, workspace, B, H, Lq, Lk, scale, dtype, ld_kv, stream_, true);
+}
+
 extern "C" int pd_attn_bwd_d32(const void *q, const void *k, const void *v, const uint8_t *mask, const void *o, const void *d_o,
                                const float *lse, void *dq, void *dk, void *dv, float *workspace, int B, int H, int Lq,
                                int Lk, float scale, int dtype, void *stream_)
@@ -776,9 +802,9 @@
   return pd_attn_bwd_d32_ld(q, k, v, mask, o, d_o, lse, dq, dk, dv, workspace, B, H, Lq, Lk, scale, dtype, H * D, stream_);
 }
 
-extern "C" int pd_attn_bwd_d32_ld(const void *q, const void *k, const void *v, const uint8_t *mask, const void *o, const void *d_o,
-                                  const float *lse, void *dq, void *dk, void *dv, float *workspace, int B, int H, int Lq,
-                                  int Lk, float scale, int dtype, int ld_kv, void *stream_)
+static int attn_bwd_impl(const void *q, const void *k, const void *v, const uint8_t *mask, const void *o, const void *d_o,
+                         const float *lse, void *dq, void *dk, void *dv, float *workspace, int B, int H, int Lq,
+                         int Lk, float scale, int dtype, int ld_kv, void *stream_, bool parts)
 {
   int rc = check(q, k, v, B, H, Lq, Lk, dtype, "pd_attn_bwd_d32");
   if (rc) return rc;
@@ -786,7 +812,9 @@
   if (ld_kv != H * D && !(dtype == PD_BF16 && Lq <= MQ && !g_pd_dbg_attn_scalar))
     return pd_set_error(PD_ERR_INVALID_ARG, "pd_attn_bwd_d32_ld: strided k / v only on the matrix-core path (bf16, <= %d queries)", MQ);
   if (B * Lq * Lk == 0) return PD_OK;
-  if (!o || !d_o || !lse || !dq || !dk || !dv || !workspace) return pd_set_error(PD_ERR_INVALID_ARG, "pd_attn_bwd_d32: null pointer");
+  if (parts && pd_attn_bwd_splits(B, H, Lq, Lk, dtype) < 2)
+    return pd_set_error(PD_ERR_INVALID_ARG, "pd_attn_bwd_parts_d32_ld: one split (or not the matrix-core path): no slabs to leave");
+  if (!o || !d_o || !lse || (!parts && !dq) || !dk || !dv || !workspace) return pd_set_error(PD_ERR_INVALID_ARG, "pd_attn_bwd_d32: null pointer");
   hipStream_t s = (hipStream_t)stream_;
   const int groups = B * H * Lq;
   if (dtype == PD_BF16 && Lq <= MQ && !g_pd_dbg_attn_scalar) {
@@ -797,7 +825,7 @@
     else hipLaunchKernelGGL(attn_bwd_mfma<false>, dim3(nc, H, B), dim3(256), 0, s, (const bf16_t *)q, (const bf16_t *)k, (const bf16_t *)v,
                             mask, (const bf16_t *)o, (const bf16_t *)d_o, lse, workspace, (bf16_t *)dq, (bf16_t *)dk, (bf16_t *)dv,
                             B, H, Lq, Lk, scale, nc, kc, ld_kv);
-    if (nc > 1) hipLaunchKernelGGL(attn_bwd_dq_reduce<bf16_t>, dim3((groups + 7) / 8), dim3(256), 0, s, workspace, (bf16_t *)dq, B, H, Lq, nc);
+    if (nc > 1 && !parts) hipLaunchKernelGGL(attn_bwd_dq_reduce<bf16_t>, dim3((groups + 7) / 8), dim3(256), 0, s, workspace, (bf16_t *)dq, B, H, Lq, nc);
     return pd_check_launch("pd_attn_bwd_d32");
   }
   const int nc = nchunks(Lk, KC_DQ);
@@ -818,3 +846,17 @@
   }
   return pd_check_launch("pd_attn_bwd_d32");
 }
+
+extern "C" int pd_attn_bwd_d32_ld(const void *q, const void *k, const void *v, const uint8_t *mask, const void *o, const void *d_o,
+                                  const float *lse, void *dq, void *dk, void *dv, float *workspace, int B, int H, int Lq,
+                                  int Lk, float scale, int dtype, int ld_kv, void *stream_)
+{
+  return attn_bwd_impl(q, k, v, mask, o, d_o, lse, dq, dk, dv, workspace, B, H, Lq, Lk, scale, dtype, ld_kv, stream_, false);
+}
+
+extern "C" int pd_attn_bwd_parts_d32_ld(const void *q, const void *k, const void *v, const uint8_t *mask, const void *o, const void *d_o,
+                                        const float *lse, void *dk, void *dv, float *workspace, int B, int H, int Lq, int Lk, float scale,
+                                        int dtype, int ld_kv, void *stream_)
+{
+  return attn_bwd_impl(q, k, v, mask, o, d_o, lse, nullptr, dk, dv, workspace, B, H, Lq, Lk, scale, dtype, ld_kv, stream_, true);
+}
diff --git a/partdistillation_amd/csrc/cmdbuf.hip b/partdistillation_amd/csrc/cmdbuf.hip
--- a/partdistillation_amd/csrc/cmdbuf.hip
+++ b/partdistillation_amd/csrc/cmdbuf.hip
@@ -121,6 +121,10 @@
   PD_E(pd_copy_segments),
   PD_E(pd_attn_fwd_d32_ld),
   PD_E(pd_attn_bwd_d32_ld),
+  PD_E(pd_attn_fwd_parts_d32_ld),
+  PD_E(pd_attn_bwd_parts_d32_ld),
+  PD_E(pd_dec_fwd_a_parts),
+  PD_E(pd_dec_bwd_b_slabs),
   PD_E(pd_match_point_logits),
   PD_E(pd_swin_merge_ln_fwd),
   PD_E(pd_swin_tail_ln_fwd),
diff --git a/partdistillation_amd/csrc/common.hip b/partdistillation_amd/csrc/common.hip
--- a/partdistillation_amd/csrc/common.hip
+++ b/partdistillation_amd/csrc/common.hip
@@ -27,7 +27,7 @@
 }
 
 extern "C" const char *pd_last_error(void) { return g_err; }
-extern "C" int pd_abi_version(void) { return 40; }
+extern "C" int pd_abi_version(void) { return 41; }
 
 extern int g_pd_dbg_atomic_scope;
 extern int g_pd_dbg_force_generic;
diff --git a/partdistillation_amd/csrc/declayer.hip b/partdistillation_amd/csrc/declayer.hip
--- a/partdistillation_amd/csrc/declayer.hip
+++ b/partdistillation_amd/csrc/declayer.hip
@@ -1,4 +1,5 @@
 #include <hip/hip_runtime.h>
+#include <math.h>
 #include <stdint.h>
 #include <stdlib.h>
 
@@ -189,11 +190,99 @@
   return s;
 }
 
+constexpr int HD = 32, NH = C / HD;
+__device__ __forceinline__ void tile_in_merge(bf16_t *dst, const float *__restrict__ parts, int ns, bf16_t *__restrict__ o_out,
+                                              float *__restrict__ lse_out, int B, int r0, int R, int tid)
+{
+  const int row = tid >> 5, col = (tid & 31) * 8, m = min(r0 + row, R - 1);
+  const int Lq = R / B, qi = m / B, b = m - qi * B, h = col >> 5;
+  const size_t bh = (size_t)b * NH + h, cs = (size_t)Lq;
+  const float2 *ml = reinterpret_cast<const float2 *>(parts + (size_t)B * NH * ns * Lq * HD) + bh * ns * Lq + qi;
+  const float *po = parts + (bh * ns * Lq + qi) * HD + (col & 31);
+  float M = -INFINITY;
+  int c = 0;
+  for (; c + 8 <= ns; c += 8) {
+    float m8[8];
+#pragma unroll
+    for (int u = 0; u < 8; ++u) m8[u] = ml[(c + u) * cs].x;
+#pragma unroll
+    for (int u = 0; u < 8; ++u) M = fmaxf(M, m8[u]);
+  }
+  for (; c < ns; ++c) M = fmaxf(M, ml[c * cs].x);
+  float L = 0.f, acc[8];
+#pragma unroll
+  for (int j = 0; j < 8; ++j) acc[j] = 0.f;
+  if (M != -INFINITY) {
+    c = 0;
+    for (; c + 8 <= ns; c += 8) {
+      float2 s8[8];
+      float4 a8[8], b8[8];
+#pragma unroll
+      for (int u = 0; u < 8; ++u) { s8[u] = ml[(c + u) * cs]; a8[u] = ld4(po + (c + u) * cs * HD); b8[u] = ld4(po + (c + u) * cs * HD + 4); }
+#pragma unroll
+      for (int u = 0; u < 8; ++u) {
+        const float w = __expf(s8[u].x - M);
+        L = fmaf(w, s8[u].y, L);
+        acc[0] = fmaf(w, a8[u].x, acc[0]); acc[1] = fmaf(w, a8[u].y, acc[1]); acc[2] = fmaf(w, a8[u].z, acc[2]); acc[3] = fmaf(w, a8[u].w, acc[3]);
+        acc[4] = fmaf(w, b8[u].x, acc[4]); acc[5] = fmaf(w, b8[u].y, acc[5]); acc[6] = fmaf(w, b8[u].z, acc[6]); acc[7] = fmaf(w, b8[u].w, acc[7]);
+      }
+    }
+    for (; c < ns; ++c) {
+      const float2 sv = ml[c * cs];
+      const float4 av = ld4(po + c * cs * HD), bv = ld4(po + c * cs * HD + 4);
+      const float w = __expf(sv.x - M);
+      L = fmaf(w, sv.y, L);
+      acc[0] = fmaf(w, av.x, acc[0]); acc[1] = fmaf(w, av.y, acc[1]); acc[2] = fmaf(w, av.z, acc[2]); acc[3] = fmaf(w, av.w, acc[3]);
+      acc[4] = fmaf(w, bv.x, acc[4]); acc[5] = fmaf(w, bv.y, acc[5]); acc[6] = fmaf(w, bv.z, acc[6]); acc[7] = fmaf(w, bv.w, acc[7]);
+    }
+  }
+  float o[8];
+#pragma unroll
+  for (int j = 0; j < 8; ++j) o[j] = L > 0.f ? acc[j] / L : 0.f;
+  const uint4 v = make_uint4(pk_bf16(o[0], o[1]), pk_bf16(o[2], o[3]), pk_bf16(o[4], o[5]), pk_bf16(o[6], o[7]));
+  *reinterpret_cast<uint4 *>(dst + row * PA + col) = v;
+  if (r0 + row < R) {
+    *reinterpret_cast<uint4 *>(o_out + (size_t)m * C + col) = v;
+    if ((tid & 3) == 0) lse_out[bh * Lq + qi] = L > 0.f ? M + __logf(L) : -INFINITY;
+  }
+}
+__device__ __forceinline__ void tile_in_sum(bf16_t *dst, const float *__restrict__ slabs, int ns, bf16_t *__restrict__ dq_out, int B, int r0,
+                                            int R, int tid)
+{
+  const int row = tid >> 5, col = (tid & 31) * 8, m = min(r0 + row, R - 1);
+  const int Lq = R / B, qi = m / B, b = m - qi * B, h = col >> 5;
+  const size_t cs = (size_t)Lq * HD;
+  const float *ps = slabs + (((size_t)b * NH + h) * ns * Lq + qi) * HD + (col & 31);
+  float acc[8];
+#pragma unroll
+  for (int j = 0; j < 8; ++j) acc[j] = 0.f;
+  int c = 0;
+  for (; c + 8 <= ns; c += 8) {
+    float4 a8[8], b8[8];
+#pragma unroll
+    for (int u = 0; u < 8; ++u) { a8[u] = ld4(ps + (c + u) * cs); b8[u] = ld4(ps + (c + u) * cs + 4); }
+#pragma unroll
+    for (int u = 0; u < 8; ++u) {
+      acc[0] += a8[u].x; acc[1] += a8[u].y; acc[2] += a8[u].z; acc[3] += a8[u].w;
+      acc[4] += b8[u].x; acc[5] += b8[u].y; acc[6] += b8[u].z; acc[7] += b8[u].w;
+    }
+  }
+  for (; c < ns; ++c) {
+    const float4 av = ld4(ps + c * cs), bv = ld4(ps + c * cs + 4);
+    acc[0] += av.x; acc[1] += av.y; acc[2] += av.z; acc[3] += av.w;
+    acc[4] += bv.x; acc[5] += bv.y; acc[6] += bv.z; acc[7] += bv.w;
+  }
+  const uint4 v = make_uint4(pk_bf16(acc[0], acc[1]), pk_bf16(acc[2], acc[3]), pk_bf16(acc[4], acc[5]), pk_bf16(acc[6], acc[7]));
+  *reinterpret_cast<uint4 *>(dst + row * PA + col) = v;
+  if (dq_out && r0 + row < R) *reinterpret_cast<uint4 *>(dq_out + (size_t)m * C + col) = v;
+}
+
 struct FwdA {
   const bf16_t *o; const float *res, *qpos; int pos_div;
   const bf16_t *w_o, *b_o; const float *ln_w, *ln_b; float eps;
   const bf16_t *w_qkv, *b_qkv;
   float *z, *stats, *y; bf16_t *y_c, *ypos_c, *q, *k, *v; int R;
+  const float *parts; int nsplit; bf16_t *o_out; float *lse_out;
 };
 
 __global__ __launch_bounds__(NTH) void dec_fwd_a(const FwdA a)
@@ -212,7 +301,8 @@
   auto bp = [&](int b) { return b == 0 ? a.w_o + (size_t)wave * BLK : a.w_qkv + (size_t)((b - 1) * 8 + wave) * BLK; };
   WHalf w[4];
   PD_HP(0); PD_HP(1); PD_HP(2);
-  tile_in(X0, a.o, r0, R, tid);
+  if (a.parts) tile_in_merge(X0, a.parts, a.nsplit, a.o_out, a.lse_out, a.pos_div, r0, R, tid);
+  else tile_in(X0, a.o, r0, R, tid);
   lds_copy_bf16(Bs, a.b_o, C, tid);
   lds_copy_bf16(Bs + C, a.b_qkv, 3 * C, tid);
   lds_copy_f32(Ls, a.ln_w, C, tid);
@@ -448,6 +538,7 @@
   const float *z3, *stats3, *ln3_w; float *dgb3, *db3, *pos_acc; int pos_div;
   const bf16_t *w2T, *h, *w1T; const float *z2, *stats2, *ln2_w; float *dgb2, *db2; const bf16_t *woT;
   bf16_t *dz3_c, *dh; float *dz2; bf16_t *dz2_c, *d_o; int R; float *slabs, *rows; int nsplit;
+  const float *dq_slabs; int dq_ns; bf16_t *dq_out;
 };
 
 template <int P, int PART, bool NXT>
@@ -480,7 +571,10 @@
   f32x4 acc[2];
   lds_copy_f32(Ls + 2 * C, a.ln2_w, C, tid);
   if (PART != 2) {
-  if (NXT) tile_in(X0, a.dqc_next, r0, R, tid);
+  if (NXT) {
+    if (a.dq_slabs) tile_in_sum(X0, a.dq_slabs, a.dq_ns, p == 0 ? a.dq_out : nullptr, a.pos_div, r0, R, tid);
+    else tile_in(X0, a.dqc_next, r0, R, tid);
+  }
 #pragma unroll
   for (int i = 0; i < HW * RB / 8 / NTH; ++i) {
     const int idx = i * NTH + tid, row = idx / (HW / 8), col = (idx % (HW / 8)) * 8;
@@ -794,7 +888,7 @@
 template <int P>
 int launch_bwd_b_split(const BwdB &a, hipStream_t s)
 {
-  const int rc = a.dqc_next ? launch_bwd_b<P, 1, true>(a, s) : launch_bwd_b<P, 1, false>(a, s);
+  const int rc = (a.dqc_next || a.dq_slabs) ? launch_bwd_b<P, 1, true>(a, s) : launch_bwd_b<P, 1, false>(a, s);
   if (rc != PD_OK) return rc;
   return launch_bwd_b<1, 2, false>(a, s);
 }
@@ -825,19 +919,39 @@
   return pd_check_launch("pd_dec_pack_grouped");
 }
 
-extern "C" int pd_dec_fwd_a(const void *o, const float *res, const float *qpos, int pos_div, const void *w_o, const void *b_o, const float *ln_w,
-                            const float *ln_b, float eps, const void *w_qkv, const void *b_qkv, float *z, float *stats, float *y, void *y_c,
-                            void *ypos_c, void *q, void *k, void *v, int R, void *stream)
-{
-  if (!o || !res || !qpos || !w_o || !b_o || !ln_w || !ln_b || !w_qkv || !b_qkv || !z || !stats || !y || !y_c || !ypos_c || !q || !k || !v)
+static int dec_fwd_a_impl(const void *o, const float *parts, int nsplit, void *o_out, float *lse_out, const float *res, const float *qpos, int pos_div,
+                          const void *w_o, const void *b_o, const float *ln_w, const float *ln_b, float eps, const void *w_qkv, const void *b_qkv, float *z,
+                          float *stats, float *y, void *y_c, void *ypos_c, void *q, void *k, void *v, int R, void *stream)
+{
+  if (parts && (!o_out || !lse_out || nsplit < 2 || pos_div <= 0 || R % pos_div))
+    return pd_set_error(PD_ERR_INVALID_ARG, "pd_dec_fwd_a_parts: %d splits (>= 2), R = %d rows of %d images, o / lse outputs required", nsplit, R, pos_div);
+  if ((!o && !parts) || !res || !qpos || !w_o || !b_o || !ln_w || !ln_b || !w_qkv || !b_qkv || !z || !stats || !y || !y_c || !ypos_c || !q || !k || !v)
     return pd_set_error(PD_ERR_INVALID_ARG, "pd_dec_fwd_a: null pointer");
   if (R <= 0 || pos_div <= 0) return pd_set_error(PD_ERR_INVALID_ARG, "pd_dec_fwd_a: R = %d, pos_div = %d", R, pos_div);
   static int ok = allow_smem(dec_fwd_a, kSmemFwdA, "pd_dec_fwd_a");
   if (ok != PD_OK) return ok;
   FwdA a{(const bf16_t *)o, res, qpos, pos_div, (const bf16_t *)w_o, (const bf16_t *)b_o, ln_w, ln_b, eps, (const bf16_t *)w_qkv, (const bf16_t *)b_qkv,
-         z, stats, y, (bf16_t *)y_c, (bf16_t *)ypos_c, (bf16_t *)q, (bf16_t *)k, (bf16_t *)v, R};
+         z, stats, y, (bf16_t *)y_c, (bf16_t *)ypos_c, (bf16_t *)q, (bf16_t *)k, (bf16_t *)v, R, parts, nsplit, (bf16_t *)o_out, lse_out};
   hipLaunchKernelGGL(dec_fwd_a, dim3((R + RB - 1) / RB), dim3(NTH), kSmemFwdA, (hipStream_t)stream, a);
   return pd_check_launch("pd_dec_fwd_a");
+}
+
+extern "C" int pd_dec_fwd_a(const void *o, const float *res, const float *qpos, int pos_div, const void *w_o, const void *b_o, const float *ln_w,
+                            const float *ln_b, float eps, const void *w_qkv, const void *b_qkv, float *z, float *stats, float *y, void *y_c,
+                            void *ypos_c, void *q, void *k, void *v, int R, void *stream)
+{
+  return dec_fwd_a_impl(o, nullptr, 0, nullptr, nullptr, res, qpos, pos_div, w_o, b_o, ln_w, ln_b, eps, w_qkv, b_qkv, z, stats, y, y_c, ypos_c, q, k, v, R,
+                        stream);
+}
+
+extern "C" int pd_dec_fwd_a_parts(const float *parts, int nsplit, void *o_out, float *lse_out, const float *res, const float *qpos, int pos_div,
+                                  const void *w_o, const void *b_o, const float *ln_w, const float *ln_b, float eps, const void *w_qkv,
+                                  const void *b_qkv, float *z, float *stats, float *y, void *y_c, void *ypos_c, void *q, void *k, void *v, int R,
+                                  void *stream)
+{
+  if (!parts) return pd_set_error(PD_ERR_INVALID_ARG, "pd_dec_fwd_a_parts: null pointer");
+  return dec_fwd_a_impl(nullptr, parts, nsplit, o_out, lse_out, res, qpos, pos_div, w_o, b_o, ln_w, ln_b, eps, w_qkv, b_qkv, z, stats, y, y_c, ypos_c, q, k,
+                        v, R, stream);
 }
 
 extern "C" int pd_dec_fwd_b(const void *o, const float *res, const float *qpos, int pos_div, const void *w_o, const void *b_o, const float *ln2_w,
@@ -871,28 +985,53 @@
   }
 }
 
+static int dec_bwd_b_impl(const void *dqc_next, const float *dq_slabs, int dq_ns, void *dq_out, const void *wqT_next, const float *d_out, const float *d_res,
+                          const float *y3, const float *hstats, const float *dn_w, float *dgb_dn, const float *z3, const float *stats3, const float *ln3_w,
+                          float *dgb3, float *db3, float *pos_acc, int pos_div, const void *w2T, const void *h, const void *w1T, const float *z2,
+                          const float *stats2, const float *ln2_w, float *dgb2, float *db2, const void *woT, void *dz3_c, void *dh, float *dz2, void *dz2_c,
+                          void *d_o, void *workspace, int R, void *stream)
+{
+  if (dq_slabs && (dq_ns < 2 || pos_div <= 0 || R % pos_div))
+    return pd_set_error(PD_ERR_INVALID_ARG, "pd_dec_bwd_b_slabs: %d splits (>= 2), R = %d rows of %d images", dq_ns, R, pos_div);
+  if (!d_out || !y3 || !hstats || !dn_w || !dgb_dn || !z3 || !stats3 || !ln3_w || !dgb3 || !db3 || !w2T || !h || !w1T || !z2 || !stats2 || !ln2_w ||
+      !dgb2 || !db2 || !woT || !dz3_c || !dh || !dz2 || !dz2_c || !d_o)
+    return pd_set_error(PD_ERR_INVALID_ARG, "pd_dec_bwd_b: null pointer");
+  const bool nxt = dqc_next || dq_slabs;
+  if (nxt != (wqT_next != nullptr) || (nxt && !pos_acc)) return pd_set_error(PD_ERR_INVALID_ARG, "pd_dec_bwd_b: next-layer operands");
+  if (R <= 0 || pos_div <= 0) return pd_set_error(PD_ERR_INVALID_ARG, "pd_dec_bwd_b: R = %d, pos_div = %d", R, pos_div);
+  BwdB a{(const bf16_t *)dqc_next, (const bf16_t *)wqT_next, d_out, d_res, y3, hstats, dn_w, dgb_dn, z3, stats3, ln3_w, dgb3, db3, pos_acc, pos_div,
+         (const bf16_t *)w2T, (const bf16_t *)h, (const bf16_t *)w1T, z2, stats2, ln2_w, dgb2, db2, (const bf16_t *)woT, (bf16_t *)dz3_c, (bf16_t *)dh, dz2,
+         (bf16_t *)dz2_c, (bf16_t *)d_o, R, reinterpret_cast<float *>(workspace),
+         reinterpret_cast<float *>(workspace) + (size_t)((R + RB - 1) / RB) * 8 * RB * C, workspace ? split_mode() : 1, dq_slabs, dq_ns,
+         (bf16_t *)dq_out};
+  hipStream_t s = (hipStream_t)stream;
+  switch (a.nsplit) {
+    case 2: return launch_bwd_b_split<2>(a, s);
+    case 4: return launch_bwd_b_split<4>(a, s);
+    case 8: return launch_bwd_b_split<8>(a, s);
+    default: return (a.dqc_next || a.dq_slabs) ? launch_bwd_b<1, 0, true>(a, s) : launch_bwd_b<1, 0, false>(a, s);
+  }
+}
+
 extern "C" int pd_dec_bwd_b(const void *dqc_next, const void *wqT_next, const float *d_out, const float *d_res, const float *y3, const float *hstats,
                             const float *dn_w, float *dgb_dn, const float *z3, const float *stats3, const float *ln3_w, float *dgb3, float *db3,
                             float *pos_acc, int pos_div, const void *w2T, const void *h, const void *w1T, const float *z2, const float *stats2,
                             const float *ln2_w, float *dgb2, float *db2, const void *woT, void *dz3_c, void *dh, float *dz2, void *dz2_c, void *d_o,
                             void *workspace, int R, void *stream)
 {
-  if (!d_out || !y3 || !hstats || !dn_w || !dgb_dn || !z3 || !stats3 || !ln3_w || !dgb3 || !db3 || !w2T || !h || !w1T || !z2 || !stats2 || !ln2_w ||
-      !dgb2 || !db2 || !woT || !dz3_c || !dh || !dz2 || !dz2_c || !d_o)
-    return pd_set_error(PD_ERR_INVALID_ARG, "pd_dec_bwd_b: null pointer");
-  if ((dqc_next != nullptr) != (wqT_next != nullptr) || (dqc_next && !pos_acc)) return pd_set_error(PD_ERR_INVALID_ARG, "pd_dec_bwd_b: next-layer operands");
-  if (R <= 0 || pos_div <= 0) return pd_set_error(PD_ERR_INVALID_ARG, "pd_dec_bwd_b: R = %d, pos_div = %d", R, pos_div);
-  BwdB a{(const bf16_t *)dqc_next, (const bf16_t *)wqT_next, d_out, d_res, y3, hstats, dn_w, dgb_dn, z3, stats3, ln3_w, dgb3, db3, pos_acc, pos_div,
-         (const bf16_t *)w2T, (const bf16_t *)h, (const bf16_t *)w1T, z2, stats2, ln2_w, dgb2, db2, (const bf16_t *)woT, (bf16_t *)dz3_c, (bf16_t *)dh, dz2,
-         (bf16_t *)dz2_c, (bf16_t *)d_o, R, reinterpret_cast<float *>(workspace),
-         reinterpret_cast<float *>(workspace) + (size_t)((R + RB - 1) / RB) * 8 * RB * C, workspace ? split_mode() : 1};
-  hipStream_t s = (hipStream_t)stream;
-  switch (a.nsplit) {
-    case 2: return launch_bwd_b_split<2>(a, s);
-    case 4: return launch_bwd_b_split<4>(a, s);
-    case 8: return launch_bwd_b_split<8>(a, s);
-    default: return a.dqc_next ? launch_bwd_b<1, 0, true>(a, s) : launch_bwd_b<1, 0, false>(a, s);
-  }
+  return dec_bwd_b_impl(dqc_next, nullptr, 0, nullptr, wqT_next, d_out, d_res, y3, hstats, dn_w, dgb_dn, z3, stats3, ln3_w, dgb3, db3, pos_acc, pos_div, w2T, h,
+                        w1T, z2, stats2, ln2_w, dgb2, db2, woT, dz3_c, dh, dz2, dz2_c, d_o, workspace, R, stream);
+}
+
+extern "C" int pd_dec_bwd_b_slabs(const float *dq_slabs, int nsplit, void *dq_out, const void *wqT_next, const float *d_out, const float *d_res,
+                                  const float *y3, const float *hstats, const float *dn_w, float *dgb_dn, const float *z3, const float *stats3,
+                                  const float *ln3_w, float *dgb3, float *db3, float *pos_acc, int pos_div, const void *w2T, const void *h,
+                                  const void *w1T, const float *z2, const float *stats2, const float *ln2_w, float *dgb2, float *db2, const void *woT,
+                                  void *dz3_c, void *dh, float *dz2, void *dz2_c, void *d_o, void *workspace, int R, void *stream)
+{
+  if (!dq_slabs) return pd_set_error(PD_ERR_INVALID_ARG, "pd_dec_bwd_b_slabs: null pointer");
+  return dec_bwd_b_impl(nullptr, dq_slabs, nsplit, dq_out, wqT_next, d_out, d_res, y3, hstats, dn_w, dgb_dn, z3, stats3, ln3_w, dgb3, db3, pos_acc, pos_div, w2T,
+                        h, w1T, z2, stats2, ln2_w, dgb2, db2, woT, dz3_c, dh, dz2, dz2_c, d_o, workspace, R, stream);
 }
 
 extern "C" int pd_dec_bwd_a(const void *dq, const void *dk, const void *dv, const void *wqkvT, const float *dz_in, const float *z, const float *stats,
diff --git a/partdistillation_amd/functions/attention.py b/partdistillation_amd/functions/attention.py
--- a/partdistillation_amd/functions/attention.py
+++ b/partdistillation_amd/functions/attention.py
@@ -51,6 +51,32 @@
     return dq, dk, dv
 
 
+def attn_fwd_splits(B, nheads, Lq, Lk, dtype):
+    return int(_lib.load().pd_attn_fwd_splits(B, nheads, Lq, Lk, _DT[dtype])) if dtype in _DT else 0
+
+
+def attn_bwd_splits(B, nheads, Lq, Lk, dtype):
+    return int(_lib.load().pd_attn_bwd_splits(B, nheads, Lq, Lk, _DT[dtype])) if dtype in _DT else 0
+
+
+def attn_fwd_parts_raw(q, k, v, m8, B, nheads, scale):
+    Lq, Lk = q.shape[0] // B, k.shape[0] // B
+    ws = _workspace(B, nheads, Lq, Lk, q.device)
+    _lib.check(_lib.load().pd_attn_fwd_parts_d32_ld(q.data_ptr(), k.data_ptr(), v.data_ptr(), m8.data_ptr() if m8 is not None else None,
+                                                    ws.data_ptr(), B, nheads, Lq, Lk, float(scale), _DT[q.dtype], _ld_kv(k, v), _stream()))
+    return ws
+
+
+def attn_bwd_parts_raw(q, k, v, m8, o, d_o, lse, B, nheads, scale):
+    Lq, Lk = q.shape[0] // B, k.shape[0] // B
+    dk, dv = (torch.empty(k.shape, dtype=k.dtype, device=k.device) for _ in range(2))
+    ws = _workspace(B, nheads, Lq, Lk, q.device)
+    _lib.check(_lib.load().pd_attn_bwd_parts_d32_ld(q.data_ptr(), k.data_ptr(), v.data_ptr(), m8.data_ptr() if m8 is not None else None,
+                                                    o.data_ptr(), d_o.data_ptr(), lse.data_ptr(), dk.data_ptr(), dv.data_ptr(), ws.data_ptr(), B,
+                                                    nheads, Lq, Lk, float(scale), _DT[q.dtype], _ld_kv(k, v), _stream()))
+    return ws, dk, dv
+
+
 class MaskedAttention32(Function):
 
     @staticmethod
diff --git a/partdistillation_amd/functions/declayer.py b/partdistillation_amd/functions/declayer.py
--- a/partdistillation_amd/functions/declayer.py
+++ b/partdistillation_amd/functions/declayer.py
@@ -71,11 +71,18 @@
     return torch.empty(shape, dtype=dtype, device=dev)
 
 
-def fwd_a(o, res, qpos, pos_div, w_o, b_o, ln_w, ln_b, eps, w_qkv, b_qkv):
-    R, dev = o.shape[0], o.device
+def fwd_a(o, res, qpos, pos_div, w_o, b_o, ln_w, ln_b, eps, w_qkv, b_qkv, parts=None):
+    R, dev = res.shape[0], res.device
     z, y = _e((R, C), torch.float32, dev), _e((R, C), torch.float32, dev)
     stats = _e((2, R), torch.float32, dev)
     y_c, ypos_c, q, k, v = (_e((R, C), bf16, dev) for _ in range(5))
+    if parts is not None:
+        o, lse = _e((R, C), bf16, dev), _e((pos_div, C // 32, R // pos_div), torch.float32, dev)
+        _lib.check(_lib.load().pd_dec_fwd_a_parts(parts[0].data_ptr(), int(parts[1]), o.data_ptr(), lse.data_ptr(), res.data_ptr(), qpos.data_ptr(),
+                                                  int(pos_div), w_o.data_ptr(), b_o.data_ptr(), ln_w.data_ptr(), ln_b.data_ptr(), float(eps),
+                                                  w_qkv.data_ptr(), b_qkv.data_ptr(), z.data_ptr(), stats.data_ptr(), y.data_ptr(), y_c.data_ptr(),
+                                                  ypos_c.data_ptr(), q.data_ptr(), k.data_ptr(), v.data_ptr(), R, _stream()))
+        return z, stats, y, y_c, ypos_c, q, k, v, o, lse
     _lib.check(_lib.load().pd_dec_fwd_a(o.data_ptr(), res.data_ptr(), qpos.data_ptr(), int(pos_div), w_o.data_ptr(), b_o.data_ptr(), ln_w.data_ptr(),
                                         ln_b.data_ptr(), float(eps), w_qkv.data_ptr(), b_qkv.data_ptr(), z.data_ptr(), stats.data_ptr(), y.data_ptr(),
                                         y_c.data_ptr(), ypos_c.data_ptr(), q.data_ptr(), k.data_ptr(), v.data_ptr(), R, _stream()))
@@ -109,6 +116,14 @@
     dz3_c, dz2_c, d_o = (_e((R, C), bf16, dev) for _ in range(3))
     dh = _e((R, FF), bf16, dev)
     dz2 = _e((R, C), torch.float32, dev)
+    if isinstance(dqc_next, tuple):
+        slabs, ns, dq = dqc_next
+        _lib.check(_lib.load().pd_dec_bwd_b_slabs(slabs.data_ptr(), int(ns), _p(dq), _p(wqT_next), d_out.data_ptr(), _p(d_res), y3.data_ptr(),
+                                                  hstats.data_ptr(), dn_w.data_ptr(), dgb_dn.data_ptr(), z3.data_ptr(), stats3.data_ptr(), ln3_w.data_ptr(),
+                                                  dgb3.data_ptr(), db3.data_ptr(), _p(pos_acc), int(pos_div), w2T.data_ptr(), h.data_ptr(), w1T.data_ptr(),
+                                                  z2.data_ptr(), stats2.data_ptr(), ln2_w.data_ptr(), dgb2.data_ptr(), db2.data_ptr(), woT.data_ptr(),
+                                                  dz3_c.data_ptr(), dh.data_ptr(), dz2.data_ptr(), dz2_c.data_ptr(), d_o.data_ptr(), _p(ws), R, _stream()))
+        return dz3_c, dh, dz2, dz2_c, d_o
     _lib.check(_lib.load().pd_dec_bwd_b(_p(dqc_next), _p(wqT_next), d_out.data_ptr(), _p(d_res), y3.data_ptr(), hstats.data_ptr(), dn_w.data_ptr(),
                                         dgb_dn.data_ptr(), z3.data_ptr(), stats3.data_ptr(), ln3_w.data_ptr(), dgb3.data_ptr(), db3.data_ptr(), _p(pos_acc),
                                         int(pos_div), w2T.data_ptr(), h.data_ptr(), w1T.data_ptr(), z2.data_ptr(), stats2.data_ptr(), ln2_w.data_ptr(),
diff --git a/partdistillation_amd/functions/decoder_core.py b/partdistillation_amd/functions/decoder_core.py
--- a/partdistillation_amd/functions/decoder_core.py
+++ b/partdistillation_amd/functions/decoder_core.py
@@ -9,7 +9,7 @@
 from . import conv_bf16, igemm
 from . import declayer as dl
 from . import smallgemm as sg
-from .attention import attn_bwd_raw, attn_fwd_raw
+from .attention import attn_bwd_parts_raw, attn_bwd_raw, attn_bwd_splits, attn_fwd_parts_raw, attn_fwd_raw, attn_fwd_splits
 
 
 class DecoderSpec:
@@ -77,6 +77,27 @@
 FUSED_HEAD = os.environ.get("PD_FUSED_HEAD", "1") != "0"
 KV_BATCH = os.environ.get("PD_DEC_KVBATCH", "1") != "0"
 FUSED_LAYER = os.environ.get("PD_DEC_FUSED", "1") != "0"
+ATTN_FOLD = os.environ.get("PD_DEC_ATTNFOLD", "1") != "0"
+
+
+def cross_attn_fwd_a(qc, k, v, mask, B, H, scale, tgt, qpos, p_co, cob, cnw, cnb, eps, p_si, sib, fold=None):
+    fold = ATTN_FOLD if fold is None else fold
+    ns = attn_fwd_splits(B, H, qc.shape[0] // B, k.shape[0] // B, qc.dtype) if fold else 0
+    if ns > 1:
+        parts = attn_fwd_parts_raw(qc, k, v, mask, B, H, scale)
+        return dl.fwd_a(None, tgt, qpos, B, p_co, cob, cnw, cnb, eps, p_si, sib, parts=(parts, ns))
+    o, lse = attn_fwd_raw(qc, k, v, mask, B, H, scale)
+    return dl.fwd_a(o, tgt, qpos, B, p_co, cob, cnw, cnb, eps, p_si, sib) + (o, lse)
+
+
+def cross_attn_bwd(q, k, v, mask, o, d_o, lse, B, H, scale, fold):
+    ns = attn_bwd_splits(B, H, q.shape[0] // B, k.shape[0] // B, q.dtype) if fold else 0
+    if ns > 1:
+        slabs, dk, dv = attn_bwd_parts_raw(q, k, v, mask, o, d_o, lse, B, H, scale)
+        dq = torch.empty_like(q)
+        return dq, dk, dv, (slabs, ns, dq)
+    dq, dk, dv = attn_bwd_raw(q, k, v, mask, o, d_o, lse, B, H, scale)
+    return dq, dk, dv, dq
 
 
 class _Acc:
@@ -335,8 +356,7 @@
                 v = igemm.linear(mem[lvl], ciw[2 * C:], cib[2 * C:])
             else:
                 k, v = sg.linear_multi([(mempos[lvl], ciw[C:2 * C], cib[C:2 * C]), (mem[lvl], ciw[2 * C:], cib[2 * C:])])
-            o, lse = attn_fwd_raw(qc, k, v, mask, B, H, scale)
-            z1, st1, y1, y1_c, y1pos_c, sq, sk, sv = dl.fwd_a(o, tgt, qpos, B, p_co, cob, cnw, cnb, spec.eps, p_si, sib)
+            z1, st1, y1, y1_c, y1pos_c, sq, sk, sv, o, lse = cross_attn_fwd_a(qc, k, v, mask, B, H, scale, tgt, qpos, p_co, cob, cnw, cnb, spec.eps, p_si, sib)
             cross = (tgtpos_c, qc, k, v, mask, o, lse, z1, st1[0], st1[1])
             o_s, lse_s = attn_fwd_raw(sq, sk, sv, None, B, H, scale)
             slf = (y1pos_c, y1_c, sq, sk, sv, o_s, lse_s, None, None, None)
@@ -493,7 +513,7 @@
                 tp_c, q, k, v, mask, o, lse, z1, m1, r1 = cross
                 dz1, dz1_c, d_oc = dl.bwd_a(dq, dk, dv, siT, dz2, z1, m1, cnw, A2(lay[i]["cnw"]), A(lay[i]["cob"]), A(s_pos), B, coT)
                 g_cow = _wgrad(dz1_c, o, queue=wq)
-                dq, dk, dv = attn_bwd_raw(q, k, v, mask, o, d_oc, lse, B, H, scale)
+                dq, dk, dv, dq_op = cross_attn_bwd(q, k, v, mask, o, d_oc, lse, B, H, scale, ATTN_FOLD and i > 0)
                 g_ciw = torch.empty_like(ciw)
                 cb = A(lay[i]["cib"])
                 _wgrad(dq, tp_c, g_ciw[:C], cb[:C], queue=wq)
@@ -501,7 +521,7 @@
                 _wgrad(dv, mem_f[lvl], g_ciw[2 * C:], cb[2 * C:], queue=wq, big=big)
                 dmempos[lvl] = dgrad_mem(dk, i, 1, dmempos[lvl])
                 dmem[lvl] = dgrad_mem(dv, i, 2, dmem[lvl])
-                dq_next = dq
+                dq_next = dq_op
                 if i == 0:
                     d_pos_c = _dgrad(dq, ciw[:C])
                 d_res = dz1
diff --git a/partdistillation_amd/lib.py b/partdistillation_amd/lib.py
--- a/partdistillation_amd/lib.py
+++ b/partdistillation_amd/lib.py
@@ -7,7 +7,7 @@
 CSRC = os.path.join(_HERE, "csrc")
 
 PD_F32, PD_F64, PD_BF16 = 0, 1, 2
-ABI_VERSION = 40
+ABI_VERSION = 41
 
 _c_int, _c_vp = ctypes.c_int, ctypes.c_void_p
 
@@ -74,6 +74,10 @@
     "pd_attn_bwd_d32": (_c_int, [_c_vp] * 11 + [_c_int] * 4 + [ctypes.c_float, _c_int, _c_vp]),
     "pd_attn_fwd_d32_ld": (_c_int, [_c_vp] * 7 + [_c_int] * 4 + [ctypes.c_float, _c_int, _c_int, _c_vp]),
     "pd_attn_bwd_d32_ld": (_c_int, [_c_vp] * 11 + [_c_int] * 4 + [ctypes.c_float, _c_int, _c_int, _c_vp]),
+    "pd_attn_fwd_splits": (_c_int, [_c_int] * 5),
+    "pd_attn_bwd_splits": (_c_int, [_c_int] * 5),
+    "pd_attn_fwd_parts_d32_ld": (_c_int, [_c_vp] * 5 + [_c_int] * 4 + [ctypes.c_float, _c_int, _c_int, _c_vp]),
+    "pd_attn_bwd_parts_d32_ld": (_c_int, [_c_vp] * 10 + [_c_int] * 4 + [ctypes.c_float, _c_int, _c_int, _c_vp]),
     "pd_nc_sums_f32": (_c_int, [_c_vp] * 6 + [_c_int] * 5 + [_c_vp]),
     "pd_nc_affine_f32": (_c_int, [_c_vp] * 4 + [_c_int] * 4 + [_c_vp]),
     "pd_nc_affine_amax_f32": (_c_int, [_c_vp] * 5 + [_c_int] * 4 + [_c_vp]),
@@ -122,6 +126,8 @@
     "pd_dec_fwd_a": (_c_int, [_c_vp] * 3 + [_c_int] + [_c_vp] * 4 + [ctypes.c_float] + [_c_vp] * 10 + [_c_int] + [_c_vp]),
     "pd_dec_fwd_b": (_c_int, [_c_vp] * 3 + [_c_int] + [_c_vp] * 20 + [ctypes.c_float] + [_c_vp] * 13 + [_c_int] * 2 + [_c_vp]),
     "pd_dec_bwd_b": (_c_int, [_c_vp] * 14 + [_c_int] + [_c_vp] * 15 + [_c_int] + [_c_vp]),
+    "pd_dec_fwd_a_parts": (_c_int, [_c_vp, _c_int] + [_c_vp] * 4 + [_c_int] + [_c_vp] * 4 + [ctypes.c_float] + [_c_vp] * 10 + [_c_int] + [_c_vp]),
+    "pd_dec_bwd_b_slabs": (_c_int, [_c_vp, _c_int] + [_c_vp] * 14 + [_c_int] + [_c_vp] * 15 + [_c_int] + [_c_vp]),
     "pd_dec_split": (_c_int, []),
     "pd_dec_workspace_bytes": (ctypes.c_int64, [_c_int]),
     "pd_dec_pack_table_bytes": (ctypes.c_int64, [_c_int]),
```

After: 111.8. No clear change (-0.3%).
